# onofreiandrea/quantum_simulations

Measured on AMD Instinct MI355X. Metric: gate-applications/sec (random 1q+CX circuit, complex128 statevector), higher is better.
Workload: dtype f64

## Files before the change

### include/qsim_hip.h

```cpp
#ifndef QSIM_HIP_H
#define QSIM_HIP_H

#include <stdint.h>

#ifdef __cplusplus
extern "C" {
#endif

#define QSIM_OK            0
#define QSIM_ERR_INVALID  (-1)
#define QSIM_ERR_NONLOCAL (-2)
#define QSIM_ERR_HIP      (-3)
#define QSIM_ERR_NOMEM    (-4)

typedef struct qsim_chunk qsim_chunk;

const char* qsim_last_error(void);
int qsim_version(void);
int qsim_device_count(int* count);

int qsim_create(int device, int n_local_qubits, qsim_chunk** out);
int qsim_create_view(qsim_chunk* parent, uint64_t offset_amps, int n_local_qubits,
                     qsim_chunk** out);
int qsim_wrap(int device, void* device_ptr, int n_local_qubits, void* stream,
              qsim_chunk** out);
int qsim_destroy(qsim_chunk* c);
int qsim_n_local_qubits(const qsim_chunk* c);
void* qsim_device_ptr(const qsim_chunk* c);

int qsim_init_zero(qsim_chunk* c, int set_amp0);
int qsim_init_random(qsim_chunk* c, uint64_t seed);
int qsim_upload(qsim_chunk* c, const double* re_im, uint64_t offset_amps, uint64_t count);
int qsim_download(qsim_chunk* c, double* re_im, uint64_t offset_amps, uint64_t count);
int qsim_download_c64(qsim_chunk* c, float* re_im, uint64_t offset_amps, uint64_t count);
int qsim_upload_c64(qsim_chunk* c, const float* re_im, uint64_t offset_amps, uint64_t count);
int qsim_copy(qsim_chunk* dst, const qsim_chunk* src);
int qsim_copy_variant(qsim_chunk* dst, const qsim_chunk* src, int variant);

int qsim_apply_1q(qsim_chunk* c, int qubit, const double U[8]);
int qsim_apply_2q(qsim_chunk* c, int qa, int qb, const double U[32]);
int qsim_apply_fused_k(qsim_chunk* c, int k, const int32_t* qubits, const double* M);
int qsim_apply_ops(qsim_chunk* c, int n_ops, const int32_t* nq, const int32_t* qubits,
                   const double* mats);
int qsim_apply_ops_unfused(qsim_chunk* c, int n_ops, const int32_t* nq, const int32_t* qubits,
                           const double* mats);
int qsim_last_pass_count(const qsim_chunk* c);
int qsim_plan_cache_clear(void);
int qsim_apply_ops_tiled(qsim_chunk* c, int n_ops, const int32_t* nq, const int32_t* qubits, const double* mats,
                         int n_tiles, const uint64_t* tile_masks);

typedef struct {
  uint32_t struct_size;
  const qsim_chunk* src; int32_t src_m; int32_t src_bits[3];
  qsim_chunk* dst; int32_t dst_m; int32_t dst_bits[3];
  qsim_chunk* dst_own; int32_t own_pattern;
  int32_t dst_parts;
  int32_t src_parts;
  int32_t n_tiles;
  const uint64_t* tile_masks;
} qsim_ops_io;
int qsim_apply_ops_io(qsim_chunk* c, int n_ops, const int32_t* nq, const int32_t* qubits,
                      const double* mats, const qsim_ops_io* io, int* n_passes);
int qsim_apply_ops_io_own_slab(const qsim_chunk* c, int32_t* in_chunk);
int qsim_apply_ops_io_load(qsim_chunk* c, int part);
int qsim_apply_ops_io_source_parts(const qsim_chunk* c, int32_t* n_parts, uint64_t* piece_amps, int32_t* n_launches);
int qsim_apply_ops_io_parts(const qsim_chunk* c, int32_t* n_parts, uint64_t* piece_amps, int32_t* n_launches);
int qsim_apply_ops_io_part(qsim_chunk* c, int part);
int qsim_split_piece_count(int n_local_qubits, int m, int dst_parts);
int qsim_tiles_per_workgroup(int n_local_qubits, int tile_bits, int n_fixed_bits);
#define QSIM_PASS_IMAGE_BYTES 4096
int qsim_plan_ops(int n_local_qubits, int n_ops, const int32_t* nq, const int32_t* qubits, const double* mats,
                  void* out, uint64_t out_capacity_bytes, int32_t* n_passes);
int qsim_plan_ops_tiled(int n_local_qubits, int n_ops, const int32_t* nq, const int32_t* qubits, const double* mats,
                        int n_tiles, const uint64_t* tile_masks, void* out, uint64_t out_capacity_bytes, int32_t* n_passes);

int qsim_plan_peek_pass(int n_local_qubits, int n_total_qubits, int n_ops, const int32_t* nq, const int32_t* qubits,
                        const double* mats, const uint8_t* done, uint64_t avoid_mask, uint64_t hint_mask, uint64_t* tile_mask,
                        uint64_t* need_mask, int32_t* n_members, int32_t* members);

int qsim_plan_search(int n_local_qubits, int n_ops, const int32_t* nq, const int32_t* qubits, const double* mats, int beam,
                     uint64_t* out_masks, int out_capacity, int32_t* n_passes);

int qsim_rewrite_ops(int n_qubits, int n_ops, const int32_t* nq, const int32_t* qubits, const double* mats, int32_t* out_nq,
                     int32_t* out_qubits, double* out_mats, int out_capacity, int32_t* n_out, int32_t* need_tile);

int qsim_plan_count_layouts(int n_local_qubits, int n_ops, const int32_t* nq, const int32_t* qubits, const double* mats,
                            int n_layouts, const int32_t* layouts, int32_t* n_passes, int n_threads);

int qsim_choose_layout(int n_local_qubits, int n_tiles, const uint64_t* tile_masks, int top_bit, const double* bit_cost,
                       const double* pair_cost, const double* triple_cost , uint64_t seed,
                       int sweeps, int32_t* out_l2p, double* cost_identity, double* cost_chosen);

int qsim_apply_1q_pair(qsim_chunk* c0, qsim_chunk* c1, const double U[8]);
int qsim_apply_2q_pair_qa_local(qsim_chunk* c0, qsim_chunk* c1, int qa, const double U[32]);
int qsim_apply_2q_pair_qb_local(qsim_chunk* c0, qsim_chunk* c1, int qb, const double U[32]);
int qsim_apply_2q_quad(qsim_chunk* c00, qsim_chunk* c01, qsim_chunk* c10, qsim_chunk* c11,
                       const double U[32]);

int qsim_pack_half(const qsim_chunk* src, int bit, int value, qsim_chunk* buf);
int qsim_unpack_half(qsim_chunk* dst, int bit, int value, const qsim_chunk* buf);
int qsim_pack_bits(const qsim_chunk* src, int m, const int32_t* bits, int pattern,
                   qsim_chunk* buf, uint64_t buf_offset_amps);
int qsim_unpack_bits(qsim_chunk* dst, int m, const int32_t* bits, int pattern,
                     const qsim_chunk* buf, uint64_t buf_offset_amps);
int qsim_pack_all(const qsim_chunk* src, int m, const int32_t* bits, qsim_chunk* buf, int skip_pattern,
                  int piece, int n_pieces);
int qsim_unpack_all(qsim_chunk* dst, int m, const int32_t* bits, const qsim_chunk* buf, int skip_pattern,
                    int piece, int n_pieces);

int qsim_swap_global_local(qsim_chunk* const* chunks, int n_chunks, const int32_t* global_bits,
                           const int32_t* local_bits, int m);

#define QSIM_COMM_ID_BYTES 128
typedef struct qsim_comm qsim_comm;
int qsim_comm_get_unique_id(uint8_t id[QSIM_COMM_ID_BYTES]);
int qsim_comm_init(int device, int rank, int world, const uint8_t id[QSIM_COMM_ID_BYTES], qsim_comm** out);
int qsim_comm_destroy(qsim_comm* comm);
int qsim_comm_rank(const qsim_comm* comm);
int qsim_comm_world(const qsim_comm* comm);
int qsim_comm_exchange(qsim_comm* comm, int n_peers, const int32_t* peers, const qsim_chunk* send,
                       const uint64_t* send_off, qsim_chunk* recv, const uint64_t* recv_off, uint64_t count_amps);
int qsim_comm_exchange_bg(qsim_comm* comm, int n_peers, const int32_t* peers, const qsim_chunk* send,
                          const uint64_t* send_off, qsim_chunk* recv, const uint64_t* recv_off, uint64_t count_amps,
                          uint32_t* ticket);
int qsim_comm_join(qsim_comm* comm, qsim_chunk* c);
int qsim_comm_wait(qsim_comm* comm, qsim_chunk* c, uint32_t ticket);
int qsim_comm_relayout(qsim_comm* comm, qsim_chunk* state, qsim_chunk* buf0, qsim_chunk* buf1, int m,
                       const int32_t* local_bits, const int32_t* global_bits, int n_pieces);
int qsim_comm_relayout_plan(int rank, int world, int n_local_qubits, int m, const int32_t* local_bits,
                            const int32_t* global_bits, int n_pieces, int32_t* out_n_pieces, int32_t* out_n_peers,
                            int32_t* out_own_pattern, int32_t* out_peers, uint64_t* out_slab_offsets,
                            uint64_t* out_piece_amps);
int qsim_comm_relayout_loopback(qsim_comm* comm, qsim_chunk* state, qsim_chunk* buf0, qsim_chunk* buf1, int m,
                                const int32_t* local_bits, const int32_t* global_bits, int n_pieces, int as_rank,
                                int as_world);
int qsim_apply_1q_pair_remote(qsim_comm* comm, qsim_chunk* shard, qsim_chunk* buf, int partner_rank, int my_side,
                              const double U[8]);
int qsim_apply_2q_pair_qa_local_remote(qsim_comm* comm, qsim_chunk* shard, qsim_chunk* buf, int partner_rank,
                                       int my_side, int qa, const double U[32]);
int qsim_apply_2q_pair_qb_local_remote(qsim_comm* comm, qsim_chunk* shard, qsim_chunk* buf, int partner_rank,
                                       int my_side, int qb, const double U[32]);

int qsim_apply_2q_quad_remote(qsim_comm* comm, qsim_chunk* shard, qsim_chunk* buf, const int32_t ranks[4], int my_index,
                              const double U[32]);
typedef struct { int32_t n_ops; const int32_t* nq; const int32_t* qubits; const double* mats; } qsim_op_list;
int qsim_comm_relayout_fused(qsim_comm* comm, qsim_chunk* shard, qsim_chunk* send, qsim_chunk* recv,
                             const qsim_op_list* before, const qsim_op_list* after, int m, const int32_t* local_bits,
                             const int32_t* global_bits, int n_pieces, int as_rank, int as_world, int* n_passes);

int qsim_count_nonzero(qsim_chunk* c, double eps, uint64_t* count);
int qsim_export_nonzero(qsim_chunk* c, double eps, uint64_t capacity, uint64_t* out_idx, double* out_re_im,
                        uint64_t* n_rows);
int qsim_sync(qsim_chunk* c);
int qsim_norm2(qsim_chunk* c, double* out);
int qsim_probabilities(qsim_chunk* c, int r, const int32_t* qubits, double* out);
int qsim_reduced_density_matrix(qsim_chunk* c, int r, const int32_t* qubits, double* out);
int qsim_expectation_pauli(qsim_chunk* c, int n_terms, const uint64_t* x_masks, const uint64_t* z_masks, double* out,
                           int* n_passes);
int qsim_plan_expectation(int n_local_qubits, int n_terms, const uint64_t* x_masks, int32_t* pass_of_term,
                          uint64_t* tile_masks, int* n_passes);
int qsim_sample(qsim_chunk* c, uint64_t n_shots, const double* randnums, uint64_t* out_indices, double* total, int* n_passes);
int qsim_sample_locate(uint64_t n_blocks, const double* block_cdf, uint64_t n_shots, const double* randnums,
                       uint64_t* out_block, double* out_local);
int qsim_sample_block_bits(void);
int qsim_max_abs_err_closed_form(qsim_chunk* c, int kind, int n_total_qubits,
                                 uint64_t base_index, double* out);
int qsim_max_abs_err_closed_form_perm(qsim_chunk* c, int kind, int n_total_qubits,
                                      uint64_t base_index, const int32_t* log_to_phys,
                                      double* out);
int qsim_fingerprint(qsim_chunk* c, int n_total_qubits, uint64_t base_index, const int32_t* log_to_phys, uint64_t seed,
                     uint64_t sel_mask, uint64_t sel_value, double out[2]);
int qsim_time_begin(qsim_chunk* c);
int qsim_time_end(qsim_chunk* c, float* elapsed_ms);


typedef struct {
  char kernel[48];
  uint64_t launches;
  double total_ms;
  double algorithmic_bytes;
  double hbm_bytes;
  uint64_t streaming_launches;
} qsim_profile_entry;
int qsim_profile_begin(qsim_chunk* c);
int qsim_profile_end(qsim_chunk* c, int max_entries, int* n_entries, qsim_profile_entry* out);

#ifdef __cplusplus
}
#endif
#endif
```

### quantum_simulations_amd/_lib.py

```python
from __future__ import annotations

import ctypes as C
import os
from pathlib import Path

LIB_NAME = "libqsim_hip.so"
LIB_PATH = Path(os.environ.get("QSIM_LIBRARY") or (Path(__file__).resolve().parent / LIB_NAME))

QSIM_OK = 0
QSIM_ERR_INVALID = -1
QSIM_ERR_NONLOCAL = -2
QSIM_ERR_HIP = -3
QSIM_ERR_NOMEM = -4


class QsimLibraryMissing(RuntimeError):
    pass


class QsimHipError(RuntimeError):
    pass


_P = C.c_void_p
_D = C.POINTER(C.c_double)
_I32 = C.POINTER(C.c_int32)

SIGNATURES = {
    "qsim_last_error": (C.c_char_p, []),
    "qsim_version": (C.c_int, []),
    "qsim_device_count": (C.c_int, [C.POINTER(C.c_int)]),
    "qsim_create": (C.c_int, [C.c_int, C.c_int, C.POINTER(_P)]),
    "qsim_create_view": (C.c_int, [_P, C.c_uint64, C.c_int, C.POINTER(_P)]),
    "qsim_wrap": (C.c_int, [C.c_int, _P, C.c_int, _P, C.POINTER(_P)]),
    "qsim_destroy": (C.c_int, [_P]),
    "qsim_n_local_qubits": (C.c_int, [_P]),
    "qsim_device_ptr": (_P, [_P]),
    "qsim_init_zero": (C.c_int, [_P, C.c_int]),
    "qsim_init_random": (C.c_int, [_P, C.c_uint64]),
    "qsim_upload": (C.c_int, [_P, _P, C.c_uint64, C.c_uint64]),
    "qsim_download": (C.c_int, [_P, _P, C.c_uint64, C.c_uint64]),
    "qsim_download_c64": (C.c_int, [_P, _P, C.c_uint64, C.c_uint64]),
    "qsim_upload_c64": (C.c_int, [_P, _P, C.c_uint64, C.c_uint64]),
    "qsim_copy": (C.c_int, [_P, _P]),
    "qsim_copy_variant": (C.c_int, [_P, _P, C.c_int]),
    "qsim_apply_1q": (C.c_int, [_P, C.c_int, _P]),
    "qsim_apply_2q": (C.c_int, [_P, C.c_int, C.c_int, _P]),
    "qsim_apply_fused_k": (C.c_int, [_P, C.c_int, _P, _P]),
    "qsim_apply_ops": (C.c_int, [_P, C.c_int, _P, _P, _P]),
    "qsim_apply_ops_unfused": (C.c_int, [_P, C.c_int, _P, _P, _P]),
    "qsim_plan_ops": (C.c_int, [C.c_int, C.c_int, _P, _P, _P, _P, C.c_uint64, _P]),
    "qsim_plan_ops_tiled": (C.c_int, [C.c_int, C.c_int, _P, _P, _P, C.c_int, _P, _P, C.c_uint64, _P]),
    "qsim_plan_search": (C.c_int, [C.c_int, C.c_int, _P, _P, _P, C.c_int, _P, C.c_int, _P]),
    "qsim_rewrite_ops": (C.c_int, [C.c_int, C.c_int, _P, _P, _P, _P, _P, _P, C.c_int, _P, _P]),
    "qsim_apply_ops_tiled": (C.c_int, [_P, C.c_int, _P, _P, _P, C.c_int, _P]),
    "qsim_choose_layout": (C.c_int, [C.c_int, C.c_int, _P, C.c_int, _P, _P, _P, C.c_uint64, C.c_int, _P, C.POINTER(C.c_double), C.POINTER(C.c_double)]),
    "qsim_plan_count_layouts": (C.c_int, [C.c_int, C.c_int, _P, _P, _P, C.c_int, _P, _P, C.c_int]),
    "qsim_plan_peek_pass": (C.c_int, [C.c_int, C.c_int, C.c_int, _P, _P, _P, _P, C.c_uint64, C.c_uint64, C.POINTER(C.c_uint64),
                                      C.POINTER(C.c_uint64), C.POINTER(C.c_int32), _P]),
    "qsim_last_pass_count": (C.c_int, [_P]),
    "qsim_plan_cache_clear": (C.c_int, []),
    "qsim_apply_ops_io": (C.c_int, [_P, C.c_int, _P, _P, _P, _P, C.POINTER(C.c_int)]),
    "qsim_apply_ops_io_part": (C.c_int, [_P, C.c_int]),
    "qsim_apply_ops_io_load": (C.c_int, [_P, C.c_int]),
    "qsim_apply_ops_io_source_parts": (C.c_int, [_P, _P, _P, _P]),
    "qsim_apply_ops_io_parts": (C.c_int, [_P, _P, _P, _P]),
    "qsim_apply_ops_io_own_slab": (C.c_int, [_P, _P]),
    "qsim_split_piece_count": (C.c_int, [C.c_int, C.c_int, C.c_int]),
    "qsim_tiles_per_workgroup": (C.c_int, [C.c_int, C.c_int, C.c_int]),
    "qsim_apply_1q_pair": (C.c_int, [_P, _P, _P]),
    "qsim_apply_2q_pair_qa_local": (C.c_int, [_P, _P, C.c_int, _P]),
    "qsim_apply_2q_pair_qb_local": (C.c_int, [_P, _P, C.c_int, _P]),
    "qsim_apply_2q_quad": (C.c_int, [_P, _P, _P, _P, _P]),
    "qsim_pack_half": (C.c_int, [_P, C.c_int, C.c_int, _P]),
    "qsim_unpack_half": (C.c_int, [_P, C.c_int, C.c_int, _P]),
    "qsim_pack_bits": (C.c_int, [_P, C.c_int, _P, C.c_int, _P, C.c_uint64]),
    "qsim_unpack_bits": (C.c_int, [_P, C.c_int, _P, C.c_int, _P, C.c_uint64]),
    "qsim_pack_all": (C.c_int, [_P, C.c_int, _P, _P, C.c_int, C.c_int, C.c_int]),
    "qsim_unpack_all": (C.c_int, [_P, C.c_int, _P, _P, C.c_int, C.c_int, C.c_int]),
    "qsim_swap_global_local": (C.c_int, [_P, C.c_int, _P, _P, C.c_int]),
    "qsim_comm_get_unique_id": (C.c_int, [_P]),
    "qsim_comm_init": (C.c_int, [C.c_int, C.c_int, C.c_int, _P, C.POINTER(_P)]),
    "qsim_comm_destroy": (C.c_int, [_P]),
    "qsim_comm_rank": (C.c_int, [_P]),
    "qsim_comm_world": (C.c_int, [_P]),
    "qsim_comm_exchange": (C.c_int, [_P, C.c_int, _P, _P, _P, _P, _P, C.c_uint64]),
    "qsim_comm_exchange_bg": (C.c_int, [_P, C.c_int, _P, _P, _P, _P, _P, C.c_uint64, C.POINTER(C.c_uint32)]),
    "qsim_comm_wait": (C.c_int, [_P, _P, C.c_uint32]),
    "qsim_comm_join": (C.c_int, [_P, _P]),
    "qsim_comm_relayout": (C.c_int, [_P, _P, _P, _P, C.c_int, _P, _P, C.c_int]),
    "qsim_comm_relayout_plan": (C.c_int, [C.c_int, C.c_int, C.c_int, C.c_int, _P, _P, C.c_int, _P, _P, _P, _P, _P, _P]),
    "qsim_comm_relayout_loopback": (C.c_int, [_P, _P, _P, _P, C.c_int, _P, _P, C.c_int, C.c_int, C.c_int]),
    "qsim_apply_1q_pair_remote": (C.c_int, [_P, _P, _P, C.c_int, C.c_int, _P]),
    "qsim_apply_2q_pair_qa_local_remote": (C.c_int, [_P, _P, _P, C.c_int, C.c_int, C.c_int, _P]),
    "qsim_apply_2q_pair_qb_local_remote": (C.c_int, [_P, _P, _P, C.c_int, C.c_int, C.c_int, _P]),
    "qsim_apply_2q_quad_remote": (C.c_int, [_P, _P, _P, _P, C.c_int, _P]),
    "qsim_comm_relayout_fused": (C.c_int, [_P, _P, _P, _P, _P, _P, C.c_int, _P, _P, C.c_int, C.c_int, C.c_int, C.POINTER(C.c_int)]),
    "qsim_count_nonzero": (C.c_int, [_P, C.c_double, C.POINTER(C.c_uint64)]),
    "qsim_export_nonzero": (C.c_int, [_P, C.c_double, C.c_uint64, _P, _P, C.POINTER(C.c_uint64)]),
    "qsim_sync": (C.c_int, [_P]),
    "qsim_norm2": (C.c_int, [_P, C.POINTER(C.c_double)]),
    "qsim_probabilities": (C.c_int, [_P, C.c_int, _P, _P]),
    "qsim_reduced_density_matrix": (C.c_int, [_P, C.c_int, _P, _P]),
    "qsim_expectation_pauli": (C.c_int, [_P, C.c_int, _P, _P, _P, C.POINTER(C.c_int)]),
    "qsim_plan_expectation": (C.c_int, [C.c_int, C.c_int, _P, _P, _P, C.POINTER(C.c_int)]),
    "qsim_sample": (C.c_int, [_P, C.c_uint64, _P, _P, C.POINTER(C.c_double), C.POINTER(C.c_int)]),
    "qsim_sample_locate": (C.c_int, [C.c_uint64, _P, C.c_uint64, _P, _P, _P]),
    "qsim_sample_block_bits": (C.c_int, []),
    "qsim_max_abs_err_closed_form": (C.c_int, [_P, C.c_int, C.c_int, C.c_uint64,
                                               C.POINTER(C.c_double)]),
    "qsim_max_abs_err_closed_form_perm": (C.c_int, [_P, C.c_int, C.c_int, C.c_uint64, _P,
                                                    C.POINTER(C.c_double)]),
    "qsim_fingerprint": (C.c_int, [_P, C.c_int, C.c_uint64, _P, C.c_uint64, C.c_uint64, C.c_uint64, _P]),
    "qsim_time_begin": (C.c_int, [_P]),
    "qsim_time_end": (C.c_int, [_P, C.POINTER(C.c_float)]),
    "qsim_profile_begin": (C.c_int, [_P]),
    "qsim_profile_end": (C.c_int, [_P, C.c_int, C.POINTER(C.c_int), _P]),
}


class OpsIo(C.Structure):
    _fields_ = [("struct_size", C.c_uint32),
                ("src", C.c_void_p), ("src_m", C.c_int32), ("src_bits", C.c_int32 * 3),
                ("dst", C.c_void_p), ("dst_m", C.c_int32), ("dst_bits", C.c_int32 * 3),
                ("dst_own", C.c_void_p), ("own_pattern", C.c_int32), ("dst_parts", C.c_int32), ("src_parts", C.c_int32),
                ("n_tiles", C.c_int32), ("tile_masks", C.c_void_p)]

    def __init__(self, *args, **kw):
        super().__init__(*args, **kw)
        self.struct_size = C.sizeof(OpsIo)


class OpList(C.Structure):
    _fields_ = [("n_ops", C.c_int32), ("nq", C.c_void_p), ("qubits", C.c_void_p), ("mats", C.c_void_p)]


class ProfileEntry(C.Structure):
    _fields_ = [("kernel", C.c_char * 48), ("launches", C.c_uint64),
                ("total_ms", C.c_double), ("algorithmic_bytes", C.c_double),
                ("hbm_bytes", C.c_double), ("streaming_launches", C.c_uint64)]

_lib = None


def source_hash() -> str:
    import hashlib
    h = hashlib.sha256()
    csrc = Path(__file__).resolve().parent / "csrc"
    for path in sorted(list(csrc.glob("*.h")) + list(csrc.glob("*.hip")) + list(csrc.glob("*.py")) + [csrc / "Makefile"]):
        h.update(path.name.encode())
        h.update(path.read_bytes())
    return h.hexdigest()[:16]


def load() -> C.CDLL:
    global _lib
    if _lib is not None:
        return _lib
    if not LIB_PATH.exists():
        raise QsimLibraryMissing(
            f"{LIB_PATH} not found: the HIP extension is not built. Run "
            "`python -c 'import __graft_entry__ as g; g.build()'` (needs hipcc). "
            "This engine has no CPU fallback.")
    lib = C.CDLL(str(LIB_PATH))
    for name, (restype, argtypes) in SIGNATURES.items():
        fn = getattr(lib, name)
        fn.restype = restype
        fn.argtypes = argtypes
    _lib = lib
    return lib


def ptr(a):
    return None if a is None else a.ctypes.data_as(C.c_void_p)


def check(rc: int) -> None:
    if rc == QSIM_OK:
        return
    msg = (load().qsim_last_error() or b"").decode("utf-8", "replace")
    if rc == QSIM_ERR_NONLOCAL:
        raise NotImplementedError(msg)
    if rc == QSIM_ERR_INVALID:
        raise ValueError(msg)
    if rc == QSIM_ERR_NOMEM:
        raise MemoryError(msg)
    raise QsimHipError(msg)
```

### quantum_simulations_amd/csrc/abi_plan.h

```cpp
extern "C" {
int qsim_plan_cache_clear(void) {
  std::lock_guard<std::mutex> lock(g_plan_cache_mu);
  g_plan_cache.clear();
  return QSIM_OK;
}

static_assert(sizeof(TileArgs) == QSIM_PASS_IMAGE_BYTES, "pass image = the kernel-argument block of k_tile");

int qsim_plan_ops(int n_local_qubits, int n_ops, const int32_t* nq, const int32_t* qubits, const double* mats,
                  void* out, uint64_t out_capacity_bytes, int32_t* n_passes) {
  return qsim_plan_ops_tiled(n_local_qubits, n_ops, nq, qubits, mats, 0, nullptr, out, out_capacity_bytes, n_passes);
}

int qsim_plan_ops_tiled(int n_local_qubits, int n_ops, const int32_t* nq, const int32_t* qubits, const double* mats,
                        int n_tiles, const uint64_t* tile_masks, void* out, uint64_t out_capacity_bytes, int32_t* n_passes) {
  if (n_tiles < 0 || (n_tiles && !tile_masks)) return fail(QSIM_ERR_INVALID, "qsim_plan_ops_tiled: bad tile list");
  if (!n_passes) return fail(QSIM_ERR_INVALID, "qsim_plan_ops: n_passes is null");
  if (n_local_qubits < kTileMinChunk || n_local_qubits > kTileMaxQubits)
    return fail(QSIM_ERR_INVALID, "qsim_plan_ops: fused passes need %d..%d local qubits", kTileMinChunk, kTileMaxQubits);
  int rc = check_op_list(n_ops, nq, qubits, mats, n_local_qubits, kQubitOfPlan);
  if (rc) return rc;
  std::vector<FusedOp> ops;
  classify_ops(n_ops, nq, qubits, mats, &ops);
  int passes = 0;
  char* dst = (char*)out;
  uint64_t used = 0;
  const TileHint hint = {tile_masks, n_tiles};
  rc = plan_fused(n_local_qubits, ops, &passes, [&](TileArgs& a, int T, double, bool, bool) {
    if (dst) {
      if (used + sizeof(TileArgs) > out_capacity_bytes) return fail(QSIM_ERR_INVALID, "qsim_plan_ops: output buffer too small");
      std::memcpy(dst + used, &a, sizeof a);
    }
    used += sizeof(TileArgs);
    return (int)QSIM_OK;
  }, n_tiles ? &hint : nullptr);
  *n_passes = passes;
  return rc;
}

int qsim_plan_search(int n_local_qubits, int n_ops, const int32_t* nq, const int32_t* qubits, const double* mats, int beam,
                     uint64_t* out_masks, int out_capacity, int32_t* n_passes) {
  if (!n_passes || out_capacity < 0) return fail(QSIM_ERR_INVALID, "qsim_plan_search: bad arguments");
  if (n_local_qubits < kTileMinChunk || n_local_qubits > kTileMaxQubits)
    return fail(QSIM_ERR_INVALID, "qsim_plan_search: fused passes need %d..%d local qubits", kTileMinChunk, kTileMaxQubits);
  int rc = check_op_list(n_ops, nq, qubits, mats, n_local_qubits, kQubitOfPlan);
  if (rc) return rc;
  std::vector<FusedOp> ops;
  classify_ops(n_ops, nq, qubits, mats, &ops);
#ifdef QSIM_PROBES
  if (beam <= 0) if (const char* e = getenv("QSIM_PLAN_BEAM")) beam = atoi(e);
#endif
  std::vector<u64> masks;
  int passes = 0;
  rc = plan_search(n_local_qubits, ops, beam, &masks, &passes);
  if (rc) return rc;
  *n_passes = passes;
  if (out_masks) {
    if ((int)masks.size() > out_capacity) return fail(QSIM_ERR_INVALID, "qsim_plan_search: output buffer too small");
    for (size_t p = 0; p < masks.size(); ++p) out_masks[p] = masks[p];
  }
  return QSIM_OK;
}

int qsim_rewrite_ops(int n_qubits, int n_ops, const int32_t* nq, const int32_t* qubits, const double* mats, int32_t* out_nq,
                     int32_t* out_qubits, double* out_mats, int out_capacity, int32_t* n_out, int32_t* need_tile) {
  if (!n_out || out_capacity < 0 || (out_capacity && (!out_nq || !out_qubits || !out_mats)))
    return fail(QSIM_ERR_INVALID, "qsim_rewrite_ops: bad arguments");
  if (n_qubits < 1 || n_qubits > 63) return fail(QSIM_ERR_INVALID, "qsim_rewrite_ops: bad qubit count %d", n_qubits);
  int rc = check_op_list(n_ops, nq, qubits, mats, n_qubits, kQubitOfState);
  if (rc) return rc;
  std::vector<RwOp> ops;
  int need_in = 0, need_out = 0;
  rewrite_op_list(n_qubits, n_ops, nq, qubits, mats, &ops, &need_in);
  *n_out = (int32_t)ops.size();
  if (ops.size() > (size_t)out_capacity) return fail(QSIM_ERR_INVALID, "qsim_rewrite_ops: output buffer too small (%d ops)", (int)ops.size());
  for (size_t i = 0; i < ops.size(); ++i) {
    out_nq[i] = ops[i].nq;
    out_qubits[2 * i] = ops[i].q[0];
    out_qubits[2 * i + 1] = ops[i].nq == 2 ? ops[i].q[1] : 0;
    std::memcpy(out_mats + 32 * i, ops[i].U, sizeof ops[i].U);
    need_out += rw_needs_tile(ops[i]);
  }
  if (need_tile) { need_tile[0] = need_in; need_tile[1] = need_out; }
  return QSIM_OK;
}

int qsim_plan_peek_pass(int n_local_qubits, int n_total_qubits, int n_ops, const int32_t* nq, const int32_t* qubits,
                        const double* mats, const uint8_t* done, uint64_t avoid_mask, uint64_t hint_mask, uint64_t* tile_mask,
                        uint64_t* need_mask, int32_t* n_members, int32_t* members) {
  if (!done || !tile_mask || !n_members || !members) return fail(QSIM_ERR_INVALID, "qsim_plan_peek_pass: null argument");
  if (n_local_qubits < kTileMinChunk || n_local_qubits > kTileMaxQubits)
    return fail(QSIM_ERR_INVALID, "qsim_plan_peek_pass: fused passes need %d..%d local qubits", kTileMinChunk, kTileMaxQubits);
  if (n_total_qubits < n_local_qubits || n_total_qubits > 63) return fail(QSIM_ERR_INVALID, "qsim_plan_peek_pass: bad total qubit count %d", n_total_qubits);
  int rc = check_op_list(n_ops, nq, qubits, mats, n_total_qubits, kQubitOfState);
  if (rc) return rc;
  std::vector<FusedOp> ops;
  std::vector<int32_t> origin;
  classify_ops(n_ops, nq, qubits, mats, &ops, &origin);
  std::vector<uint8_t> done_ops;
  for (int32_t i : origin) done_ops.push_back(done[i]);
  std::vector<size_t> held;
  PeekPlan peek;
  peek.n_total = n_total_qubits;
  peek.done = done_ops.data();
  peek.avoid = avoid_mask;
  peek.tile_mask = peek.need_mask = 0;
  peek.members = &held;
  int passes = 0;
  const TileHint hint = {&hint_mask, 1};
  rc = plan_fused(n_local_qubits, ops, &passes, [](TileArgs&, int, double, bool, bool) { return (int)QSIM_OK; },
                  hint_mask ? &hint : nullptr, &peek);
  if (rc) return rc;
  *tile_mask = peek.tile_mask;
  if (need_mask) *need_mask = peek.need_mask;
  *n_members = (int32_t)held.size();
  for (size_t j = 0; j < held.size(); ++j) members[j] = origin[held[j]];
  return QSIM_OK;
}

int qsim_plan_count_layouts(int n_local_qubits, int n_ops, const int32_t* nq, const int32_t* qubits, const double* mats,
                            int n_layouts, const int32_t* layouts, int32_t* n_passes, int n_threads) {
  if (!n_passes || n_layouts < 0 || (n_layouts && !layouts)) return fail(QSIM_ERR_INVALID, "qsim_plan_count_layouts: bad arguments");
  if (n_local_qubits < kTileMinChunk || n_local_qubits > kTileMaxQubits)
    return fail(QSIM_ERR_INVALID, "qsim_plan_count_layouts: fused passes need %d..%d local qubits", kTileMinChunk, kTileMaxQubits);
  const int bad_ops = check_op_list(n_ops, nq, qubits, mats, n_local_qubits, kQubitOfPlan);
  if (bad_ops) return bad_ops;
  for (int l = 0; l < n_layouts; ++l) {
    u64 seen = 0;
    for (int q = 0; q < n_local_qubits; ++q) {
      const int b = layouts[(size_t)l * n_local_qubits + q];
      if (b < 0 || b >= n_local_qubits || ((seen >> b) & 1)) return fail(QSIM_ERR_INVALID, "qsim_plan_count_layouts: layout %d is not a permutation", l);
      seen |= 1ull << b;
    }
  }
  (void)tuning();
  std::atomic<int> next{0}, bad{0};
  auto work = [&]() {
    std::vector<FusedOp> ops;
    for (;;) {
      const int l = next.fetch_add(1);
      if (l >= n_layouts) return;
      const int32_t* lay = layouts + (size_t)l * n_local_qubits;
      ops.clear();
      for (int i = 0; i < n_ops; ++i) {
        const int32_t q[2] = {lay[qubits[2 * i]], nq[i] == 2 ? lay[qubits[2 * i + 1]] : -1};
        FusedOp o;
        if (classify_op(nq[i], q, mats + 32 * (size_t)i, &o)) ops.push_back(o);
      }
      int passes = 0;
      const int rc = plan_fused(n_local_qubits, ops, &passes, [](TileArgs&, int, double, bool, bool) { return (int)QSIM_OK; });
      if (rc) bad.store(1);
      n_passes[l] = rc ? -1 : passes;
    }
  };
  const int nt = std::max(1, std::min(n_threads > 0 ? n_threads : 1, std::min(n_layouts, 64)));
  std::vector<std::thread> pool;
  for (int t = 1; t < nt; ++t) pool.emplace_back(work);
  work();
  for (std::thread& t : pool) t.join();
  if (bad.load()) return fail(QSIM_ERR_INVALID, "qsim_plan_count_layouts: a layout could not be planned");
  return QSIM_OK;
}

int qsim_choose_layout(int n_local_qubits, int n_tiles, const uint64_t* tile_masks, int top_bit, const double* bit_cost,
                       const double* pair_cost, const double* triple_cost, uint64_t seed, int sweeps, int32_t* out_l2p,
                       double* cost_identity, double* cost_chosen) {
  const int n = n_local_qubits, low = kTileLow;
  if (n < low + 2 || n > 62 || n_tiles < 0 || (n_tiles && !tile_masks) || !bit_cost || !pair_cost || !out_l2p || top_bit < low || top_bit > 62 || sweeps < 1)
    return fail(QSIM_ERR_INVALID, "qsim_choose_layout: bad arguments");
  const int nb = top_bit - low + 1;
  std::vector<std::vector<int>> tiles((size_t)n_tiles);
  std::vector<std::vector<int>> member((size_t)n);
  for (int t = 0; t < n_tiles; ++t)
    for (int q = low; q < n; ++q)
      if ((tile_masks[t] >> q) & 1) { tiles[(size_t)t].push_back(q); member[(size_t)q].push_back(t); }
  std::vector<double> sym((size_t)nb * nb, 0.0);
  for (int a = 0; a < nb; ++a)
    for (int b = a + 1; b < nb; ++b) sym[(size_t)a * nb + b] = sym[(size_t)b * nb + a] = pair_cost[(size_t)a * nb + b];
  std::vector<int> l2p((size_t)n);
  for (int q = 0; q < n; ++q) l2p[(size_t)q] = q;
  auto cost_of = [&](int t) {
    int idx[64], m = 0;
    for (int q : tiles[(size_t)t]) idx[m++] = std::min(l2p[(size_t)q], top_bit) - low;
    double c = 0;
    for (int i = 0; i < m; ++i) {
      c += bit_cost[idx[i]];
      for (int j = i + 1; j < m; ++j) c += sym[(size_t)idx[i] * nb + idx[j]];
    }
    if (triple_cost) {
      std::sort(idx, idx + m);
      for (int i = 0; i < m; ++i)
        for (int j = i + 1; j < m; ++j) {
          if (idx[j] == idx[i]) continue;
          const double* row = triple_cost + ((size_t)idx[i] * nb + idx[j]) * nb;
          for (int l = j + 1; l < m; ++l) if (idx[l] != idx[j]) c += row[idx[l]];
        }
    }
    return c;
  };
  std::vector<double> costs((size_t)n_tiles);
  double cur = 0;
  for (int t = 0; t < n_tiles; ++t) cur += (costs[(size_t)t] = cost_of(t));
  const double identity = cur;
  double best = cur;
  std::vector<int> best_l2p = l2p;
  u64 rs = seed * 0x9E3779B97F4A7C15ull + 0x2545F4914F6CDD1Dull;
  auto rnd = [&]() { rs ^= rs << 13; rs ^= rs >> 7; rs ^= rs << 17; return rs; };
  const int np_ = n - low;
  const long steps = (long)sweeps * np_ * np_ / 2;
  const double T0 = std::max(1e-3, 0.03 * identity / std::max(1, n_tiles));
  std::vector<int> touched;
  std::vector<double> fresh;
  for (long it = 0; it < steps && n_tiles > 0; ++it) {
    const int a = low + (int)(rnd() % (u64)np_);
    int b = low + (int)(rnd() % (u64)(np_ - 1));
    if (b >= a) ++b;
    touched.clear();
    for (int t : member[(size_t)a]) touched.push_back(t);
    for (int t : member[(size_t)b]) if (std::find(touched.begin(), touched.end(), t) == touched.end()) touched.push_back(t);
    if (touched.empty()) continue;
    std::swap(l2p[(size_t)a], l2p[(size_t)b]);
    fresh.clear();
    double delta = 0;
    for (int t : touched) { fresh.push_back(cost_of(t)); delta += fresh.back() - costs[(size_t)t]; }
    const double T = T0 * (1.0 - (double)it / (double)steps) + 1e-4;
    const double u = (double)(rnd() >> 11) * 0x1p-53;
    if (delta < 0 || u < std::exp(-delta / T)) {
      for (size_t i = 0; i < touched.size(); ++i) costs[(size_t)touched[i]] = fresh[i];
      cur += delta;
      if (cur < best - 1e-12) { best = cur; best_l2p = l2p; }
    } else {
      std::swap(l2p[(size_t)a], l2p[(size_t)b]);
    }
  }
  for (int q = 0; q < n; ++q) out_l2p[q] = best_l2p[(size_t)q];
  if (cost_identity) *cost_identity = identity;
  if (cost_chosen) *cost_chosen = best;
  return QSIM_OK;
}

int qsim_split_piece_count(int n_local_qubits, int m, int dst_parts) {
  if (m < 1 || m > 3 || m > n_local_qubits || dst_parts == 0) return 1;
  return 1 << piece_bits_for(n_local_qubits, m, dst_parts < 0 ? -dst_parts : dst_parts, dst_parts < 0 ? kTileLow : 20);
}

int qsim_tiles_per_workgroup(int n_local_qubits, int tile_bits, int n_fixed_bits) {
  return tiles_per_workgroup(n_local_qubits, tile_bits, n_fixed_bits);
}
}
```

### quantum_simulations_amd/csrc/abi_relayout.h

```cpp

static int check_swapped_bits(int k, int g_bits, int m, const int32_t* local_bits, const int32_t* global_bits, const char* what,
                              const char* shards, const char* index_bit) {
  for (int i = 0; i < m; ++i) {
    if (local_bits[i] < 0 || local_bits[i] >= k) return fail(QSIM_ERR_NONLOCAL, "%s: local bit %d is non-local for 2^%d %s", what, local_bits[i], k, shards);
    if (global_bits[i] < 0 || global_bits[i] >= g_bits) return fail(QSIM_ERR_INVALID, "%s: %s %d out of range", what, index_bit, global_bits[i]);
    for (int j = 0; j < i; ++j)
      if (local_bits[j] == local_bits[i] || global_bits[j] == global_bits[i]) return fail(QSIM_ERR_INVALID, "%s: repeated bit", what);
  }
  return QSIM_OK;
}
static int peer_of(int rank, int m, const int32_t* global_bits, int d) {
  for (int i = 0; i < m; ++i) rank = (rank & ~(1 << global_bits[i])) | (((d >> i) & 1) << global_bits[i]);
  return rank;
}

static int partial_launch_args(const TileArgs& planned, int T, int k, const int* piece_bits, int n_free, int g, TileArgs* out) {
  *out = planned;
  out->nfix = (uint8_t)n_free;
  out->fix_or = 0;
  for (int i = 0; i < n_free; ++i) {
    const int bit = piece_bits[i];
    int below = 0;
    for (int j = 0; j < T - kTileLow; ++j) below += out->h[j] < bit;
    out->fix_pos[i] = (uint8_t)(bit - below);
    if ((g >> i) & 1) out->fix_or |= 1ull << bit;
    if (bit >= k || bit < kTileLow) return fail(QSIM_ERR_INVALID, "internal: piece bit %d", bit);
  }
  return QSIM_OK;
}

extern "C" {
static int half_slab(qsim_chunk* state, int bit, int value, qsim_chunk* buf, bool pack, const char* what) {
  int rc = check_chunk(state, what);
  if (rc || (rc = check_chunk(buf, what))) return rc;
  if (bit < 0 || bit >= state->k || buf->k != state->k - 1 || (value != 0 && value != 1))
    return fail(QSIM_ERR_INVALID, "%s: bit %d / buffer size mismatch", what, bit);
  HIP_TRY(hipSetDevice(state->device));
  const u64 n_half = amps(buf), off = value ? (1ull << bit) : 0ull;
  if (pack) hipLaunchKernelGGL(k_pack_half, dim3(stream_grid(n_half)), dim3(kBlock), 0, state->stream, buf->amp, (const double2*)state->amp, n_half, bit, off);
  else hipLaunchKernelGGL(k_unpack_half, dim3(stream_grid(n_half)), dim3(kBlock), 0, state->stream, state->amp, (const double2*)buf->amp, n_half, bit, off);
  HIP_TRY(hipGetLastError());
  return QSIM_OK;
}
int qsim_pack_half(const qsim_chunk* src, int bit, int value, qsim_chunk* buf) {
  return half_slab(const_cast<qsim_chunk*>(src), bit, value, buf, true, "qsim_pack_half");
}
int qsim_unpack_half(qsim_chunk* dst, int bit, int value, const qsim_chunk* buf) {
  return half_slab(dst, bit, value, const_cast<qsim_chunk*>(buf), false, "qsim_unpack_half");
}

static int slab_args(const qsim_chunk* c, int m, const int32_t* bits, int pattern, const qsim_chunk* buf,
                     uint64_t buf_offset, int pos[3], u64* value_off, u64* n_slab) {
  if (m < 1 || m > 3 || !bits) return fail(QSIM_ERR_INVALID, "slab: 1..3 bits expected, got %d", m);
  if (m > c->k) return fail(QSIM_ERR_INVALID, "slab: more bits than the chunk has");
  if (pattern < 0 || pattern >= (1 << m)) return fail(QSIM_ERR_INVALID, "slab: pattern out of range");
  int sorted[3] = {0, 0, 0};
  *value_off = 0;
  for (int i = 0; i < m; ++i) {
    if (bits[i] < 0 || bits[i] >= c->k) return fail(QSIM_ERR_INVALID, "slab: bit %d out of range", bits[i]);
    for (int j = 0; j < i; ++j)
      if (bits[j] == bits[i]) return fail(QSIM_ERR_INVALID, "slab: repeated bit %d", bits[i]);
    sorted[i] = bits[i];
    if ((pattern >> i) & 1) *value_off |= 1ull << bits[i];
  }
  std::sort(sorted, sorted + m);
  for (int i = 0; i < 3; ++i) pos[i] = sorted[i];
  *n_slab = 1ull << (c->k - m);
  if (buf_offset > amps(buf) || *n_slab > amps(buf) - buf_offset)
    return fail(QSIM_ERR_INVALID, "slab: buffer range outside the buffer chunk");
  return QSIM_OK;
}

static int one_slab(qsim_chunk* state, int m, const int32_t* bits, int pattern, qsim_chunk* buf, uint64_t buf_offset_amps,
                    bool pack, const char* what) {
  int rc = check_chunk(state, what);
  if (rc || (rc = check_chunk(buf, what))) return rc;
  int pos[3];
  u64 voff, n_slab;
  if ((rc = slab_args(state, m, bits, pattern, buf, buf_offset_amps, pos, &voff, &n_slab))) return rc;
  HIP_TRY(hipSetDevice(state->device));
  if (pack) hipLaunchKernelGGL(k_pack_bits, dim3(stream_grid(n_slab)), dim3(kBlock), 0, state->stream,
                               buf->amp + buf_offset_amps, (const double2*)state->amp, n_slab, m, pos[0], pos[1], pos[2], voff);
  else hipLaunchKernelGGL(k_unpack_bits, dim3(stream_grid(n_slab)), dim3(kBlock), 0, state->stream,
                          state->amp, (const double2*)buf->amp + buf_offset_amps, n_slab, m, pos[0], pos[1], pos[2], voff);
  HIP_TRY(hipGetLastError());
  return QSIM_OK;
}
int qsim_pack_bits(const qsim_chunk* src, int m, const int32_t* bits, int pattern, qsim_chunk* buf, uint64_t buf_offset_amps) {
  return one_slab(const_cast<qsim_chunk*>(src), m, bits, pattern, buf, buf_offset_amps, true, "qsim_pack_bits");
}
int qsim_unpack_bits(qsim_chunk* dst, int m, const int32_t* bits, int pattern, const qsim_chunk* buf, uint64_t buf_offset_amps) {
  return one_slab(dst, m, bits, pattern, const_cast<qsim_chunk*>(buf), buf_offset_amps, false, "qsim_unpack_bits");
}

static int slabs_all(qsim_chunk* state, int m, const int32_t* bits, qsim_chunk* buf, int skip_pattern, int piece,
                     int n_pieces, bool pack, const char* what) {
  int rc = check_chunk(state, what);
  if (rc || (rc = check_chunk(buf, what))) return rc;
  int pos[3];
  u64 voff, n_slab;
  if ((rc = slab_args(state, m, bits, 0, buf, 0, pos, &voff, &n_slab))) return rc;
  if (amps(buf) < amps(state)) return fail(QSIM_ERR_INVALID, "%s: the buffer must hold all 2^%d slabs", what, m);
  if (skip_pattern < -1 || skip_pattern >= (1 << m)) return fail(QSIM_ERR_INVALID, "%s: skip pattern out of range", what);
  int piece_bits = 0;
  while ((1 << piece_bits) < n_pieces) ++piece_bits;
  if (n_pieces < 1 || (1 << piece_bits) != n_pieces || piece_bits > 3 || piece_bits > state->k - m)
    return fail(QSIM_ERR_INVALID, "%s: n_pieces must be 1, 2, 4 or 8 and at most the slab length", what);
  if (piece < 0 || piece >= n_pieces) return fail(QSIM_ERR_INVALID, "%s: piece %d out of range", what, piece);
  int pb[3] = {0, 0, 0};
  top_free_bits(state->k, m, bits, piece_bits, pb);
  HIP_TRY(hipSetDevice(state->device));
  const int b0 = bits[0], b1 = m > 1 ? bits[1] : 0, b2 = m > 2 ? bits[2] : 0;
  const int s_lo = pos[0], s_mid = m > 1 ? pos[1] : 0, s_hi = m > 2 ? pos[2] : 0;
  const u64 n = amps(state) >> piece_bits;
  if (pack)
    hipLaunchKernelGGL((k_slabs_all<true>), dim3(stream_grid(n)), dim3(kBlock), 0, state->stream, state->amp, buf->amp,
                       n, m, b0, b1, b2, s_hi, s_mid, s_lo, state->k - m, skip_pattern, piece_bits, pb[0], pb[1], pb[2], piece);
  else
    hipLaunchKernelGGL((k_slabs_all<false>), dim3(stream_grid(n)), dim3(kBlock), 0, state->stream, state->amp, buf->amp,
                       n, m, b0, b1, b2, s_hi, s_mid, s_lo, state->k - m, skip_pattern, piece_bits, pb[0], pb[1], pb[2], piece);
  HIP_TRY(hipGetLastError());
  return QSIM_OK;
}

int qsim_pack_all(const qsim_chunk* src, int m, const int32_t* bits, qsim_chunk* buf, int skip_pattern, int piece, int n_pieces) {
  return slabs_all(const_cast<qsim_chunk*>(src), m, bits, buf, skip_pattern, piece, n_pieces, true, "qsim_pack_all");
}
int qsim_unpack_all(qsim_chunk* dst, int m, const int32_t* bits, const qsim_chunk* buf, int skip_pattern, int piece, int n_pieces) {
  return slabs_all(dst, m, bits, const_cast<qsim_chunk*>(buf), skip_pattern, piece, n_pieces, false, "qsim_unpack_all");
}

int qsim_swap_global_local(qsim_chunk* const* chunks, int n_chunks, const int32_t* global_bits, const int32_t* local_bits, int m) {
  if (!chunks || !global_bits || !local_bits) return fail(QSIM_ERR_INVALID, "qsim_swap_global_local: null argument");
  if (m < 1 || m > 3) return fail(QSIM_ERR_INVALID, "qsim_swap_global_local: 1..3 qubit pairs expected, got %d", m);
  if (n_chunks < 2 || (n_chunks & (n_chunks - 1)) || n_chunks > 4096)
    return fail(QSIM_ERR_INVALID, "qsim_swap_global_local: chunk count must be a power of two >= 2");
  int rc = QSIM_OK;
  for (int i = 0; i < n_chunks; ++i) {
    if ((rc = check_chunk(chunks[i], "qsim_swap_global_local"))) return rc;
    if (chunks[i]->k != chunks[0]->k || chunks[i]->device != chunks[0]->device)
      return fail(QSIM_ERR_INVALID, "qsim_swap_global_local: chunks differ in size or device");
  }
  const int k = chunks[0]->k;
  int g_bits = 0;
  while ((1 << g_bits) < n_chunks) ++g_bits;
  if ((rc = check_swapped_bits(k, g_bits, m, local_bits, global_bits, "qsim_swap_global_local", "chunks", "chunk-index bit"))) return rc;
  int sorted[3] = {0, 0, 0};
  std::copy(local_bits, local_bits + m, sorted);
  std::sort(sorted, sorted + m);
  HIP_TRY(hipSetDevice(chunks[0]->device));
  const u64 n_slab = 1ull << (k - m);
  auto local_offset = [&](int pattern) {
    u64 off = 0;
    for (int i = 0; i < m; ++i) if ((pattern >> i) & 1) off |= 1ull << local_bits[i];
    return off;
  };
  for (int c = 0; c < n_chunks; ++c) {
    int mine = 0;
    for (int i = 0; i < m; ++i) mine |= ((c >> global_bits[i]) & 1) << i;
    for (int d = 0; d < (1 << m); ++d) {
      if (d == mine) continue;
      const int peer = peer_of(c, m, global_bits, d);
      if (peer < c) continue;
      hipLaunchKernelGGL(k_swap_slabs, dim3(stream_grid(n_slab)), dim3(kBlock), 0, chunks[0]->stream,
                         chunks[c]->amp, chunks[peer]->amp, n_slab, m, sorted[0], sorted[1], sorted[2],
                         local_offset(d), local_offset(mine));
      HIP_TRY(hipGetLastError());
    }
  }
  return QSIM_OK;
}

static int finish_out_side(qsim_chunk* c, const qsim_ops_io* io, FusedIo& fio) {
  int rc = QSIM_OK;
  if (io->dst && io->dst_parts != 0) {
    PendingLast* p = c->pending ? c->pending : (c->pending = new PendingLast());
    const bool stashed = p->mode == PendingLast::kStashed;
    p->mode = stashed ? PendingLast::kTile : (fio.fused_out ? PendingLast::kDone : PendingLast::kPack);
    p->m = io->dst_m;
    for (int i = 0; i < io->dst_m; ++i) p->bits[i] = io->dst_bits[i];
    p->dst = io->dst; p->dst_own = io->dst_own; p->own_pattern = io->own_pattern;
    const int min_piece_bits = io->dst_parts < 0 ? kTileLow : 20;
    const int want = io->dst_parts < 0 ? -io->dst_parts : io->dst_parts;
    plan_parts(p, c->k, want, p->mode == PendingLast::kTile ? p->a.h : nullptr, p->mode == PendingLast::kTile ? p->T - kTileLow : 0, min_piece_bits);
  } else if (io->dst && !fio.fused_out) {
    if ((rc = slabs_all(c, io->dst_m, io->dst_bits, io->dst, io->own_pattern, 0, 1, true, "qsim_apply_ops_io"))) return rc;
    if (io->own_pattern >= 0) {
      const uint64_t slab = 1ull << (c->k - io->dst_m);
      if ((rc = qsim_pack_bits(c, io->dst_m, io->dst_bits, io->own_pattern, io->dst_own, (uint64_t)io->own_pattern * slab))) return rc;
    }
  }
  return QSIM_OK;
}

static int apply_ops_io_deferred(qsim_chunk* c, int n_ops, const int32_t* nq, const int32_t* qubits, const double* mats,
                                 const qsim_ops_io* io, const FusedIo& fio_in, const std::vector<FusedOp>& ops, bool tiles, int* n_passes) {
  DeferredIo* d = c->deferred ? c->deferred : (c->deferred = new DeferredIo());
  *d = DeferredIo();
  d->tiles = tiles;
  d->n_ops = n_ops;
  d->io = *io;
  d->fio = fio_in;
  const int want = io->src_parts < 0 ? -io->src_parts : io->src_parts;
  d->nb = piece_bits_for(c->k, io->src_m, want, io->src_parts < 0 ? kTileLow : 20);
  top_free_bits(c->k, io->src_m, io->src_bits, d->nb, d->piece_bit);
  int passes = 0, rc = QSIM_OK;
  if (io->src && !d->fio.src) ++passes;
  if (tiles) {
    int p = 0;
    const TileHint hint = {io->tile_masks, io->n_tiles};
    if ((rc = run_fused(c, ops, &p, &d->fio, n_ops, nq, qubits, mats, &d->passes, io->n_tiles ? &hint : nullptr))) return rc;
    d->io.tile_masks = nullptr;
    d->io.n_tiles = 0;
    passes += p;
    c->own_in_chunk = d->fio.own_in_chunk;
    if (d->fio.src && !d->fio.fused_in) return fail(QSIM_ERR_INVALID, "internal: the first pass did not take the source buffer");
    const bool first_stores = d->passes.size() == 1 && io->dst != nullptr;
    if (d->fio.src && !first_stores && !d->passes.empty() && d->passes[0].T == kTileBitsMax) {
      auto is_tile = [&](int b) { for (int j = 0; j < kTileBitsMax - kTileLow; ++j) if (d->passes[0].a.h[j] == b) return true; return false; };
      while (d->nb_free < d->nb && !is_tile(d->piece_bit[d->nb - 1 - d->nb_free])) ++d->nb_free;
    }
  } else {
    d->nq.assign(nq, nq + n_ops);
    d->qubits.assign(qubits, qubits + 2 * (size_t)n_ops);
    d->mats.assign(mats, mats + 32 * (size_t)n_ops);
    passes += n_ops;
  }
  if (io->dst && !d->fio.fused_out) ++passes;
  d->active = true;
  c->last_passes = passes;
  if (n_passes) *n_passes = passes;
  return QSIM_OK;
}

int qsim_apply_ops_io(qsim_chunk* c, int n_ops, const int32_t* nq, const int32_t* qubits, const double* mats, const qsim_ops_io* io, int* n_passes) {
  int rc = validate_ops(c, n_ops, nq, qubits, mats);
  if (rc) return rc;
  if (!io) return fail(QSIM_ERR_INVALID, "qsim_apply_ops_io: io is null");
  if (io->struct_size != sizeof(qsim_ops_io))
    return fail(QSIM_ERR_INVALID, "qsim_apply_ops_io: io->struct_size is %u, this library's qsim_ops_io has %zu bytes (zero the struct, "
                "set struct_size = sizeof(qsim_ops_io) and rebuild against this library's include/qsim_hip.h)", io->struct_size, sizeof(qsim_ops_io));
  if (io->n_tiles < 0 || (io->n_tiles && !io->tile_masks)) return fail(QSIM_ERR_INVALID, "qsim_apply_ops_io: bad tile list");
  auto check_side = [&](const qsim_chunk* b, int m, const int32_t* bits, const char* side) -> int {
    int r = check_chunk(b, "qsim_apply_ops_io");
    if (r) return r;
    if (b->k != c->k || b->device != c->device || b->amp == c->amp)
      return fail(QSIM_ERR_INVALID, "qsim_apply_ops_io: the %s buffer must be a distinct chunk of the state's size and device", side);
    if (m < 1 || m > 3 || m > c->k) return fail(QSIM_ERR_INVALID, "qsim_apply_ops_io: %s: 1..3 slab bits expected, got %d", side, m);
    for (int i = 0; i < m; ++i) {
      if (bits[i] < 0 || bits[i] >= c->k) return fail(QSIM_ERR_NONLOCAL, "qsim_apply_ops_io: %s slab bit %d is non-local for 2^%d amplitudes", side, bits[i], c->k);
      for (int j = 0; j < i; ++j) if (bits[j] == bits[i]) return fail(QSIM_ERR_INVALID, "qsim_apply_ops_io: %s: repeated slab bit %d", side, bits[i]);
    }
    return QSIM_OK;
  };
  if (io->src && (rc = check_side(io->src, io->src_m, io->src_bits, "source"))) return rc;
  if (io->dst) {
    if ((rc = check_side(io->dst, io->dst_m, io->dst_bits, "destination"))) return rc;
    if (io->own_pattern < -1 || io->own_pattern >= (1 << io->dst_m)) return fail(QSIM_ERR_INVALID, "qsim_apply_ops_io: own_pattern out of range");
    if (io->own_pattern >= 0 && (rc = check_side(io->dst_own, io->dst_m, io->dst_bits, "own-slab"))) return rc;
    if (io->own_pattern >= 0 && io->dst_own->amp == io->dst->amp) return fail(QSIM_ERR_INVALID, "qsim_apply_ops_io: the own-slab buffer must differ from the destination");
    if (io->src && io->src->amp == io->dst->amp)
      return fail(QSIM_ERR_INVALID, "qsim_apply_ops_io: the source buffer must differ from the destination buffer (one pass may read and write them at once)");
  }
  HIP_TRY(hipSetDevice(c->device));
  std::vector<FusedOp> ops;
  classify_ops(n_ops, nq, qubits, mats, &ops);
  const bool tiles = c->k >= kTileMinChunk && c->k <= kTileMaxQubits && !ops.empty();
  auto whole_lines = [](int m, const int32_t* bits) { for (int i = 0; i < m; ++i) if (bits[i] < kTileLow) return false; return true; };
  FusedIo fio;
  if (io->src && tiles && whole_lines(io->src_m, io->src_bits)) {
    fio.src = io->src;
    fio.in.m = io->src_m;
    for (int i = 0; i < io->src_m; ++i) fio.in.bits[i] = io->src_bits[i];
  }
  if (io->dst && tiles && whole_lines(io->dst_m, io->dst_bits)) {
    fio.dst = io->dst;
    fio.dst_own = io->dst_own;
    fio.own_pattern = io->own_pattern;
    fio.out.m = io->dst_m;
    for (int i = 0; i < io->dst_m; ++i) fio.out.bits[i] = io->dst_bits[i];
  }
  const bool parts = io->dst && io->dst_parts != 0;
  c->own_in_chunk = false;
  if (parts_pending(c))
    return fail(QSIM_ERR_INVALID, "qsim_apply_ops_io: pieces of an earlier split call are pending on this chunk (qsim_apply_ops_io_part / _load)");
  fio.parts = parts;
  if (io->src && io->src_parts != 0) return apply_ops_io_deferred(c, n_ops, nq, qubits, mats, io, fio, ops, tiles, n_passes);
  int passes = 0;
  if (io->src && !fio.src) {
    if ((rc = slabs_all(c, io->src_m, io->src_bits, const_cast<qsim_chunk*>(io->src), -1, 0, 1, false, "qsim_apply_ops_io"))) return rc;
    ++passes;
  }
  if (tiles) {
    int p = 0;
    const TileHint hint = {io->tile_masks, io->n_tiles};
    if ((rc = run_fused(c, ops, &p, &fio, n_ops, nq, qubits, mats, nullptr, io->n_tiles ? &hint : nullptr))) return rc;
    passes += p;
    c->own_in_chunk = fio.own_in_chunk;
    if (fio.src && !fio.fused_in) return fail(QSIM_ERR_INVALID, "internal: the first pass did not take the source buffer");
  } else {
    if ((rc = qsim_apply_ops_unfused(c, n_ops, nq, qubits, mats))) return rc;
    passes += n_ops;
  }
  if (io->dst && !fio.fused_out) ++passes;
  if ((rc = finish_out_side(c, io, fio))) return rc;
  c->last_passes = passes;
  if (n_passes) *n_passes = passes;
  return QSIM_OK;
}

int qsim_apply_ops_io_part(qsim_chunk* c, int part) {
  int rc = check_chunk(c, "qsim_apply_ops_io_part");
  if (rc) return rc;
  PendingLast* p = c->pending;
  if (!p || p->mode == PendingLast::kNone) return fail(QSIM_ERR_INVALID, "qsim_apply_ops_io_part: no split op list is pending on this chunk");
  const int n_parts = 1 << p->nb;
  if (part < 0 || part >= n_parts) return fail(QSIM_ERR_INVALID, "qsim_apply_ops_io_part: piece %d out of range", part);
  if ((p->stored >> part) & 1) return fail(QSIM_ERR_INVALID, "qsim_apply_ops_io_part: piece %d has been stored already", part);
  HIP_TRY(hipSetDevice(c->device));
  if (p->mode == PendingLast::kTile) {
    const int g = part >> (p->nb - p->nb_free);
    if (!((p->launched >> g) & 1)) {
      TileArgs a;
      if ((rc = partial_launch_args(p->a, p->T, c->k, p->piece_bit + (p->nb - p->nb_free), p->nb_free, g, &a))) return rc;
      if ((rc = launch_tile_any(a, p->T, c, c->stream, p->alg_bytes / (double)(1 << p->nb_free)))) return rc;
      p->launched |= 1u << g;
    }
  } else if (p->mode == PendingLast::kPack) {
    if ((rc = slabs_all(c, p->m, p->bits, p->dst, p->own_pattern, part, n_parts, true, "qsim_apply_ops_io_part"))) return rc;
    if (p->own_pattern >= 0 && p->stored == 0) {
      const uint64_t slab = 1ull << (c->k - p->m);
      if ((rc = qsim_pack_bits(c, p->m, p->bits, p->own_pattern, p->dst_own, (uint64_t)p->own_pattern * slab))) return rc;
    }
  }
  p->stored |= 1u << part;
  if (p->stored == (1u << n_parts) - 1u) p->mode = PendingLast::kNone;
  return QSIM_OK;
}

int qsim_apply_ops_io_load(qsim_chunk* c, int part) {
  int rc = check_chunk(c, "qsim_apply_ops_io_load");
  if (rc) return rc;
  DeferredIo* d = c->deferred;
  if (!d || !d->active) return fail(QSIM_ERR_INVALID, "qsim_apply_ops_io_load: no op list with a split source is pending on this chunk");
  const int n_parts = 1 << d->nb;
  if (part < 0 || part >= n_parts) return fail(QSIM_ERR_INVALID, "qsim_apply_ops_io_load: piece %d out of range", part);
  if ((d->announced >> part) & 1) return fail(QSIM_ERR_INVALID, "qsim_apply_ops_io_load: piece %d has been announced already", part);
  HIP_TRY(hipSetDevice(c->device));
  PendingGuard guard{c, true};
  d->announced |= 1u << part;
  const qsim_ops_io* io = &d->io;
  if (!d->fio.src) {
    if ((rc = slabs_all(c, io->src_m, io->src_bits, const_cast<qsim_chunk*>(io->src), -1, part, n_parts, false, "qsim_apply_ops_io_load"))) return rc;
  } else if (d->nb_free > 0) {
    const int shift = d->nb - d->nb_free;
    const int g = part >> shift;
    const unsigned group = ((1u << (1 << shift)) - 1u) << (g << shift);
    if ((d->announced & group) == group && !((d->launched >> g) & 1)) {
      CachedPass& p0 = d->passes[0];
      TileArgs a;
      if ((rc = partial_launch_args(p0.a, p0.T, c->k, d->piece_bit + shift, d->nb_free, g, &a))) return rc;
      if ((rc = launch_tile_any(a, p0.T, c, c->stream, p0.alg_bytes / (double)(1 << d->nb_free)))) return rc;
      d->launched |= 1u << g;
    }
  }
  if (d->announced != (n_parts >= 32 ? ~0u : (1u << n_parts) - 1u)) { guard.armed = false; return QSIM_OK; }
  d->active = false;
  if (d->tiles) {
    for (size_t i = 0; i < d->passes.size(); ++i) {
      if (i == 0 && d->nb_free > 0) continue;
      CachedPass& p = d->passes[i];
      if ((rc = dispatch_planned(c, p.a, p.T, p.alg_bytes, i + 1 == d->passes.size(), &d->fio))) return rc;
    }
  } else {
    if ((rc = qsim_apply_ops_unfused(c, d->n_ops, d->nq.data(), d->qubits.data(), d->mats.data()))) return rc;
  }
  if ((rc = finish_out_side(c, io, d->fio))) return rc;
  guard.armed = false;
  return QSIM_OK;
}

int qsim_apply_ops_io_own_slab(const qsim_chunk* c, int32_t* in_chunk) {
  if (!c || !in_chunk) return fail(QSIM_ERR_INVALID, "qsim_apply_ops_io_own_slab: null argument");
  *in_chunk = c->own_in_chunk ? 1 : 0;
  return QSIM_OK;
}

int qsim_apply_ops_io_source_parts(const qsim_chunk* c, int32_t* n_parts, uint64_t* piece_amps, int32_t* n_launches) {
  if (!c || !c->deferred || !c->deferred->active) return fail(QSIM_ERR_INVALID, "qsim_apply_ops_io_source_parts: nothing pending on this chunk");
  const DeferredIo* d = c->deferred;
  if (n_parts) *n_parts = 1 << d->nb;
  if (piece_amps) *piece_amps = (1ull << (c->k - d->io.src_m)) >> d->nb;
  if (n_launches) *n_launches = d->nb_free > 0 ? (1 << d->nb_free) : 0;
  return QSIM_OK;
}

int qsim_apply_ops_io_parts(const qsim_chunk* c, int32_t* n_parts, uint64_t* piece_amps, int32_t* n_launches) {
  if (!c || !c->pending || c->pending->mode == PendingLast::kNone) return fail(QSIM_ERR_INVALID, "qsim_apply_ops_io_parts: no split op list is pending on this chunk");
  const PendingLast* p = c->pending;
  if (n_parts) *n_parts = 1 << p->nb;
  if (piece_amps) *piece_amps = (1ull << (c->k - p->m)) >> p->nb;
  if (n_launches) *n_launches = p->mode == PendingLast::kTile ? (1 << p->nb_free) : (p->mode == PendingLast::kPack ? (1 << p->nb) : 0);
  return QSIM_OK;
}
}
```

### quantum_simulations_amd/csrc/tile_groups.h

```cpp

template <class Fn>
static void for_each_triple(unsigned mask, Fn&& fn) {
  for (unsigned a = mask; a; a &= a - 1)
    for (unsigned b = a & (a - 1); b; b &= b - 1)
      for (unsigned c = b & (b - 1); c; c &= c - 1) fn((a & -a) | (b & -b) | (c & -c));
}

struct PhaseRuns {
  struct Acc { uint16_t blk; u64 outer; double2 phi[3]; unsigned touched; };
  std::vector<Acc> open;

  static int run_bytes(unsigned touched) { const int n = __builtin_popcount(touched); return desc_bytes(n == 1 ? 2 : (n == 2 ? 6 : 14)); }
  int reserve() const {
    int bytes = 0;
    for (const Acc& acc : open) bytes += run_bytes(acc.touched);
    return bytes;
  }
  void add(uint16_t blk, u64 outer, int r, double2 phase) {
    size_t i = 0;
    while (i < open.size() && !(open[i].blk == blk && open[i].outer == outer)) ++i;
    if (i == open.size()) {
      Acc acc;
      acc.blk = blk; acc.outer = outer; acc.touched = 0;
      for (int e = 0; e < 3; ++e) acc.phi[e] = make_double2(1.0, 0.0);
      open.push_back(acc);
    }
    Acc& acc = open[i];
    acc.phi[r] = cmul(acc.phi[r], phase);
    acc.touched |= 1u << r;
  }
  static TileDesc single(const TileDesc& pred, int r, double2 v) {
    TileDesc s1 = pred;
    const int fam = phase_family(v);
    s1.opcode = (uint8_t)(fam + (1u << r));
    if (fam == OPC_PHASE) { s1.m[0] = v.x; s1.m[1] = v.y; s1.nd = 2; }
    return s1;
  }
  static int cost1(double2 v) {
    if (!tuning().tile_special) return 16;
    return (v.x == -1 && v.y == 0) ? 8 : ((v.x == 0 && (v.y == 1 || v.y == -1)) ? 12 : 16);
  }
  int flush(size_t i, std::vector<TileDesc>* gates) {
    const Acc acc = open[i];
    open.erase(open.begin() + (long)i);
    const size_t from = gates->size();
    TileDesc d;
    std::memset(&d, 0, sizeof d);
    d.blk_mask = acc.blk;
    d.outer_mask = acc.outer;
    double2 m[3];
    int nm = 0, regs[3];
    for (int r = 0; r < 3; ++r) if (acc.touched & (1u << r)) { regs[nm] = r; m[nm++] = acc.phi[r]; }
    auto put = [&](int at, double2 v) { d.m[2 * at] = v.x; d.m[2 * at + 1] = v.y; };
    int separate = 0;
    for (int e = 0; e < nm; ++e) separate += cost1(m[e]);
    if (nm == 1 || separate < (nm == 2 ? 24 : 28)) {
      for (int e = 0; e < nm; ++e) gates->push_back(single(d, regs[e], m[e]));
    } else if (nm == 2) {
      d.opcode = (uint8_t)(OPC_DIAGR + (acc.touched == 3 ? 0 : acc.touched == 5 ? 1 : 2));
      put(0, m[0]); put(1, m[1]); put(2, cmul(m[0], m[1])); d.nd = 6;
      gates->push_back(d);
    } else {
      d.opcode = (uint8_t)(OPC_DIAGR + 3);
      const double2 ab = cmul(m[0], m[1]);
      put(0, m[0]); put(1, m[1]); put(2, m[2]);
      put(3, ab); put(4, cmul(m[0], m[2])); put(5, cmul(m[1], m[2])); put(6, cmul(ab, m[2]));
      d.nd = 14;
      gates->push_back(d);
    }
    int bytes = 0;
    for (size_t g = from; g < gates->size(); ++g) bytes += desc_bytes((*gates)[g]);
    return bytes;
  }
};

struct GroupEmitter {
  static constexpr int kDirectWorth = 2;

  const std::vector<FusedOp>& ops;
  const std::vector<size_t>& members;
  const std::vector<int>& high;
  const int T, low = kTileLow;
  std::vector<TileGroup>* out;
  std::vector<char>* emitted;
  const unsigned line_bits = (1u << kTileLow) - 1;
  const bool merge_on = tuning().tile_merge_diag != 0;
  const bool direct_ends;
  double pass_scale = 1.0;
  std::vector<char> done;
  size_t left;
  int used = 0;
  int regs[kGroupBits] = {0, 0, 0};
  std::vector<char> reserved;
  unsigned last_own = 0;
  int reserve_bytes = 0;
  size_t n_reserved = 0;

  struct Item { FusedOp op; size_t mi; int with_next; };
  struct Half { FusedOp op; size_t stands_for; };

  GroupEmitter(const std::vector<FusedOp>& ops_, const std::vector<size_t>& members_, const std::vector<int>& high_, int T_,
               std::vector<TileGroup>* out_, std::vector<char>* emitted_)
      : ops(ops_), members(members_), high(high_), T(T_), out(out_), emitted(emitted_),
        direct_ends(tuning().tile_direct && T_ == kTileBitsMax), done(members_.size(), 0), left(members_.size()),
        reserved(members_.size(), 0) {}

  static void emit(const std::vector<FusedOp>& ops, const std::vector<size_t>& members, const std::vector<int>& high, int T,
                   std::vector<TileGroup>* out, std::vector<char>* emitted, bool last_search = false) {
    GroupEmitter e(ops, members, high, T, out, emitted);
    out->clear();
    if (e.direct_ends && last_search && members.size() > 1) e.reserve_last();
    while (e.left > e.n_reserved) {
      std::vector<size_t> grp;
      unsigned claimed = 0;
      e.next_group(&grp, &claimed);
      if (grp.empty()) break;
      if (e.write_group(grp, claimed)) break;
    }
    if (e.n_reserved) e.write_reserved();
    e.move_last_forward();
    e.apply_scale();
  }

  int tile_pos(int b) const {
    if (b < low) return b;
    for (size_t j = 0; j < high.size(); ++j) if (high[j] == b) return low + (int)j;
    return -1;
  }
  int reg_pos(int tile_bit) const {
    for (int j = 0; j < kGroupBits; ++j) if (regs[j] == tile_bit) return j;
    return -1;
  }
  struct Pending { size_t mi; u64 qm; unsigned need; int bytes; };
  Pending pending(size_t mi, int phase_bytes) const {
    const FusedOp& o = ops[members[mi]];
    const OpShape shape = op_shape(o);
    unsigned need = 0;
    for (int t = 0; t < o.ntargets; ++t) need |= 1u << tile_pos(o.target[t]);
    return Pending{mi, op_qmask(o), need, phase_bytes ? phase_bytes : desc_bytes(shape.nd)};
  }

  int terminal(const std::vector<Pending>& tail, unsigned own, std::vector<char>* mark) {
    u64 blocked = 0;
    int count = 0, bytes = kGroupRecordBytes;
    for (size_t mi = members.size(); mi-- > 0;) {
      const Pending& t = tail[mi];
      if ((blocked & t.qm) || (t.need & ~own) || bytes + t.bytes > kTileRecordBudget / 2) { blocked |= t.qm; continue; }
      bytes += t.bytes;
      ++count;
      if (mark) (*mark)[mi] = 1;
    }
    if (mark) reserve_bytes = bytes;
    return count;
  }
  void reserve_last() {
    std::vector<Pending> tail;
    unsigned cand = 0;
    for (size_t mi = 0; mi < members.size(); ++mi) {
      tail.push_back(pending(mi, ops[members[mi]].kind == TG_PHASE ? 48 : 0));
      cand |= tail[mi].need & ~line_bits;
    }
    int best = 0;
    while (__builtin_popcount(cand) < kGroupBits)
      for (int b = T - 1; b >= low; --b) if (!(cand & (1u << b))) { cand |= 1u << b; break; }
    for_each_triple(cand, [&](unsigned own) {
      const int count = terminal(tail, own, nullptr);
      if (count > best) { best = count; last_own = own; }
    });
    if (best > 0 && (size_t)best < members.size()) {
      n_reserved = (size_t)terminal(tail, last_own, &reserved);
      used = reserve_bytes;
    } else {
      last_own = 0;
    }
  }
  void write_reserved() {
    used -= reserve_bytes;
    std::vector<size_t> grp;
    u64 blocked = 0;
    for (size_t mi = 0; mi < members.size(); ++mi) {
      if (done[mi]) continue;
      const u64 qm = op_qmask(ops[members[mi]]);
      if (!reserved[mi] || (blocked & qm)) { blocked |= qm; continue; }
      grp.push_back(mi);
    }
    if (!grp.empty()) write_group(grp, last_own);
  }

  int select(const std::vector<Pending>& pend, unsigned own, std::vector<size_t>* grp_out, unsigned* claimed_out) const {
    const bool first_come = own == 0;
    u64 blocked = 0;
    int est = used + kGroupRecordBytes, count = 0;
    unsigned claimed = own;
    for (const Pending& pd : pend) {
      bool ok = !(blocked & pd.qm);
      if (ok && first_come && __builtin_popcount(claimed | pd.need) > kGroupBits) ok = false;
      if (ok && !first_come && (pd.need & ~own)) ok = false;
      if (ok && est + pd.bytes > kTileRecordBudget) ok = false;
      if (!ok) { blocked |= pd.qm; continue; }
      claimed |= pd.need;
      est += pd.bytes;
      ++count;
      if (grp_out) grp_out->push_back(pd.mi);
    }
    if (claimed_out) *claimed_out = first_come ? claimed : own;
    return count;
  }
  int score(int count, unsigned own_bits) const {
    const bool want_direct = out->empty() && direct_ends;
    return count * 2 + ((want_direct && !(own_bits & line_bits)) ? 2 * kDirectWorth - 1 : 0);
  }
  void next_group(std::vector<size_t>* grp, unsigned* claimed) const {
    std::vector<Pending> pend;
    pend.reserve(left);
    unsigned cand_mask = 0;
    for (size_t mi = 0; mi < members.size(); ++mi) {
      if (done[mi] || reserved[mi]) continue;
      pend.push_back(pending(mi, (merge_on && op_shape(ops[members[mi]]).family == OPC_PHASE) ? 16 : 0));
      cand_mask |= pend.back().need;
    }
    unsigned best_own = 0;
    unsigned fc_claimed = 0;
    const int fc_count = select(pend, 0, nullptr, &fc_claimed);
    int best_score = score(fc_count, fc_claimed);
    if (tuning().tile_group_search && __builtin_popcount(cand_mask) > kGroupBits)
      for_each_triple(cand_mask, [&](unsigned own) {
        const int count = select(pend, own, nullptr, nullptr);
        if (count > 0 && score(count, own) > best_score) { best_score = score(count, own); best_own = own; }
      });
    select(pend, best_own, grp, claimed);
  }

  std::vector<Item> mux_pairs(const std::vector<size_t>& grp) const {
    const size_t ng = grp.size();
    std::vector<Item> seq;
    seq.reserve(ng + 4);
    std::vector<char> gone(ng, 0), paired(ng, 0);
    std::vector<Half> first_half(ng);
    auto op_at = [&](size_t g) -> const FusedOp& { return ops[members[grp[g]]]; };
    auto is_plain_1q = [](const FusedOp& u) { return (u.kind == TG_DENSE1 || u.kind == TG_ANTI1) && u.control < 0; };
    for (size_t p = 0; p < (tuning().tile_mux ? ng : 0); ++p) {
      const FusedOp& cv = op_at(p);
      if (gone[p] || paired[p] || cv.control < 0 || tile_pos(cv.control) >= 0) continue;
      if (cv.kind != TG_SWAP1 && cv.kind != TG_ANTI1 && cv.kind != TG_DENSE1) continue;
      const u64 tbit = 1ull << cv.target[0];
      long partner = -1;
      bool u_first = false;
      for (size_t q = p + 1; q < ng; ++q) {
        if (gone[q] || !(op_qmask(op_at(q)) & tbit)) continue;
        if (is_plain_1q(op_at(q)) && !paired[q]) partner = (long)q;
        break;
      }
      if (partner < 0) {
        bool touched_later = false;
        for (size_t q = p + 1; q < ng && !touched_later; ++q) touched_later = !gone[q] && (op_qmask(op_at(q)) & tbit);
        if (cv.kind == TG_SWAP1 && tuning().tile_sink_swaps && !touched_later) continue;
        for (size_t q = p; q-- > 0;) {
          if (gone[q] || !(op_qmask(op_at(q)) & tbit)) continue;
          if (is_plain_1q(op_at(q)) && !paired[q]) { partner = (long)q; u_first = true; }
          break;
        }
      }
      if (partner < 0) continue;
      const FusedOp& u = op_at((size_t)partner);
      Half& half = first_half[(size_t)partner];
      half.op = cv;
      if (u_first) mul2x2(cv.m, u.m, half.op.m); else mul2x2(u.m, cv.m, half.op.m);
      set_1q_kind(&half.op);
      half.stands_for = p;
      paired[(size_t)partner] = 1;
      gone[p] = 1;
    }
    for (size_t q = 0; q < ng; ++q) {
      if (gone[q]) continue;
      const FusedOp& u = op_at(q);
      if (!paired[q]) { seq.push_back(Item{u, grp[q], 0}); continue; }
      const FusedOp& a = first_half[q].op;
      FusedOp b = u;
      b.control = a.control;
      b.control_zero = true;
      b.nq = 2;
      b.qubits[1] = a.control;
      seq.push_back(Item{a, grp[first_half[q].stands_for], desc_bytes(op_shape(b).nd)});
      seq.push_back(Item{b, grp[q], 0});
    }
    return seq;
  }

  TileDesc describe(const FusedOp& o, const OpShape& shape, u64 touched_later, unsigned* reg_mask) {
    TileDesc d;
    std::memset(&d, 0, sizeof d);
    int ctrl_reg = -1;
    *reg_mask = 0;
    auto require_one = [&](int qubit) {
      const int p = tile_pos(qubit);
      if (p < 0) { d.outer_mask |= 1ull << qubit; return; }
      const int r = reg_pos(p);
      if (r >= 0) { *reg_mask |= 1u << r; ctrl_reg = r; }
      else d.blk_mask |= (uint16_t)(1u << p);
    };
    auto put = [&](int at, double2 v) { d.m[2 * at] = v.x; d.m[2 * at + 1] = v.y; };
    if (o.kind == TG_PHASE) {
      for (int t = 0; t < o.nbits; ++t) require_one(o.bits[t]);
      d.opcode = (uint8_t)(shape.family + *reg_mask);
      if (shape.nd) { put(0, o.m[0]); d.nd = 2; }
    } else if (o.kind == TG_DENSE2) {
      d.opcode = (uint8_t)(OPC_DENSE2 + 3 * reg_pos(tile_pos(o.target[0])) + reg_pos(tile_pos(o.target[1])));
      for (int e = 0; e < 16; ++e) put(e, o.m[e]);
      d.nd = 32;
    } else {
      const int J = reg_pos(tile_pos(o.target[0]));
      if (o.control >= 0 && o.control_zero) { d.outer_mask |= 1ull << o.control; d.outer_zero = true; }
      else if (o.control >= 0) require_one(o.control);
      d.opcode = (uint8_t)(shape.family + opc_1q_variant(J, ctrl_reg));
      if (shape.family == OPC_SWAP1 && tuning().tile_sink_swaps &&
          !(touched_later & (1ull << o.target[0])) && !(ctrl_reg >= 0 && (touched_later & (1ull << o.control))))
        d.opcode = (uint8_t)(OPC_ASWAP1 + opc_1q_variant(J, ctrl_reg));
      if (shape.family == OPC_HAD1) {
        pass_scale *= o.m[0].x;
      } else if (shape.family == OPC_REAL1) {
        d.m[0] = o.m[0].x; d.m[1] = o.m[1].x; d.m[2] = o.m[2].x; d.m[3] = o.m[3].x; d.nd = 4;
      } else if (shape.family == OPC_ANTI1) {
        put(0, o.m[1]); put(1, o.m[2]); d.nd = 4;
      } else if (shape.family == OPC_DENSE1) {
        for (int e = 0; e < 4; ++e) put(e, o.m[e]);
        d.nd = 8;
      }
    }
    return d;
  }

  bool write_group(const std::vector<size_t>& grp, unsigned claimed) {
    std::vector<int> S;
    for (unsigned m = claimed; m; m &= m - 1) S.push_back(__builtin_ctz(m));
    for (int b = T - 1; (int)S.size() < kGroupBits && b >= 0; --b)
      if (std::find(S.begin(), S.end(), b) == S.end()) S.push_back(b);
    std::sort(S.begin(), S.end());
    TileGroup tg;
    for (int j = 0; j < 3; ++j) tg.s[j] = regs[j] = S[j];
    tg.qmask = 0;
    used += kGroupRecordBytes;
    PhaseRuns runs;
    const std::vector<Item> seq = mux_pairs(grp);
    std::vector<u64> later(seq.size() + 1, 0);
    for (size_t i = seq.size(); i-- > 0;) later[i] = later[i + 1] | op_qmask(seq[i].op);
    bool cut = false;
    size_t gi = 0;
    for (const Item& item : seq) {
      const u64 touched_later = later[++gi];
      const FusedOp& o = item.op;
      const OpShape shape = op_shape(o);
      {
        const bool mergeable = merge_on && o.kind == TG_PHASE;
        if (used + runs.reserve() + (mergeable ? desc_bytes(14) : desc_bytes(shape.nd)) + item.with_next > kTileRecordBudget) { cut = true; break; }
      }
      done[item.mi] = 1;
      (*emitted)[item.mi] = 1;
      --left;
      tg.qmask |= op_qmask(o);
      unsigned reg_mask = 0;
      const TileDesc d = describe(o, shape, touched_later, &reg_mask);
      if (o.kind == TG_PHASE && merge_on && __builtin_popcount(reg_mask) == 1) {
        runs.add(d.blk_mask, d.outer_mask, __builtin_ctz(reg_mask), o.m[0]);
        continue;
      }
      if (o.kind != TG_PHASE) {
        unsigned tmask = 0;
        for (int t = 0; t < o.ntargets; ++t) tmask |= 1u << reg_pos(tile_pos(o.target[t]));
        for (size_t i = runs.open.size(); i-- > 0;) if (runs.open[i].touched & tmask) used += runs.flush(i, &tg.gates);
      }
      used += desc_bytes(d);
      tg.gates.push_back(d);
    }
    while (!runs.open.empty()) used += runs.flush(0, &tg.gates);
    if (!tg.gates.empty()) out->push_back(tg);
    else used -= kGroupRecordBytes;
    return cut;
  }

  void move_last_forward() {
    if (!(tuning().tile_direct && T == kTileBitsMax && out->size() > 1 && out->back().s[0] < low)) return;
    size_t at = out->size() - 1;
    while (at > 0 && !((*out)[at].qmask & (*out)[at - 1].qmask)) { std::swap((*out)[at], (*out)[at - 1]); --at; }
    if (out->back().s[0] < low)
      while (at + 1 < out->size()) { std::swap((*out)[at], (*out)[at + 1]); ++at; }
  }
  void apply_scale() {
    if (!(pass_scale != 1.0 && !out->empty())) return;
    TileDesc* host = nullptr;
    for (TileGroup& g : *out)
      for (TileDesc& d : g.gates) {
        const bool fam = (d.opcode >= OPC_REAL1 && d.opcode < OPC_REAL1 + 3) || (d.opcode >= OPC_DENSE1 && d.opcode < OPC_DENSE1 + 3) ||
                         (d.opcode >= OPC_ANTI1 && d.opcode < OPC_ANTI1 + 3);
        if (fam && !d.blk_mask && !d.outer_mask && !host) host = &d;
      }
    if (host) {
      for (int e = 0; e < host->nd; ++e) host->m[e] *= pass_scale;
    } else {
      TileDesc d;
      std::memset(&d, 0, sizeof d);
      d.opcode = OPC_SCALE;
      d.m[0] = pass_scale;
      d.nd = 1;
      out->back().gates.push_back(d);
    }
  }
};
```

### quantum_simulations_amd/csrc/tile_kernel.h

```cpp
#include "tile_engine_gen.h"

#ifndef QSIM_TILE_LOW
#define QSIM_TILE_LOW 3
#endif
constexpr int kTileLow = QSIM_TILE_LOW;
#ifndef QSIM_TILE_BITS_MAX
#define QSIM_TILE_BITS_MAX 11
#endif
constexpr int kTileBitsMax = QSIM_TILE_BITS_MAX;
constexpr int kGroupBits = 3;
#ifndef QSIM_TILE_THREAD_BITS
#define QSIM_TILE_THREAD_BITS 8
#endif
constexpr int kTileThreadBits = QSIM_TILE_THREAD_BITS;
constexpr int kTileThreads = 1 << kTileThreadBits;
constexpr int kTileMaxQubits = 35;

enum : uint8_t {
  OPC_NOP = QS_ENT_NOP,
  OPC_DENSE1 = QS_ENT_DENSE1,
  OPC_SWAP1 = QS_ENT_SWAP1,
  OPC_ANTI1 = QS_ENT_ANTI1,
  OPC_PHASE = QS_ENT_PHASE,
  OPC_DENSE2 = QS_ENT_DENSE2,
  OPC_REAL1 = QS_ENT_REAL1,
  OPC_YLIKE1 = QS_ENT_YLIKE1,
  OPC_PHASE_NEG = QS_ENT_PHASE_NEG,
  OPC_PHASE_I = QS_ENT_PHASE_I,
  OPC_PHASE_NI = QS_ENT_PHASE_NI,
  OPC_DIAGR = QS_ENT_DIAGR,
  OPC_PRED_OUTER = QS_ENT_PRED_OUTER,
  OPC_PRED_LANE = QS_ENT_PRED_LANE,
  OPC_GROUP = QS_ENT_GROUP,
  OPC_GROUP_FIRST = QS_ENT_GROUP_FIRST,
  OPC_END = QS_ENT_END,
  OPC_HAD1 = QS_ENT_HAD1,
  OPC_SCALE = QS_ENT_SCALE,
  OPC_ASWAP1 = QS_ENT_ASWAP1,
  OPC_GROUP_DIRECT = QS_ENT_GROUP_DIRECT,
  OPC_END_DIRECT = QS_ENT_END_DIRECT,
  OPC_PRED_OUTER_ZERO = QS_ENT_PRED_OUTER_ZERO
};
static inline int opc_1q_variant(int J, int C) {
  return C < 0 ? J : 3 + 2 * J + ((C > J ? C - 1 : C) == 0 ? 0 : 1);
}

constexpr int kTileArgBytes = 4096;
constexpr int kTileStreamOff = 192;
constexpr int kTileStreamBytes = kTileArgBytes - kTileStreamOff;
constexpr int kTileStreamSlack = 48;

struct TileSlab {
  u64 field[4];
  uint8_t bit[3];
  uint8_t top;
  uint8_t pad[4];
};
struct TileArgs {
  double2* amp;
  int nrec;
  int T;
  uint8_t h[11];
  uint8_t order;
  uint32_t ntiles;
  uint8_t lay_in[12];
  uint8_t lay_out[12];
  double2* amp_out;
  double2* amp_out_own;
  u64 own_mask, own_value;
  TileSlab slab_in, slab_out;
  uint8_t nbits;
  uint8_t perm;
  uint8_t nfix;
  uint8_t fix_pos[3];
  uint8_t reserved0[2];
  u64 fix_or;
  uint8_t reserved[8];
  uint32_t stream[kTileStreamBytes / 4];
};
constexpr uint8_t kTilePermIn = 1, kTilePermOut = 2, kTileOwnOut = 4;
constexpr uint8_t kTileDirectIn = 0x10, kTileDirectOut = 0x20, kTileOrderMask = 0x03;
static_assert(sizeof(TileArgs) == kTileArgBytes, "kernel arguments are one 4 KiB block");
static_assert(offsetof(TileArgs, nbits) % 8 == 0 && offsetof(TileArgs, nfix) == offsetof(TileArgs, nbits) + 2 &&
              offsetof(TileArgs, fix_pos) == offsetof(TileArgs, nbits) + 3 && offsetof(TileArgs, fix_or) == offsetof(TileArgs, nbits) + 8,
              "k_tile<PART> reads {nbits .. fix_pos} and fix_or as two aligned 8-byte words");
static_assert(offsetof(TileArgs, stream) == kTileStreamOff, "record offsets are relative to the argument block");

__host__ __device__ __forceinline__ unsigned lds_slot(unsigned t) { return t ^ ((t >> 4) & 15u); }

constexpr int tile_waves(int T, int tiles_per_wg = 1) {
  const int granules = ((1 << T) * 16 + 1279) / 1280;
  const int per_simd = (128 / granules) * (kTileThreads / 256);
  return per_simd > 5 ? 5 : (per_simd < 1 ? 1 : per_simd);
}

template <int T, bool NT, bool WIDE, int TPW, bool PART = false>
__global__ __launch_bounds__(kTileThreads, tile_waves(T, TPW)) void k_tile(const TileArgs a) {
  constexpr int N = 1 << T;
  constexpr int LOW = kTileLow;
  constexpr int NH = T - LOW;
  constexpr int BLOCK = kTileThreads;
  constexpr int TB = kTileThreadBits;
  constexpr int PER = N / BLOCK;
  constexpr int NBLK = N >> kGroupBits;
  static_assert(N >= BLOCK && NBLK <= BLOCK, "one register block per thread, at least one element per thread");
#ifndef QSIM_LDS_PAD_ELEMS
#define QSIM_LDS_PAD_ELEMS 0
#endif
  __shared__ double2 lds[N + QSIM_LDS_PAD_ELEMS];
#ifdef QSIM_PROBES
  unsigned long long* const stamps = *reinterpret_cast<unsigned long long* const*>(&a.stream[(kTileArgBytes - 8 - kTileStreamOff) / 4]);
  const unsigned long long t_entry = __builtin_readcyclecounter();
  unsigned long long t_loaded = 0, t_engine = 0;
#endif
  const int tid = threadIdx.x;
  int hs[NH];
#pragma unroll
  for (int j = 0; j < NH; ++j) hs[j] = __builtin_amdgcn_readfirstlane((int)a.h[j]);
  using off_t = typename std::conditional<WIDE, u64, unsigned>::type;
  constexpr int NTB = (TB - LOW) < NH ? (TB - LOW) : NH;
  const bool din = (a.order & kTileDirectIn) != 0, dout = (a.order & kTileDirectOut) != 0;
  auto thread_off = [&](const uint8_t* lay) -> off_t {
    off_t o = tid & ((1 << LOW) - 1);
#pragma unroll
    for (int i = 0; i < NTB; ++i) o |= (off_t)((tid >> (LOW + i)) & 1) << __builtin_amdgcn_readfirstlane((int)lay[i]);
    return o;
  };
  const off_t tin = thread_off(a.lay_in), tout = thread_off(a.lay_out);
  int rin[NH - NTB + 1], rout[NH - NTB + 1];
#pragma unroll
  for (int i = NTB; i < NH; ++i) {
    rin[i - NTB] = __builtin_amdgcn_readfirstlane((int)a.lay_in[i]);
    rout[i - NTB] = __builtin_amdgcn_readfirstlane((int)a.lay_out[i]);
  }
  const unsigned nfix = PART ? __builtin_amdgcn_readfirstlane((unsigned)a.nfix) : 0u;
  auto tile_base = [&](unsigned i) -> u64 {
    unsigned tile = blockIdx.x * TPW + i;
#ifdef QSIM_PROBES
    if ((a.order & kTileOrderMask) == 1) tile = (tile * 0x9E3779B1u) & (a.ntiles - 1);
    if ((a.order & kTileOrderMask) == 2) tile = a.ntiles > 1 ? __brev(tile) >> (__clz(a.ntiles) + 1) : 0;
#endif
    u64 base = (u64)tile << LOW;
    u64 fix_or = 0;
    if (PART && nfix) {
      typedef __attribute__((address_space(4))) const u64 cu64_t;
      cu64_t* fp = (cu64_t*)((__attribute__((address_space(4))) const char*)__builtin_amdgcn_kernarg_segment_ptr() + offsetof(TileArgs, nbits));
      asm volatile("" : "+s"(fp));
      const u64 w0 = fp[0];
      fix_or = fp[1];
      for (unsigned j = 0; j < nfix; ++j) {
        const int p = (int)((w0 >> (8 * (3 + j))) & 0xffu);
        base = ((base >> p) << (p + 1)) | (base & ((1ull << p) - 1));
      }
    }
#pragma unroll
    for (int j = 0; j < NH; ++j) {
      const int p = hs[j];
      base = ((base >> p) << (p + 1)) | (base & ((1ull << p) - 1));
    }
    return base | fix_or;
  };
  const unsigned perm = __builtin_amdgcn_readfirstlane((unsigned)a.perm);
  typedef __attribute__((address_space(4))) const TileSlab cslab_t;
  auto slab_base = [&](u64 lbase, unsigned off) -> u64 {
    cslab_t* sp = (cslab_t*)((__attribute__((address_space(4))) const char*)__builtin_amdgcn_kernarg_segment_ptr() + off);
    asm volatile("" : "+s"(sp));
    u64 o = (lbase & sp->field[0]) | ((lbase & sp->field[1]) >> 1) | ((lbase & sp->field[2]) >> 2) | ((lbase & sp->field[3]) >> 3);
#pragma unroll
    for (int j = 0; j < 3; ++j) o |= ((lbase >> sp->bit[j]) & 1ull) << (sp->top + j);
    return o;
  };
  auto base_in = [&](u64 lbase) -> u64 { return (perm & kTilePermIn) ? slab_base(lbase, (unsigned)offsetof(TileArgs, slab_in)) : lbase; };
  auto base_out = [&](u64 lbase) -> u64 { return (perm & kTilePermOut) ? slab_base(lbase, (unsigned)offsetof(TileArgs, slab_out)) : lbase; };
  typedef double amp_t __attribute__((ext_vector_type(2)));
  typedef __attribute__((address_space(1))) amp_t gamp_t;
  auto element = [&](u64 base, int j, off_t toff, const int* rbits, double2* amp) -> gamp_t* {
    u64 oj = 0;
#pragma unroll
    for (int i = 0; i < NH - NTB; ++i) oj |= (u64)((j >> i) & 1) << rbits[i];
    if constexpr (WIDE) {
      return (gamp_t*)(u64)(amp + base + toff + oj);
    } else {
      const u64 r = reinterpret_cast<u64>(amp + base + oj);
      const u64 row = ((u64)__builtin_amdgcn_readfirstlane((unsigned)(r >> 32)) << 32) |
                      (unsigned)__builtin_amdgcn_readfirstlane((unsigned)r);
      unsigned tb = toff << 4;
      asm volatile("" : "+v"(tb));
      return (gamp_t*)((__attribute__((address_space(1))) char*)row + tb);
    }
  };
#ifndef QSIM_TILE_LOAD_NT
#define QSIM_TILE_LOAD_NT 1
#endif
#ifndef QSIM_TILE_STORE_NT
#define QSIM_TILE_STORE_NT 1
#endif
  auto load = [&](gamp_t* p) -> amp_t { return (NT && QSIM_TILE_LOAD_NT) ? __builtin_nontemporal_load(p) : *p; };
  auto store = [&](gamp_t* p, amp_t v) { if (NT && QSIM_TILE_STORE_NT) __builtin_nontemporal_store(v, p); else *p = v; };
  auto store_to = [&](u64 lbase) -> double2* {
    return ((perm & kTileOwnOut) && (lbase & a.own_mask) == a.own_value) ? a.amp_out_own : a.amp_out;
  };
  const unsigned slot0 = lds_slot(tid);
  static_assert(BLOCK >= 256, "lds_slot(tid + BLOCK * j) = lds_slot(tid) + BLOCK * j needs BLOCK to be a multiple of 256");
  amp_t* const tile = reinterpret_cast<amp_t*>(lds);
  u64 base = tile_base(0);
  amp_t v[PER];
  {
    const u64 pb = base_in(base);
#pragma unroll
    for (int j = 0; j < PER; ++j) v[j] = load(element(pb, j, tin, rin, a.amp));
  }
#pragma unroll 1
  for (int it = 0; it < TPW; ++it) {
    amp_t x[8];
#pragma unroll
    for (int j = 0; j < 8; ++j) x[j] = j < PER ? v[j < PER ? j : 0] : amp_t{0.0, 0.0};
    if (!din) {
#pragma unroll
      for (int j = 0; j < PER; ++j) tile[slot0 + BLOCK * j] = v[j];
      __syncthreads();
    }
    const u64 cur = base;
    if (it + 1 < TPW) {
      base = tile_base(it + 1);
      const u64 pb = base_in(base);
#pragma unroll
      for (int j = 0; j < PER; ++j) v[j] = load(element(pb, j, tin, rin, a.amp));
    }
#ifdef QSIM_PROBES
    if (it == 0) t_loaded = __builtin_readcyclecounter();
#endif
    {
      const auto karg = __builtin_amdgcn_kernarg_segment_ptr();
      const unsigned baseh = __builtin_amdgcn_readfirstlane((unsigned)(cur >> LOW));
      if constexpr (NBLK == BLOCK) {
        asm volatile(QS_ENGINE_ASM_FULL
                     : "+{v[4:7]}"(x[0]), "+{v[8:11]}"(x[1]), "+{v[12:15]}"(x[2]), "+{v[16:19]}"(x[3]),
                       "+{v[20:23]}"(x[4]), "+{v[24:27]}"(x[5]), "+{v[28:31]}"(x[6]), "+{v[32:35]}"(x[7])
                     : [tid] "v"(tid), [karg] "s"(karg), [baseh] "s"(baseh), [first] "i"(kTileStreamOff)
                     : QS_ENGINE_CLOBBERS);
      } else {
        asm volatile(QS_ENGINE_ASM_PARTIAL
                     : "+{v[4:7]}"(x[0]), "+{v[8:11]}"(x[1]), "+{v[12:15]}"(x[2]), "+{v[16:19]}"(x[3]),
                       "+{v[20:23]}"(x[4]), "+{v[24:27]}"(x[5]), "+{v[28:31]}"(x[6]), "+{v[32:35]}"(x[7])
                     : [tid] "v"(tid), [karg] "s"(karg), [baseh] "s"(baseh), [first] "i"(kTileStreamOff), [nblk] "s"(NBLK)
                     : QS_ENGINE_CLOBBERS);
      }
    }
#ifdef QSIM_PROBES
    if (it == 0) t_engine = __builtin_readcyclecounter();
#endif
    double2* const dst = store_to(cur);
    const u64 pcur = base_out(cur);
    if (dout) {
#pragma unroll
      for (int j = 0; j < PER; ++j) store(element(pcur, j, tout, rout, dst), x[j < 8 ? j : 0]);
    } else {
      amp_t w[PER];
#pragma unroll
      for (int j = 0; j < PER; ++j) w[j] = tile[slot0 + BLOCK * j];
#pragma unroll
      for (int j = 0; j < PER; ++j) store(element(pcur, j, tout, rout, dst), w[j]);
    }
    if (it + 1 < TPW) __syncthreads();
  }
#ifdef QSIM_PROBES
  if (stamps && tid == 0 && (blockIdx.x & 63) == 0) {
    unsigned long long* o = stamps + 4 * (blockIdx.x >> 6);
    o[0] = t_entry; o[1] = t_loaded; o[2] = t_engine; o[3] = __builtin_readcyclecounter();
  }
#endif
}

struct TileDesc {
  uint8_t opcode;
  uint16_t blk_mask;
  u64 outer_mask;
  bool outer_zero;
  int nd;
  double m[32];
};
struct TileGroup {
  int s[3];
  u64 qmask = 0;
  std::vector<TileDesc> gates;
};

static inline int desc_bytes(int nd) { return 16 + ((8 * nd + 15) & ~15); }
static inline int desc_bytes(const TileDesc& d) { return desc_bytes(d.nd); }
constexpr int kGroupRecordBytes = 48;
constexpr int kEndRecordBytes = 16;
constexpr int kScaleRecordBytes = 32;
constexpr int kTileRecordBudget = kTileStreamBytes - kEndRecordBytes - kTileStreamSlack - kScaleRecordBytes;

static int serialize_pass(const std::vector<TileGroup>& groups, TileArgs* a) {
  unsigned char* const base = reinterpret_cast<unsigned char*>(a);
  int off = kTileStreamOff;
  int nrec = 0;
  auto put32 = [&](int at, uint32_t v) { std::memcpy(base + at, &v, 4); };
  auto room = [&](int bytes) { return off + bytes + kEndRecordBytes + kTileStreamSlack <= kTileArgBytes; };
  bool first = true;
  if (groups.empty()) return fail(QSIM_ERR_INVALID, "internal: a pass needs at least one register group");
  const int nh = a->T - kTileLow;
  const bool full = a->T == kTileBitsMax && kTileBitsMax - kTileLow == kTileThreadBits;
  auto layout = [&](const TileGroup& g, uint8_t* lay) -> bool {
    const bool direct = full && tuning().tile_direct && g.s[0] >= kTileLow;
    if (!direct) {
      for (int i = 0; i < nh; ++i) lay[i] = a->h[i];
      return false;
    }
    int nt = 0;
    for (int b = kTileLow; b < a->T; ++b)
      if (b != g.s[0] && b != g.s[1] && b != g.s[2]) lay[nt++] = a->h[b - kTileLow];
    for (int i = 0; i < 3; ++i) lay[nt + i] = a->h[g.s[i] - kTileLow];
    return true;
  };
  const bool din = layout(groups.front(), a->lay_in), dout = layout(groups.back(), a->lay_out);
  a->order = (uint8_t)((a->order & kTileOrderMask) | (din ? kTileDirectIn : 0) | (dout ? kTileDirectOut : 0));
  for (const TileGroup& g : groups) {
    if (!room(kGroupRecordBytes)) return fail(QSIM_ERR_INVALID, "internal: pass record stream overflow");
    put32(off + 0, 4u * (first ? (din ? OPC_GROUP_DIRECT : OPC_GROUP_FIRST) : OPC_GROUP));
    put32(off + 4, (uint32_t)(off + kGroupRecordBytes));
    for (int i = 0; i < 3; ++i) put32(off + 8 + 4 * i, ~0u << g.s[i]);
    for (int r = 1; r < 8; ++r) {
      unsigned t = 0;
      for (int i = 0; i < 3; ++i) if ((r >> i) & 1) t |= 1u << g.s[i];
      put32(off + 16 + 4 * r, lds_slot(t) << 4);
    }
    off += kGroupRecordBytes;
    ++nrec;
    first = false;
    for (TileDesc d : g.gates) {
      if (dout && &g == &groups.back() && d.opcode >= OPC_ASWAP1 && d.opcode < OPC_ASWAP1 + 9)
        d.opcode = (uint8_t)(OPC_SWAP1 + (d.opcode - OPC_ASWAP1));
      const int bytes = desc_bytes(d);
      if (!room(bytes)) return fail(QSIM_ERR_INVALID, "internal: pass record stream overflow");
      if ((d.outer_mask & ((1ull << kTileLow) - 1)) || (d.outer_mask >> kTileLow) > 0xFFFFFFFFull)
        return fail(QSIM_ERR_INVALID, "internal: outer predicate outside index bits %d..%d", kTileLow, kTileMaxQubits - 1);
      if (d.outer_zero && (d.blk_mask || !d.outer_mask))
        return fail(QSIM_ERR_INVALID, "internal: a zero-predicate needs outer bits and no lane bits");
      const uint32_t entry = d.blk_mask ? OPC_PRED_LANE : (d.outer_mask ? (d.outer_zero ? OPC_PRED_OUTER_ZERO : OPC_PRED_OUTER) : d.opcode);
      put32(off + 0, 4u * entry);
      put32(off + 4, (uint32_t)(off + bytes));
      put32(off + 8, (uint32_t)(d.outer_mask >> kTileLow));
      put32(off + 12, (uint32_t)d.blk_mask | (4u * d.opcode) << 16);
      if (d.opcode >= OPC_DENSE2 && d.opcode < OPC_DENSE2 + 9) {
        std::memcpy(base + off + bytes - 256, d.m, 256);
      } else {
        const int head = d.nd < 6 ? d.nd : 6;
        std::memcpy(base + off + 16, d.m, 8 * (size_t)head);
        if (d.nd > 6) std::memcpy(base + off + bytes - 8 * (d.nd - 6), d.m + 6, 8 * (size_t)(d.nd - 6));
      }
      off += bytes;
      ++nrec;
    }
  }
  put32(off + 0, 4u * (dout ? OPC_END_DIRECT : OPC_END));
  put32(off + 4, (uint32_t)off);
  ++nrec;
  a->nrec = nrec;
  return QSIM_OK;
}
```

### quantum_simulations_amd/csrc/tile_launch.h

```cpp
static int tile_order_for(const TileArgs&, int) {
#ifdef QSIM_PROBES
  if (tuning().tile_order >= 0) return tuning().tile_order;
#endif
  return 0;
}

static uint8_t slab_position(const TileSlab& t, int b) {
  for (int j = 0; j < 3; ++j) if (t.bit[j] == b) return (uint8_t)(t.top + j);
  for (int i = 0; i < 4; ++i) if ((t.field[i] >> b) & 1) return (uint8_t)(b - i);
  return (uint8_t)b;
}

static void probe_out_of_place(TileArgs* args, const qsim_chunk* c) {
#ifdef QSIM_PROBES
  if (getenv("QSIM_DEBUG_OUT_OF_PLACE")) {
    static double2* other = nullptr;
    static size_t other_bytes = 0;
    const size_t need = sizeof(double2) << c->k;
    if (other_bytes < need) { if (other) (void)hipFree(other); (void)hipMalloc((void**)&other, need); other_bytes = need; }
    args->amp_out = other;
  }
#endif
}
static void probe_stamps_arm(TileArgs* args, u64 ntiles, hipStream_t stream) {
#ifdef QSIM_PROBES
  static unsigned long long* dbuf = nullptr;
  static const char* path = getenv("QSIM_DEBUG_STAMPS");
  if (path && !dbuf) (void)hipMalloc((void**)&dbuf, sizeof(unsigned long long) * 4 * ((1u << 22)));
  unsigned long long* p = path ? dbuf : nullptr;
  std::memcpy(reinterpret_cast<unsigned char*>(args) + kTileArgBytes - 8, &p, 8);
  if (p) (void)hipMemsetAsync(p, 0, sizeof(unsigned long long) * 4 * (ntiles / 64 + 1), stream);
#endif
}
static void probe_stamps_dump(const TileArgs& args, int nrec, u64 ntiles, hipStream_t stream) {
#ifdef QSIM_PROBES
  if (const char* path = getenv("QSIM_DEBUG_STAMPS")) {
    unsigned long long* p = nullptr;
    std::memcpy(&p, reinterpret_cast<const unsigned char*>(&args) + kTileArgBytes - 8, 8);
    std::vector<unsigned long long> host(4 * (ntiles / 64 + 1));
    (void)hipStreamSynchronize(stream);
    (void)hipMemcpy(host.data(), p, host.size() * 8, hipMemcpyDeviceToHost);
    if (FILE* f = std::fopen(path, "a")) {
      std::fprintf(f, "# pass nrec %d ntiles %llu\n", nrec, (u64)ntiles);
      for (size_t i = 0; i + 3 < host.size(); i += 4)
        if (host[i]) std::fprintf(f, "%llu %llu %llu %llu\n", host[i], host[i + 1], host[i + 2], host[i + 3]);
      std::fclose(f);
    }
  }
#endif
}

#ifndef QSIM_TILES_PER_WG
#define QSIM_TILES_PER_WG 2
#endif
template <int T, int TPW, bool PART>
static void launch_k_tile(bool nt, bool wide, unsigned grid, hipStream_t stream, const TileArgs& args) {
  if (nt && wide) hipLaunchKernelGGL((k_tile<T, true, true, TPW, PART>), dim3(grid), dim3(kTileThreads), 0, stream, args);
  else if (nt) hipLaunchKernelGGL((k_tile<T, true, false, TPW, PART>), dim3(grid), dim3(kTileThreads), 0, stream, args);
  else if (wide) hipLaunchKernelGGL((k_tile<T, false, true, TPW, PART>), dim3(grid), dim3(kTileThreads), 0, stream, args);
  else hipLaunchKernelGGL((k_tile<T, false, false, TPW, PART>), dim3(grid), dim3(kTileThreads), 0, stream, args);
}

static int tiles_per_workgroup(int k, int T, int nfix) {
  if (T > kTileBitsMax || T < kTileThreadBits) return fail(QSIM_ERR_INVALID, "internal: tile size %d not built", T);
  if (k < T) return fail(QSIM_ERR_INVALID, "internal: a %d-bit tile on a chunk of %d qubits", T, k);
  if (nfix < 0 || (nfix && (T != kTileBitsMax || nfix > 3 || k - T < nfix)))
    return fail(QSIM_ERR_INVALID, "internal: partial launch of a %d-bit tile", T);
  if (k - T - nfix >= 32) return fail(QSIM_ERR_INVALID, "internal: too many tiles");
  const u64 ntiles = 1ull << (k - T - nfix);
  constexpr int TPW = QSIM_TILES_PER_WG;
  return TPW > 1 && ntiles >= (u64)TPW * 4096 ? TPW : 1;
}

template <int T>
static int launch_tile(const TileArgs& a, const qsim_chunk* c, hipStream_t stream, double alg_bytes) {
  if constexpr (T > kTileBitsMax || T < kTileThreadBits) {
    return fail(QSIM_ERR_INVALID, "internal: tile size %d not built", T);
  } else {
  const int per_wg = tiles_per_workgroup(c->k, T, a.nfix);
  if (per_wg < 0) return per_wg;
  const u64 ntiles = 1ull << (c->k - T - a.nfix);
  TileArgs args = a;
  args.ntiles = (uint32_t)ntiles;
  args.order = (uint8_t)((a.order & ~kTileOrderMask) | (tile_order_for(a, T) & kTileOrderMask));
  args.nbits = (uint8_t)c->k;
  if (!args.amp_out) args.amp_out = args.amp;
  for (int i = 0; i < T - kTileLow; ++i) {
    if (args.perm & kTilePermIn) args.lay_in[i] = slab_position(args.slab_in, args.lay_in[i]);
    if (args.perm & kTilePermOut) args.lay_out[i] = slab_position(args.slab_out, args.lay_out[i]);
  }
  probe_out_of_place(&args, c);
  probe_stamps_arm(&args, ntiles, stream);
  bool wide = false;
  for (int i = 0; i < kTileThreadBits - kTileLow && i < T - kTileLow; ++i) wide = wide || args.lay_in[i] >= 28 || args.lay_out[i] >= 28;
  bool nt = c->span_bytes > tuning().mall_bytes;
  if (tuning().force_nt >= 0) nt = tuning().force_nt != 0;
  ProfileScope prof(6, alg_bytes, stream, nt, 32.0 * (double)(ntiles << T));
  constexpr int TPW = QSIM_TILES_PER_WG;
  const bool two = per_wg > 1;
  const unsigned grid = (unsigned)(two ? ntiles / TPW : ntiles);
  bool part = false;
  if constexpr (T == kTileBitsMax) {
    part = args.nfix != 0;
    if (part && two) launch_k_tile<T, TPW, true>(nt, wide, grid, stream, args);
    else if (part) launch_k_tile<T, 1, true>(nt, wide, grid, stream, args);
  }
  if (!part && two) launch_k_tile<T, TPW, false>(nt, wide, grid, stream, args);
  else if (!part) launch_k_tile<T, 1, false>(nt, wide, grid, stream, args);
  prof.done(stream);
  HIP_TRY(hipGetLastError());
  if (!part) probe_stamps_dump(args, a.nrec, ntiles, stream);
  return QSIM_OK;
  }
}

static int launch_tile_any(const TileArgs& a, int T, const qsim_chunk* c, hipStream_t stream, double alg_bytes) {
  switch (T) {
    case 8: return launch_tile<8>(a, c, stream, alg_bytes);
    case 9: return launch_tile<9>(a, c, stream, alg_bytes);
    case 10: return launch_tile<10>(a, c, stream, alg_bytes);
    case 11: return launch_tile<11>(a, c, stream, alg_bytes);
    case 12: return launch_tile<12>(a, c, stream, alg_bytes);
  }
  return fail(QSIM_ERR_INVALID, "internal: tile size %d", T);
}

struct SlabLayout {
  int m = 0;
  int bits[3] = {0, 0, 0};
};
static void slab_descriptor(int k, const SlabLayout& L, TileSlab* t) {
  int sorted[3] = {64, 64, 64};
  for (int j = 0; j < L.m; ++j) sorted[j] = L.bits[j];
  std::sort(sorted, sorted + L.m);
  auto below = [](int b) -> u64 { return b >= 64 ? ~0ull : ((1ull << b) - 1); };
  t->field[0] = below(sorted[0]);
  for (int i = 1; i < 4; ++i) {
    const int lo = sorted[i - 1], hi = i < 3 ? sorted[i] : 64;
    t->field[i] = lo >= 64 ? 0 : (below(hi) & ~below(lo + 1));
  }
  for (int j = 0; j < 3; ++j) t->bit[j] = (uint8_t)(j < L.m ? L.bits[j] : 63);
  t->top = (uint8_t)(k - L.m);
  std::memset(t->pad, 0, sizeof t->pad);
}
struct FusedIo {
  const qsim_chunk* src = nullptr;
  SlabLayout in;
  qsim_chunk* dst = nullptr;
  SlabLayout out;
  qsim_chunk* dst_own = nullptr;
  int own_pattern = -1;
  bool parts = false;
  bool fused_in = false, fused_out = false;
  bool own_in_chunk = false;
};

struct PendingLast {
  enum Mode { kNone = 0, kStashed, kTile, kPack, kDone };
  int mode = kNone;
  TileArgs a;
  int T = 0;
  double alg_bytes = 0;
  int m = 0;
  int32_t bits[3] = {0, 0, 0};
  qsim_chunk* dst = nullptr;
  qsim_chunk* dst_own = nullptr;
  int own_pattern = -1;
  int nb = 0;
  int piece_bit[3] = {0, 0, 0};
  int nb_free = 0;
  unsigned stored = 0;
  unsigned launched = 0;
};

static int piece_bits_for(int k, int m, int want, int min_piece_bits) {
  int nb = 0;
  while (nb < 3 && (2 << nb) <= want && (k - m) - (nb + 1) >= min_piece_bits && (k - m) - (nb + 1) >= kTileLow) ++nb;
  return nb;
}

static void top_free_bits(int k, int m, const int32_t* slab_bits, int nb, int* out) {
  for (int b = k - 1, found = 0; b >= 0 && found < nb; --b) {
    bool slab = false;
    for (int i = 0; i < m; ++i) slab = slab || slab_bits[i] == b;
    if (!slab) out[nb - 1 - found++] = b;
  }
}

static void plan_parts(PendingLast* p, int k, int want, const uint8_t* tile_high, int n_tile_high, int min_piece_bits) {
  auto is_tile = [&](int b) { for (int j = 0; j < n_tile_high; ++j) if (tile_high[j] == b) return true; return false; };
  p->nb = piece_bits_for(k, p->m, want, min_piece_bits);
  top_free_bits(k, p->m, p->bits, p->nb, p->piece_bit);
  p->nb_free = 0;
  while (p->nb_free < p->nb && !is_tile(p->piece_bit[p->nb - 1 - p->nb_free])) ++p->nb_free;
  p->stored = p->launched = 0;
}

static void prepare_planned(qsim_chunk* c, TileArgs& a, int T, bool first, bool last, FusedIo* io) {
  a.amp = c->amp;
  a.amp_out = c->amp;
  a.amp_out_own = nullptr;
  a.perm = 0;
  if (io && first && io->src) {
    a.amp = io->src->amp;
    a.perm |= kTilePermIn;
    slab_descriptor(c->k, io->in, &a.slab_in);
    io->fused_in = true;
  }
  if (io && last && io->dst) {
    bool clash = false;
    for (int j = 0; j < T - kTileLow; ++j)
      for (int i = 0; i < io->out.m; ++i) clash = clash || a.h[j] == io->out.bits[i];
    if (!clash || io->own_pattern < 0) {
      a.amp_out = io->dst->amp;
      a.perm |= kTilePermOut;
      slab_descriptor(c->k, io->out, &a.slab_out);
      if (io->own_pattern >= 0) {
        a.perm |= kTileOwnOut;
        a.amp_out_own = io->dst_own->amp;
        if (first && io->src && io->dst_own->amp == io->src->amp) {
          a.amp_out_own = c->amp;
          io->own_in_chunk = true;
        }
        a.own_mask = a.own_value = 0;
        for (int i = 0; i < io->out.m; ++i) {
          a.own_mask |= 1ull << io->out.bits[i];
          if ((io->own_pattern >> i) & 1) a.own_value |= 1ull << io->out.bits[i];
        }
      }
      io->fused_out = true;
    }
  }
}

static int dispatch_planned(qsim_chunk* c, TileArgs& a, int T, double alg_bytes, bool last, FusedIo* io) {
  if (io && last && io->dst && io->parts && io->fused_out && T == kTileBitsMax) {
    PendingLast* p = c->pending ? c->pending : (c->pending = new PendingLast());
    p->mode = PendingLast::kStashed; p->a = a; p->T = T; p->alg_bytes = alg_bytes; p->launched = 0;
    return QSIM_OK;
  }
  if (tuning().debug_stats < 2) return launch_tile_any(a, T, c, c->stream, alg_bytes);
  hipEvent_t e0, e1;
  (void)hipEventCreate(&e0); (void)hipEventCreate(&e1);
  (void)hipEventRecord(e0, c->stream);
  const int rc = launch_tile_any(a, T, c, c->stream, alg_bytes);
  (void)hipEventRecord(e1, c->stream);
  (void)hipEventSynchronize(e1);
  float ms = 0;
  (void)hipEventElapsedTime(&ms, e0, e1);
  std::fprintf(stderr, "[qsim] timed pass: %.3f ms, %d records, high bits", ms, a.nrec);
  for (int j = 0; j < T - kTileLow; ++j) std::fprintf(stderr, " %d", a.h[j]);
  std::fprintf(stderr, "\n");
  (void)hipEventDestroy(e0); (void)hipEventDestroy(e1);
  return rc;
}

static int launch_planned(qsim_chunk* c, TileArgs& a, int T, double alg_bytes, bool first, bool last, FusedIo* io) {
  prepare_planned(c, a, T, first, last, io);
  return dispatch_planned(c, a, T, alg_bytes, last, io);
}

struct CachedPass { TileArgs a; int T; double alg_bytes; };
struct CachedPlan {
  int k = 0;
  u64 hash = 0;
  std::vector<unsigned char> key;
  std::vector<CachedPass> passes;
};
constexpr size_t kPlanCacheEntries = 8;
constexpr size_t kPlanCacheMaxKeyBytes = 4u << 20;
static std::list<CachedPlan> g_plan_cache;
static std::mutex g_plan_cache_mu;

static int run_fused(qsim_chunk* c, const std::vector<FusedOp>& ops, int* n_passes, FusedIo* io = nullptr,
                     int n_ops = 0, const int32_t* nq = nullptr, const int32_t* qubits = nullptr, const double* mats = nullptr,
                     std::vector<CachedPass>* defer = nullptr, const TileHint* hint = nullptr) {
  std::vector<unsigned char> key;
  u64 hash = 0;
  const size_t hint_bytes = hint ? sizeof(uint64_t) * (size_t)hint->n : 0;
  const size_t key_bytes = (size_t)n_ops * (sizeof(int32_t) * 3 + sizeof(double) * 32) + hint_bytes;
  const bool cacheable = nq && qubits && mats && n_ops > 0 && key_bytes <= kPlanCacheMaxKeyBytes && tuning().debug_stats == 0 &&
                         tuning().debug_skip_gates == 0;
  if (cacheable) {
    key.resize(key_bytes);
    unsigned char* w = key.data();
    std::memcpy(w, nq, sizeof(int32_t) * (size_t)n_ops); w += sizeof(int32_t) * (size_t)n_ops;
    std::memcpy(w, qubits, sizeof(int32_t) * 2 * (size_t)n_ops); w += sizeof(int32_t) * 2 * (size_t)n_ops;
    std::memcpy(w, mats, sizeof(double) * 32 * (size_t)n_ops); w += sizeof(double) * 32 * (size_t)n_ops;
    if (hint_bytes) std::memcpy(w, hint->masks, hint_bytes);
    hash = fnv1a(key.data(), key.size(), 1469598103934665603ull ^ (u64)c->k);
    std::vector<CachedPass> hit;
    {
      std::lock_guard<std::mutex> lock(g_plan_cache_mu);
      for (auto it = g_plan_cache.begin(); it != g_plan_cache.end(); ++it)
        if (it->hash == hash && it->k == c->k && it->key == key) {
          g_plan_cache.splice(g_plan_cache.begin(), g_plan_cache, it);
          hit = g_plan_cache.front().passes;
          break;
        }
    }
    if (!hit.empty()) {
      for (size_t p = 0; p < hit.size(); ++p) {
        if (defer) {
          prepare_planned(c, hit[p].a, hit[p].T, p == 0, p + 1 == hit.size(), io);
          defer->push_back(hit[p]);
          continue;
        }
        const int rc = launch_planned(c, hit[p].a, hit[p].T, hit[p].alg_bytes, p == 0, p + 1 == hit.size(), io);
        if (rc) return rc;
      }
      *n_passes = (int)hit.size();
      return QSIM_OK;
    }
  }
  std::vector<CachedPass> made;
  const int rc = plan_fused(c->k, ops, n_passes, [&](TileArgs& a, int T, double alg_bytes, bool first, bool last) {
    if (cacheable) made.push_back(CachedPass{a, T, alg_bytes});
    if (defer) {
      prepare_planned(c, a, T, first, last, io);
      defer->push_back(CachedPass{a, T, alg_bytes});
      return (int)QSIM_OK;
    }
    return launch_planned(c, a, T, alg_bytes, first, last, io);
  }, hint);
  if (rc == QSIM_OK && cacheable && !made.empty()) {
    std::lock_guard<std::mutex> lock(g_plan_cache_mu);
    g_plan_cache.emplace_front();
    CachedPlan& e = g_plan_cache.front();
    e.k = c->k; e.hash = hash; e.key.swap(key); e.passes.swap(made);
    while (g_plan_cache.size() > kPlanCacheEntries) g_plan_cache.pop_back();
  }
  return rc;
}
```

### quantum_simulations_amd/csrc/tile_planner.h

```cpp
constexpr int kTileMinChunk = kTileThreadBits > 8 ? kTileThreadBits : 8;

struct TileHint { const uint64_t* masks; int n; };
struct PeekPlan {
  int n_total;
  const uint8_t* done;
  uint64_t avoid;
  uint64_t tile_mask;
  uint64_t need_mask;
  std::vector<size_t>* members;
};

struct PassBuilder {
  const Tuning& tune;
  const std::vector<FusedOp>& ops;
  const int k, T, low, cap;
  const size_t n_ops;
  std::vector<char> done;
  std::vector<u64> qm, need;
  std::vector<u64> tm;
  std::vector<u64> xm;
  u64 all_qubits, rank_bits;
  bool lookahead;
  size_t remaining, first = 0;
  int scan_window;
  static constexpr int kSaturated = 64;
  bool tie_break;
  u64 jit_state;
  u64 forced_static = 0;
  int anchor;
  std::vector<u64> cands, cands2;
  std::vector<size_t> trial;

  PassBuilder(int k_, const std::vector<FusedOp>& ops_, int n_bits)
      : tune(tuning()), ops(ops_), k(k_), T(k_ < kTileBitsMax ? k_ : kTileBitsMax), low(kTileLow), cap(T - kTileLow),
        n_ops(ops_.size()), done(ops_.size(), 0), qm(ops_.size()), need(ops_.size()), tm(ops_.size()), xm(ops_.size()) {
    for (size_t i = 0; i < n_ops; ++i) {
      qm[i] = op_qmask(ops[i]);
      need[i] = 0;
      tm[i] = xm[i] = 0;
      for (int t = 0; t < ops[i].ntargets; ++t) {
        tm[i] |= 1ull << ops[i].target[t];
        if (ops[i].target[t] >= low) need[i] |= 1ull << ops[i].target[t];
      }
      if (ops[i].kind == TG_SWAP1 && tune.plan_commute >= 2) xm[i] = tm[i];
      if (!tune.plan_commute) tm[i] = qm[i];
    }
    all_qubits = n_bits >= 64 ? ~0ull : ((1ull << n_bits) - 1);
    rank_bits = all_qubits & ~(k >= 64 ? ~0ull : ((1ull << k) - 1));
    lookahead = tune.plan_lookahead >= 0 ? tune.plan_lookahead != 0 : k >= 24;
    remaining = n_ops;
    scan_window = tune.plan_scan_window;
    tie_break = tune.plan_conflict_cost < 0;
    jit_state = 0x9E3779B97F4A7C15ull * (u64)(tune.plan_jitter + 1);
    for (int b = low; b < low + tune.plan_force_low && b < k && __builtin_popcountll(forced_static) < cap; ++b) forced_static |= 1ull << b;
    anchor = tune.plan_anchor;
  }

  struct Blocked {
    const PassBuilder& pb;
    u64 bt = 0, bd = 0, bx = 0;
    bool admits(size_t i) const { return !(pb.qm[i] & bt) && !(pb.tm[i] & bd) && !((pb.qm[i] & ~pb.xm[i]) & bx); }
    bool add(size_t i) {
      bt |= pb.tm[i] & ~pb.xm[i];
      bx |= pb.xm[i];
      bd |= pb.qm[i] & ~pb.tm[i];
      return bt == pb.all_qubits;
    }
  };

  void begin_pass() {
    while (first < n_ops && done[first]) ++first;
    scan_window = remaining > 4 * (size_t)tune.plan_scan_window ? std::max(1, tune.plan_scan_window * 2 / 3) : tune.plan_scan_window;
  }

  int holds(u64 tile_mask, std::vector<size_t>* out) const {
    Blocked blocked{*this};
    int count = 0, seen = 0;
    for (size_t i = first; i < n_ops && count < tune.max_gates_per_pass; ++i) {
      if (done[i]) continue;
      if (++seen > scan_window) break;
      if (!blocked.admits(i) || (need[i] & ~tile_mask)) {
        if (blocked.add(i)) break;
        continue;
      }
      ++count;
      if (out) out->push_back(i);
    }
    return count;
  }
  static int conflicts(u64 mask) {
    int c = 0;
    for (int b = 13; b <= 16; ++b) c += 2 * (int)(((mask >> b) & (mask >> (b + 7)) & 1));
    for (int b = 18; b <= 19; ++b) c += (int)(((mask >> b) & (mask >> (b + 8)) & 1));
    return c;
  }
  int penalty(u64 mask) const { return tune.plan_conflict_cost > 0 ? tune.plan_conflict_cost * conflicts(mask) / 2 : 0; }
  unsigned jitter() { jit_state ^= jit_state << 13; jit_state ^= jit_state >> 7; jit_state ^= jit_state << 17; return (unsigned)(jit_state >> 33); }
  int keyed(int count, u64 mask) {
    if (tune.plan_jitter > 0) return (count - (int)(jitter() % 8 == 0) - (int)(jitter() % 16 == 0)) * 64 + (int)(jitter() % 64);
    return tie_break ? count * 64 - conflicts(mask) : count;
  }
  static u64 mask_of(const std::vector<int>& bits, size_t n) { u64 m = 0; for (size_t i = 0; i < n && i < bits.size(); ++i) m |= 1ull << bits[i]; return m; }

  u64 grow(u64 mask) {
    while (__builtin_popcountll(mask) < cap) {
      int pick = -1, pick_count = -(1 << 20);
      for (int b = low; b < k; ++b) {
        if ((mask >> b) & 1) continue;
        const int c = keyed(holds(mask | (1ull << b), nullptr) - penalty(mask | (1ull << b)), mask | (1ull << b));
        if (c > pick_count) { pick_count = c; pick = b; }
      }
      if (pick < 0) break;
      mask |= 1ull << pick;
    }
    return mask;
  }


  u64 first_come(u64 forced, std::vector<int>* claimed) const {
    const int n_forced = __builtin_popcountll(forced);
    Blocked blocked{*this};
    u64 mask = forced;
    int count = 0, seen = 0;
    for (size_t i = first; i < n_ops && count < tune.max_gates_per_pass; ++i) {
      if (done[i]) continue;
      if (++seen > scan_window) break;
      bool ok = blocked.admits(i);
      const u64 extra = need[i] & ~mask;
      if (ok && (n_forced + (int)claimed->size() + __builtin_popcountll(extra) > cap || (extra & rank_bits))) ok = false;
      if (!ok) { if (blocked.add(i)) break; continue; }
      for (u64 e = extra; e; e &= e - 1) claimed->push_back(__builtin_ctzll(e));
      mask |= extra;
      ++count;
    }
    return mask;
  }

  void candidates(std::vector<u64>* out, size_t max_seed, size_t seed_step, u64 prev, bool always = false) {
    u64 forced = forced_static;
    if (anchor > 0 && prev) {
      for (int picked = 0; picked < anchor && picked < cap; ++picked) {
        int pick = -1, pick_count = -(1 << 20);
        for (int b = low; b < k; ++b) {
          if (!((prev >> b) & 1) || ((forced >> b) & 1)) continue;
          const int c = holds(forced | (1ull << b), nullptr);
          if (c > pick_count) { pick_count = c; pick = b; }
        }
        if (pick < 0) break;
        forced |= 1ull << pick;
      }
    }
    std::vector<int> claimed;
    first_come(forced, &claimed);
    out->clear();
    out->push_back(forced | mask_of(claimed, claimed.size()));
    if (!((lookahead || always) && k - low > cap) || holds(out->front(), nullptr) >= kSaturated) return;
    for (size_t seed = 0; seed <= max_seed && seed <= claimed.size(); seed += seed_step)
      out->push_back(grow(forced | mask_of(claimed, seed)));
  }

  std::vector<int> filled(std::vector<int> high) const {
    for (int b = low; (int)high.size() < cap && b < k; ++b)
      if (std::find(high.begin(), high.end(), b) == high.end()) high.push_back(b);
    std::sort(high.begin(), high.end());
    return high;
  }
  std::vector<int> bits_of(u64 mask) const {
    std::vector<int> high;
    for (int b = low; b < k; ++b) if ((mask >> b) & 1) high.push_back(b);
    return high;
  }

  void emit(const std::vector<size_t>& members, const std::vector<int>& high, std::vector<TileGroup>* groups, std::vector<char>* emitted) const {
    emitted->assign(members.size(), 0);
    GroupEmitter::emit(ops, members, high, T, groups, emitted);
    if (lookahead && tune.tile_direct && tune.tile_last_search && T == kTileBitsMax) {
      auto trips = [&](const std::vector<TileGroup>& g) {
        return g.empty() ? 1 << 20 : (int)g.size() + (g.front().s[0] < kTileLow) + (g.back().s[0] < kTileLow);
      };
      auto count = [](const std::vector<char>& e) { size_t c = 0; for (char x : e) c += x != 0; return c; };
      std::vector<char> emitted2(members.size(), 0);
      std::vector<TileGroup> groups2;
      GroupEmitter::emit(ops, members, high, T, &groups2, &emitted2, true);
      if (count(emitted2) > count(*emitted) || (count(emitted2) == count(*emitted) && trips(groups2) < trips(*groups))) {
        groups->swap(groups2);
        emitted->swap(emitted2);
      }
    }
  }

  u64 choose_tile(const TileHint* hint, int pass, u64 prev_mask, bool depth2) {
    if (hint && pass < hint->n) {
      const u64 m = hint->masks[pass] & all_qubits & ~((1ull << low) - 1);
      if (m && __builtin_popcountll(m) <= cap && holds(m, nullptr) > 0) return m;
    }
    candidates(&cands, 6, 2, prev_mask);
    u64 best_mask = cands[0];
    int best_score = -(1 << 20);
    for (size_t ci = 0; ci < cands.size(); ++ci) {
      trial.clear();
      int score = std::min(holds(cands[ci], &trial), kSaturated) - penalty(cands[ci]);
      if (depth2 && cands.size() > 1 && trial.size() < remaining) {
        const size_t first_saved = first;
        for (size_t i : trial) done[i] = 1;
        while (first < n_ops && done[first]) ++first;
        candidates(&cands2, 4, 4, cands[ci]);
        int next_best = 0;
        for (u64 m2 : cands2) next_best = std::max(next_best, std::min(holds(m2, nullptr), kSaturated) - penalty(m2));
        for (size_t i : trial) done[i] = 0;
        first = first_saved;
        score += next_best;
      } else if (depth2 && trial.size() >= remaining) {
        score += 2 * kSaturated;
      }
      score = keyed(score, cands[ci]);
      if (score > best_score) { best_score = score; best_mask = cands[ci]; }
    }
    return best_mask;
  }

  u64 keep_needed(const std::vector<size_t>& members, u64 avoid, std::vector<int>* high) const {
    u64 needed = 0;
    for (size_t i : members) needed |= need[i];
    std::vector<int> kept;
    for (int b : *high) if ((needed >> b) & 1) kept.push_back(b);
    for (int b = low; (int)kept.size() < cap && b < k; ++b)
      if (!((avoid >> b) & 1) && std::find(kept.begin(), kept.end(), b) == kept.end()) kept.push_back(b);
    *high = kept;
    return needed;
  }
  double account(const std::vector<size_t>& members, const std::vector<char>& emitted, size_t* n_emitted) {
    double alg_bytes = 0;
    *n_emitted = 0;
    for (size_t mi = 0; mi < members.size(); ++mi)
      if (emitted[mi]) {
        const FusedOp& o = ops[members[mi]];
        const int halvings = o.kind == TG_PHASE ? o.nbits : (o.control >= 0 ? 1 : o.halvings);
        alg_bytes += 32.0 * (double)((1ull << k) >> halvings) + 32.0 * (double)(1ull << k) * o.absorbed;
        done[members[mi]] = 1; --remaining; ++*n_emitted;
      }
    return alg_bytes;
  }
};

#ifdef QSIM_PROBES
static std::vector<int> probe_int_list(const char* name) {
  std::vector<int> bits;
  if (const char* e = getenv(name))
    for (const char* p = e; *p;) { bits.push_back(atoi(p)); while (*p && *p != ',') ++p; if (*p) ++p; }
  return bits;
}
#endif
static void probe_tile_bits(int k, int low, int cap, std::vector<int>* high_io) {
#ifdef QSIM_PROBES
  std::vector<int>& high = *high_io;
  const int mode = tuning().debug_skip_gates;
  if (mode == 2) for (int j = 0; j < cap; ++j) high[j] = low + j;
  if (mode == 3) for (int j = 0; j < cap; ++j) high[j] = k - cap + j;
  if (mode == 4) {
    const std::vector<int> bits = probe_int_list("QSIM_DEBUG_TILE_BITS");
    if ((int)bits.size() == cap) { high = bits; std::sort(high.begin(), high.end()); }
  }
#endif
}
static void probe_strip_gates(std::vector<TileGroup>* groups) {
#ifdef QSIM_PROBES
  if (tuning().debug_skip_gates) {
    groups->resize(1);
    (*groups)[0].gates.clear();
  }
#endif
}
static void probe_remap_tile(int T, int cap, TileArgs* a) {
#ifdef QSIM_PROBES
  std::vector<int> bits = probe_int_list("QSIM_DEBUG_REMAP_TILE");
  if ((int)bits.size() == cap && T == kTileBitsMax) {
    std::sort(bits.begin(), bits.end());
    uint8_t map[64];
    for (int b = 0; b < 64; ++b) map[b] = (uint8_t)b;
    for (int j = 0; j < cap; ++j) map[a->h[j]] = (uint8_t)bits[(size_t)j];
    for (int j = 0; j < cap; ++j) { a->lay_in[j] = map[a->lay_in[j]]; a->lay_out[j] = map[a->lay_out[j]]; }
    for (int j = 0; j < cap; ++j) a->h[j] = (uint8_t)bits[(size_t)j];
  }
#endif
}

template <class Sink>
static int plan_fused(int k, const std::vector<FusedOp>& ops_in, int* n_passes, Sink&& sink, const TileHint* hint = nullptr,
                      PeekPlan* peek = nullptr) {
  const Tuning& tune = tuning();
  const std::vector<FusedOp> ops = planned_ops(ops_in);
  PassBuilder pb(k, ops, peek ? peek->n_total : k);
  const int T = pb.T;
  *n_passes = 0;
  if (peek) {
    pb.remaining = 0;
    for (size_t i = 0; i < pb.n_ops; ++i) { pb.done[i] = peek->done[i] != 0; pb.remaining += !pb.done[i]; }
    peek->tile_mask = peek->need_mask = 0;
    peek->members->clear();
  }
  const bool depth2 = tune.plan_lookahead >= 0 ? tune.plan_lookahead >= 2 : k >= 26;
  u64 prev_mask = 0;
  while (pb.remaining) {
    pb.begin_pass();
    const u64 best_mask = pb.choose_tile(hint, *n_passes, prev_mask, depth2);
    std::vector<int> high = pb.bits_of(best_mask);
    std::vector<size_t> members;
    pb.holds(best_mask, &members);
    if (peek) {
      if (members.empty()) { *n_passes = 0; return QSIM_OK; }
      peek->need_mask = pb.keep_needed(members, peek->avoid, &high);
    }
    if (members.empty()) return fail(QSIM_ERR_INVALID, "internal: fused planner made no progress");
    high = pb.filled(high);
    prev_mask = PassBuilder::mask_of(high, high.size());
    probe_tile_bits(k, pb.low, pb.cap, &high);
    TileArgs a;
    std::memset(&a, 0, sizeof a);
    a.T = T;
    for (size_t j = 0; j < high.size(); ++j) a.h[j] = (uint8_t)high[j];
    std::vector<char> emitted;
    std::vector<TileGroup> groups;
    pb.emit(members, high, &groups, &emitted);
    size_t n_emitted = 0;
    const double alg_bytes = pb.account(members, emitted, &n_emitted);
    if (!n_emitted) return fail(QSIM_ERR_INVALID, "internal: fused planner emitted nothing");
    if (peek) {
      for (int b : high) peek->tile_mask |= 1ull << b;
      for (size_t mi = 0; mi < members.size(); ++mi) if (emitted[mi]) peek->members->push_back(members[mi]);
      *n_passes = 1;
      return QSIM_OK;
    }
    probe_strip_gates(&groups);
    int rc = serialize_pass(groups, &a);
    if (rc) return rc;
    probe_remap_tile(T, pb.cap, &a);
    if (tune.debug_stats) {
      size_t descs = 0;
      for (const TileGroup& g : groups) descs += g.gates.size();
      std::fprintf(stderr, "[qsim] pass %d: %zu gates, %zu groups, %zu descriptors\n", *n_passes, n_emitted, groups.size(), descs);
    }
    rc = sink(a, T, alg_bytes, *n_passes == 0, pb.remaining == 0);
    if (rc) return rc;
    ++*n_passes;
  }
  return QSIM_OK;
}
```

### quantum_simulations_amd/csrc/tile_search.h

```cpp
struct SearchNode { int parent; u64 mask; };
struct SearchState {
  std::vector<char> done;
  size_t remaining;
  int parent;
  u64 mask;
  long rank;
  int conflicts;
  u64 hash;
};

constexpr int kSearchBeamDefault = 8;
constexpr size_t kSearchPairSeeds = 10;
constexpr int kSearchBeamMax = 4096;

static int planned_tiles(int k, const std::vector<FusedOp>& ops, const TileHint* hint, std::vector<u64>* masks, int* n_passes) {
  masks->clear();
  return plan_fused(k, ops, n_passes, [&](TileArgs& a, int T, double, bool, bool) {
    u64 m = 0;
    for (int j = 0; j < T - kTileLow; ++j) m |= 1ull << a.h[j];
    masks->push_back(m);
    return (int)QSIM_OK;
  }, hint);
}

static int plan_search(int k, const std::vector<FusedOp>& ops_in, int beam, std::vector<u64>* masks, int* n_passes) {
  beam = std::max(1, std::min(beam > 0 ? beam : kSearchBeamDefault, kSearchBeamMax));
  int rc = planned_tiles(k, ops_in, nullptr, masks, n_passes);
  if (rc) return rc;
  const int greedy_passes = *n_passes;
  const std::vector<FusedOp> ops = planned_ops(ops_in);
  PassBuilder pb(k, ops, k);
  if (greedy_passes <= 1 || k - pb.low <= pb.cap) return QSIM_OK;
  const size_t n_ops = pb.n_ops;

  std::vector<std::vector<SearchNode>> nodes;
  std::vector<SearchState> states(1), children;
  states[0].done.assign(n_ops, 0);
  states[0].remaining = n_ops;
  states[0].parent = -1;
  states[0].mask = 0;
  states[0].conflicts = 0;
  std::vector<u64> cands, tried, seeds;
  std::vector<size_t> members, order;
  std::vector<int> claimed;
  std::vector<char> emitted;
  std::vector<TileGroup> groups;
  int finished = -1;
  for (int depth = 0; depth + 1 < greedy_passes && finished < 0 && !states.empty(); ++depth) {
    children.clear();
    for (size_t si = 0; si < states.size(); ++si) {
      const SearchState& s = states[si];
      pb.done = s.done;
      pb.remaining = s.remaining;
      pb.first = 0;
      pb.begin_pass();
      pb.candidates(&cands, (size_t)pb.cap, 1, s.mask, true);
      {
        PassBuilder::Blocked blocked{pb};
        int seen = 0;
        seeds.clear();
        for (size_t i = pb.first; i < n_ops; ++i) {
          if (pb.done[i]) continue;
          if (++seen > pb.scan_window) break;
          if (blocked.admits(i) && pb.need[i] && __builtin_popcountll(pb.need[i]) <= pb.cap &&
              std::find(seeds.begin(), seeds.end(), pb.need[i]) == seeds.end())
            seeds.push_back(pb.need[i]);
          if (blocked.add(i)) break;
        }
        for (u64 seed : seeds) cands.push_back(pb.grow(seed));
        for (size_t a = 0; a < seeds.size() && a < kSearchPairSeeds; ++a)
          for (size_t b = a + 1; b < seeds.size() && b < kSearchPairSeeds; ++b)
            if (__builtin_popcountll(seeds[a] | seeds[b]) <= pb.cap) cands.push_back(pb.grow(seeds[a] | seeds[b]));
      }
      tried.clear();
      for (u64 cand : cands) {
        const std::vector<int> high = pb.filled(pb.bits_of(cand));
        u64 mask = 0;
        for (int b : high) mask |= 1ull << b;
        if (std::find(tried.begin(), tried.end(), mask) != tried.end()) continue;
        tried.push_back(mask);
        members.clear();
        if (pb.holds(mask, &members) == 0) continue;
        pb.emit(members, high, &groups, &emitted);
        SearchState c;
        c.done = s.done;
        c.remaining = s.remaining;
        for (size_t mi = 0; mi < members.size(); ++mi)
          if (emitted[mi]) { c.done[members[mi]] = 1; --c.remaining; }
        if (c.remaining == s.remaining) continue;
        c.parent = depth == 0 ? -1 : (int)si;
        c.mask = mask;
        c.conflicts = s.conflicts + PassBuilder::conflicts(mask);
        c.hash = fnv1a(reinterpret_cast<const unsigned char*>(c.done.data()), n_ops);
        children.push_back(std::move(c));
      }
    }
    for (SearchState& c : children) {
      pb.done = c.done;
      pb.remaining = c.remaining;
      pb.first = 0;
      pb.begin_pass();
      claimed.clear();
      const u64 next = pb.first_come(pb.forced_static, &claimed);
      c.rank = 2 * (long)c.remaining - std::min(pb.holds(next, nullptr), PassBuilder::kSaturated);
    }
    order.resize(children.size());
    for (size_t i = 0; i < order.size(); ++i) order[i] = i;
    std::stable_sort(order.begin(), order.end(), [&](size_t a, size_t b) {
      if (children[a].rank != children[b].rank) return children[a].rank < children[b].rank;
      return children[a].conflicts < children[b].conflicts;
    });
    std::vector<SearchState> kept;
    nodes.emplace_back();
    for (size_t i : order) {
      if ((int)kept.size() >= beam) break;
      bool dup = false;
      for (const SearchState& o : kept) if (o.hash == children[i].hash && o.done == children[i].done) { dup = true; break; }
      if (dup) continue;
      nodes.back().push_back(SearchNode{children[i].parent, children[i].mask});
      kept.push_back(std::move(children[i]));
    }
    for (size_t i = 0; i < kept.size() && finished < 0; ++i) if (kept[i].remaining == 0) finished = (int)i;
    states.swap(kept);
  }
  if (finished < 0) return QSIM_OK;
  std::vector<u64> found(nodes.size());
  for (int d = (int)nodes.size() - 1, at = finished; d >= 0; --d) {
    found[(size_t)d] = nodes[(size_t)d][(size_t)at].mask;
    at = nodes[(size_t)d][(size_t)at].parent;
  }
  std::vector<u64> replay;
  int replay_passes = 0;
  const std::vector<uint64_t> named(found.begin(), found.end());
  const TileHint hint = {named.data(), (int)named.size()};
  rc = planned_tiles(k, ops_in, &hint, &replay, &replay_passes);
  if (rc) return rc;
  if (replay_passes == (int)found.size() && replay == found) { *masks = found; *n_passes = replay_passes; }
  return QSIM_OK;
}
```

### quantum_simulations_amd/kernel/planner.py

```python
from __future__ import annotations

import ctypes as C

import numpy as np

from quantum_simulations_amd import _lib
from quantum_simulations_amd._lib import ptr
from quantum_simulations_amd.kernel.device import as_packed

IMAGE_BYTES = 4096
STREAM_OFF = 192
PASS_IMAGE = np.dtype([("amp", "<u8"), ("nrec", "<i4"), ("T", "<i4"), ("h", "u1", (11,)), ("order", "u1"), ("ntiles", "<u4"),
                       ("lay_in", "u1", (12,)), ("lay_out", "u1", (12,)), ("amp_out", "<u8"),
                       ("amp_out_own", "<u8"), ("own_mask", "<u8"), ("own_value", "<u8"),
                       ("slab_in", "u1", (40,)), ("slab_out", "u1", (40,)), ("nbits", "u1"), ("perm", "u1"), ("reserved", "u1", (22,)),
                       ("stream", "u1", (IMAGE_BYTES - STREAM_OFF,))])
assert PASS_IMAGE.itemsize == IMAGE_BYTES
_FIRST_BUFFER = 64


def tile_bits(image) -> list:
    return [int(b) for b in image["h"][:int(image["T"]) - 3]]


def tile_masks(images) -> np.ndarray:
    return np.array([sum(1 << b for b in tile_bits(img)) for img in images], dtype=np.uint64)


def _plan(n: int, ops, tiles, images) -> tuple:
    nq, qubits, mats = as_packed(ops)
    lib, count = _lib.load(), C.c_int32()
    head = (n, len(nq), ptr(nq), ptr(qubits), ptr(mats))
    tail = (ptr(images), 0 if images is None else images.nbytes, C.byref(count))
    tm = np.ascontiguousarray(tiles if tiles is not None else [], dtype=np.uint64)
    rc = lib.qsim_plan_ops_tiled(*head, len(tm), ptr(tm), *tail) if len(tm) else lib.qsim_plan_ops(*head, *tail)
    return rc, count.value


def plan_ops(n: int, ops, tiles=None) -> np.ndarray:
    room = _FIRST_BUFFER
    while True:
        images = np.zeros(room, dtype=PASS_IMAGE)
        rc, count = _plan(n, ops, tiles, images)
        if rc != _lib.QSIM_ERR_INVALID or count < room:
            _lib.check(rc)
            return images[:count]
        room *= 2


def pass_count(n: int, ops, tiles=None) -> int:
    rc, count = _plan(n, ops, tiles, None)
    _lib.check(rc)
    return count


def tiles_per_workgroup(n: int, tile_bits: int, fixed_bits: int = 0) -> int:
    rc = int(_lib.load().qsim_tiles_per_workgroup(int(n), int(tile_bits), int(fixed_bits)))
    if rc < 0:
        _lib.check(rc)
    return rc


def search_tiles(n: int, ops, beam: int = 0) -> np.ndarray:
    nq, qubits, mats = as_packed(ops)
    count = C.c_int32()
    out = np.zeros(len(nq), dtype=np.uint64)
    _lib.check(_lib.load().qsim_plan_search(n, len(nq), ptr(nq), ptr(qubits), ptr(mats), beam, ptr(out), len(out), C.byref(count)))
    return out[:count.value].copy()


def rewrite_ops(n: int, ops, stats: dict = None) -> list:
    nq, qubits, mats = as_packed(ops)
    room = 2 * len(nq) + n
    out_nq, out_q = np.zeros(room, dtype=np.int32), np.zeros(2 * room, dtype=np.int32)
    out_m = np.zeros((room, 16), dtype=np.complex128)
    count, need = C.c_int32(), np.zeros(2, dtype=np.int32)
    _lib.check(_lib.load().qsim_rewrite_ops(n, len(nq), ptr(nq), ptr(qubits), ptr(mats), ptr(out_nq), ptr(out_q), ptr(out_m),
                                            room, C.byref(count), ptr(need)))
    if stats is not None:
        stats.update(ops_in=len(nq), ops_out=int(count.value), need_tile_in=int(need[0]), need_tile_out=int(need[1]))
    return [([int(out_q[2 * i])], out_m[i, :4].reshape(2, 2).copy()) if out_nq[i] == 1 else
            ([int(out_q[2 * i]), int(out_q[2 * i + 1])], out_m[i].reshape(4, 4).copy()) for i in range(count.value)]


def count_layouts(n: int, ops, layouts, threads: int) -> np.ndarray:
    nq, qubits, mats = as_packed(ops)
    lay = np.ascontiguousarray(layouts, dtype=np.int32)
    out = np.zeros(len(lay), dtype=np.int32)
    _lib.check(_lib.load().qsim_plan_count_layouts(n, len(nq), ptr(nq), ptr(qubits), ptr(mats), len(lay), ptr(lay), ptr(out), threads))
    return out


def peek_pass(k: int, n: int, nq, qubits, mats, done, members, avoid: int = 0, hint: int = 0) -> tuple:
    mask, need, count = C.c_uint64(), C.c_uint64(), C.c_int32()
    _lib.check(_lib.load().qsim_plan_peek_pass(k, n, len(nq), ptr(nq), ptr(qubits), ptr(mats), ptr(done), avoid, hint,
                                               C.byref(mask), C.byref(need), C.byref(count), ptr(members)))
    return int(mask.value), int(need.value), [int(i) for i in members[:count.value]]
```

### quantum_simulations_amd/runner/engine.py

```python
from __future__ import annotations

import numpy as np

from quantum_simulations_amd.circuit.fusion import batch_levels
from quantum_simulations_amd.circuit.io import levelize, validate_circuit_dict
from quantum_simulations_amd.kernel import gates as gate_table, planner
from quantum_simulations_amd.kernel.device import DeviceChunk


def gate_ops(cd: dict) -> list:
    return [(g["qubits"], gate_table.gate_matrix(g["gate"], g["params"])) for g in cd["gates"]]


class GpuPlan(list):
    tiles: list
    l2p: list | None = None
    model_ms: tuple | None = None


class SingleGpuEngine:

    world = 1
    rank = 0
    LAYOUT_MIN_QUBITS = 26
    LAYOUT_MIN_REPEATS = 8
    LAYOUT_CANDIDATES = 31
    LAYOUT_BEAM = 0
    LAYOUT_FINALISTS = 8

    def __init__(self, n_qubits: int, device: int = 0, mode: str = "fused", layout: str = "auto", tune_on_device: bool = False):
        if layout not in ("auto", "search", "identity"):
            raise ValueError("layout must be 'auto', 'search' or 'identity'")
        self.n = n_qubits
        self.mode = mode
        self.layout_mode = layout
        self.tune_on_device = bool(tune_on_device)
        self.state = DeviceChunk.empty(n_qubits, device)
        self.l2p: list | None = None
        self._zero = False

    def init_zero_state(self) -> None:
        self.state.init_zero(True)
        self.l2p, self._zero = None, True

    def init_random_state(self, seed: int) -> None:
        self.state.init_random(seed)
        self.l2p, self._zero = None, False

    def norm2(self) -> float:
        return self.state.norm2()

    def state_vector(self) -> np.ndarray:
        psi = self.state.download()
        if self.l2p is None:
            return psi
        from quantum_simulations_amd.circuit.staging import permute_state
        return permute_state(psi, self.l2p)

    def expectation(self, obs) -> float:
        return self.state.expectation(obs, l2p=self.l2p if self.l2p is not None else list(range(self.n)))

    def reduced_density_matrix(self, qubits) -> np.ndarray:
        l2p = self.l2p if self.l2p is not None else list(range(self.n))
        return self.state.reduced_density_matrix([l2p[int(q)] for q in qubits])

    def sample(self, shots: int, seed: int = 0, qubits=None) -> np.ndarray:
        from quantum_simulations_amd import sampling
        values = sampling.to_logical(self.state.sample(sampling.draw(shots, seed)), self.l2p)
        return values if qubits is None else sampling.marginal(values, qubits)

    def logical_index(self, offset: int, count: int) -> np.ndarray:
        x = offset + np.arange(count, dtype=np.int64)
        if self.l2p is None:
            return x
        y = np.zeros_like(x)
        for q, p in enumerate(self.l2p):
            y |= ((x >> p) & 1) << q
        return y

    def plan(self, circuit_dict: dict, repeats: int = 1) -> GpuPlan:
        cd = validate_circuit_dict(circuit_dict)
        if cd["number_of_qubits"] != self.n:
            raise ValueError(f"circuit has {cd['number_of_qubits']} qubits, engine has {self.n}")
        from quantum_simulations_amd.kernel.device import pack_ops
        if self.mode == "per-gate":
            plan = GpuPlan([pack_ops(gate_ops(cd))])
            plan.tiles = [None]
            return plan
        return self.plan_batches([p["local_ops"] for p in batch_levels(levelize(cd), self.n)], repeats)

    def plan_batches(self, batches, repeats: int = 1) -> GpuPlan:
        from quantum_simulations_amd.kernel.device import pack_ops
        search = self.layout_mode == "search" or (self.layout_mode == "auto" and repeats >= self.LAYOUT_MIN_REPEATS)
        if not search or self.n < self.LAYOUT_MIN_QUBITS:
            plan = GpuPlan([pack_ops(ops) for ops in batches])
            plan.tiles = [None] * len(batches)
            return plan
        import time
        t0 = time.perf_counter()
        tune = self.tune_on_device and self._zero
        own_batches, rewrite = batches, {"ops_in": 0, "ops_out": 0, "need_tile_in": 0, "need_tile_out": 0}
        batches = []
        for ops in own_batches:
            stats = {}
            batches.append(planner.rewrite_ops(self.n, ops, stats))
            for key in rewrite:
                rewrite[key] += stats[key]
        own_identity = int(_count_passes(self.n, own_batches, np.arange(self.n, dtype=np.int32)[None, :], 1)[0])
        finalists = choose_plan_layout(self.n, batches, self.LAYOUT_CANDIDATES, n_finalists=self.LAYOUT_FINALISTS if tune else 4,
                                       all_finalists=True, beam=self.LAYOUT_BEAM)

        def build(l2p, masks, info):
            plan = GpuPlan([pack_ops([([l2p[q] for q in qs], U) for qs, U in ops]) for ops in batches])
            plan.tiles = masks
            plan.l2p = None if l2p == list(range(self.n)) else l2p
            plan.model_ms = info["model_ms"]
            plan.layout_info = dict(info, passes_identity=own_identity, rewrite=dict(rewrite))
            return plan
        plans = [build(*f) for f in finalists]
        chosen = plans[0]
        if tune and len(plans) > 1:
            timed = []
            for p in plans:
                self.init_zero_state()
                self.execute(p)
                ms = []
                for _ in range(2):
                    self.state.time_begin()
                    self.execute(p)
                    ms.append(self.state.time_end())
                timed.append(min(ms))
            chosen = plans[int(np.argmin(timed))]
            chosen.layout_info["tuned_on_device_ms"] = [round(t, 3) for t in timed]
            self.init_zero_state()
        chosen.layout_info["seconds"] = round(time.perf_counter() - t0, 3)
        return chosen

    def _adopt_layout(self, l2p) -> None:
        if l2p == self.l2p or (l2p is None and self.l2p == list(range(self.n))):
            return
        if self._zero:
            self.l2p = l2p
            return
        SW = gate_table.SWAP()
        swaps = [([a, b], SW) for a, b in layout_swaps(self.l2p, l2p, self.n)]
        if swaps:
            self.state.apply_ops(swaps)
        self.l2p = l2p

    def execute(self, plan) -> None:
        self._adopt_layout(getattr(plan, "l2p", None))
        self._zero = False
        self.last_passes = 0
        tiles = getattr(plan, "tiles", None) or [None] * len(plan)
        for ops, masks in zip(plan, tiles):
            if masks is not None and self.mode != "per-gate":
                self.last_passes += self.state.apply_ops_tiled(ops, masks)
            else:
                self.last_passes += self.state.apply_ops(ops, fused=self.mode != "per-gate")

    def passes_per_step(self, plan: list) -> int:
        return getattr(self, "last_passes", sum(len(ops[0]) for ops in plan))

    def barrier(self) -> None:
        self.state.sync()

    def max_over_ranks(self, value: float) -> float:
        return value

    def profile_begin(self) -> None:
        self.state.profile_begin()

    def profile_end(self) -> list[dict]:
        return self.state.profile_end()

    def sweep_gates(self, n: int, reps: int = 5) -> dict:
        dev = self.state if n == self.n else DeviceChunk.empty(n, self.state.device)
        dev.init_random(30)
        if dev is self.state:
            self.l2p, self._zero = None, False
        H, T, CX = gate_table.H(), gate_table.T(), gate_table.CNOT()
        N = 1 << n

        def timed(fn) -> float:
            fn()
            dev.sync()
            ts = []
            for _ in range(reps):
                dev.time_begin()
                fn()
                ts.append(dev.time_end())
            return float(np.median(ts))

        def moved_bytes(fn) -> float:
            dev.profile_begin()
            fn()
            return float(sum(e["hbm_bytes"] for e in dev.profile_end()))

        def row(label, targets, fn, nbytes, note=None) -> dict:
            ms = [timed(lambda q=q: fn(q)) for q in targets]
            fr = [nbytes / (t * 1e-3) / 8.0e12 for t in ms]
            moved = [moved_bytes(lambda q=q: fn(q)) for q in targets]
            mf = [b / (t * 1e-3) / 8.0e12 for b, t in zip(moved, ms)]
            out = {"targets": [int(q) for q in targets], "algorithmic_bytes_per_gate": nbytes,
                   "ms_per_target": [round(t, 4) for t in ms], "frac_of_8TBps": [round(f, 4) for f in fr],
                   "moved_bytes_per_target": [int(b) for b in moved], "moved_frac": [round(f, 4) for f in mf],
                   "min_frac": round(min(fr), 4), "median_frac": round(float(np.median(fr)), 4),
                   "max_frac": round(max(fr), 4), "min_moved_frac": round(min(mf), 4),
                   "gate_apps_per_s_median": round(1e3 / float(np.median(ms)), 1)}
            if note:
                out["note"] = note
            return out

        subline = ("a diagonal / control bit below index bit 3 shares every 128-B line with the untouched half: every "
                   "line must move, so the algorithmic fraction of those targets is capped near 0.37 by construction")
        rows = {"H(q)": row("H", range(n), lambda q: dev.apply_1q(q, H), 32 * N),
                "T(q)": row("T", range(n), lambda q: dev.apply_1q(q, T), 16 * N, subline),
                "CNOT(q,q+1)": row("CX", range(n - 1), lambda q: dev.apply_2q(q, q + 1, CX), 16 * N, subline),
                "CNOT(0,q)": row("CX0", range(1, n), lambda q: dev.apply_2q(0, q, CX), 16 * N, subline)}
        rng = np.random.default_rng(4)
        dense = {}
        MFMA_F64_PEAK_TFLOPS = 78.6
        for k in (3, 4, 5, 6):
            mixed = [5, 14, n - 2, n - 9, 8, 12][:k]
            sets = [list(range(3, 3 + k)), list(range(10, 10 + k)), list(range(n - k, n)), mixed, list(range(k))]
            sets = [qs for qs in sets if max(qs) < n and len(set(qs)) == k]
            M = np.linalg.qr(rng.standard_normal((1 << k, 1 << k)) + 1j * rng.standard_normal((1 << k, 1 << k)))[0]
            ms = [timed(lambda qs=qs: dev.apply_fused_k(qs, M)) for qs in sets]
            fr = [32 * N / (t * 1e-3) / 8.0e12 for t in ms]
            flop = 8.0 * (1 << k) * N
            tf = [flop / (t * 1e-3) / 1e12 for t in ms]
            bound = "mfma" if flop / (MFMA_F64_PEAK_TFLOPS * 1e12) > 32.0 * N / 8.0e12 else "hbm"
            dense[f"k={k}"] = {"qubit_sets": sets, "sets_are": ["low", "middle", "high", "mixed", "line bits 0.." + str(k - 1)][:len(sets)],
                               "ms": [round(t, 4) for t in ms], "frac_of_8TBps": [round(f, 4) for f in fr],
                               "flop_per_amplitude": 8 * (1 << k), "achieved_TFLOPs": [round(x, 2) for x in tf],
                               "frac_of_mfma_f64_peak": [round(x / MFMA_F64_PEAK_TFLOPS, 4) for x in tf], "bound": bound,
                               "kernel": f"k_dense_mfma2<{k}> (v_mfma_f64_16x16x4_f64, 16 blocks per wave and step, in place; "
                                         + ("matrix image in LDS" if k >= 5 else "matrix image in registers") + ")"}
        norm2 = dev.norm2()
        if dev is not self.state:
            dev.close()
        return {"n_qubits": n, "reps": reps, "rows": rows, "dense_blocks": dense, "norm2_after": norm2}

    def copy_ceiling(self, reps: int = 7) -> dict:
        other = DeviceChunk.empty(self.n, self.state.device)
        other.copy_from(self.state)
        other.sync()
        ts = []
        for _ in range(reps):
            other.time_begin()
            other.copy_from(self.state)
            ts.append(other.time_end())
        other.close()
        ms = float(np.median(ts))
        gbps = 32.0 * (1 << self.n) / (ms * 1e-3) / 1e9
        return {"GBps": round(gbps, 1), "frac_of_8TBps": round(gbps / 8000.0, 4), "ms": round(ms, 4),
                "bytes": 32 * (1 << self.n), "kernel": "k_copy (read + write, non-temporal above 256 MiB)"}

    def stream_ceiling(self, reps: int = 5) -> dict:
        other = DeviceChunk.empty(self.n, self.state.device)
        nbytes = 32.0 * (1 << self.n)
        H = gate_table.H()

        def timed(fn) -> float:
            fn()
            other.sync()
            ts = []
            for _ in range(reps):
                other.time_begin()
                fn()
                ts.append(other.time_end())
            return float(np.median(ts))
        other.copy_from(self.state)
        rows = {"copy_nontemporal": timed(lambda: other.copy_from(self.state, 1)),
                "copy_plain": timed(lambda: other.copy_from(self.state, 2)),
                "copy_hipMemcpyAsync": timed(lambda: other.copy_from(self.state, 3)),
                "inplace_rmw_H_bit12": timed(lambda: other.apply_1q(min(12, self.n - 1), H)),
                "inplace_rmw_H_bit5": timed(lambda: other.apply_1q(min(5, self.n - 1), H))}
        other.close()
        gbps = {name: round(nbytes / (ms * 1e-3) / 1e9, 1) for name, ms in rows.items()}
        best = max(gbps, key=gbps.get)
        return {"GBps": gbps[best], "best": best, "frac_of_8TBps": round(gbps[best] / 8000.0, 4), "candidates_GBps": gbps,
                "bytes": int(nbytes), "note": "each candidate moves 32 B per amplitude of a buffer of the state's size; median of %d" % reps}

    def prefix_parity(self, circuit_dict: dict, n_gates: int, expected: np.ndarray) -> float:
        cd = validate_circuit_dict(circuit_dict)
        prefix = {"number_of_qubits": self.n, "gates": cd["gates"][:n_gates]}
        self.init_zero_state()
        tune, self.tune_on_device = self.tune_on_device, False
        try:
            plan = self.plan(prefix, repeats=self.LAYOUT_MIN_REPEATS)
        finally:
            self.tune_on_device = tune
        self.execute(plan)
        worst = 0.0
        step = 1 << 24
        for off in range(0, 1 << self.n, step):
            cnt = min(step, (1 << self.n) - off)
            got = self.state.download(off, cnt)
            want = expected[off:off + cnt] if self.l2p is None else expected[self.logical_index(off, cnt)]
            worst = max(worst, float(np.max(np.abs(got - want))))
        self.last_parity_layout = None if self.l2p is None else list(self.l2p)
        return worst

    def close(self) -> None:
        self.state.close()


def layout_swaps(cur, want, n: int) -> list:
    cur = list(cur) if cur is not None else list(range(n))
    want = list(want) if want is not None else list(range(n))
    at = {p: q for q, p in enumerate(cur)}
    swaps = []
    for q in range(n):
        a, b = cur[q], want[q]
        if a != b:
            other = at[b]
            swaps.append((a, b))
            at[a], at[b] = other, q
            cur[other], cur[q] = a, b
    return swaps


def _count_passes(n: int, batches, layouts: np.ndarray, threads: int) -> np.ndarray:
    total = np.zeros(len(layouts), dtype=np.int64)
    for ops in batches:
        total += planner.count_layouts(n, ops, layouts, threads) if len(ops) >= 2 else len(ops)
    return total


def choose_plan_layout(n: int, batches, n_candidates: int = 31, seed: int = 20260504, n_finalists: int = 4,
                       all_finalists: bool = False, beam: int = 0):
    import os
    from concurrent.futures import ThreadPoolExecutor

    from quantum_simulations_amd import _lib
    from quantum_simulations_amd.runner import tile_layout
    rng = np.random.default_rng(seed)
    layouts = np.tile(np.arange(n, dtype=np.int32), (n_candidates + 1, 1))
    for row in layouts[1:]:
        for bit, q in enumerate(int(x) for x in rng.choice(n, size=3, replace=False)):
            j = int(np.flatnonzero(row == bit)[0])
            row[j], row[q] = row[q], bit
    try:
        threads = len(os.sched_getaffinity(0))
    except AttributeError:
        threads = os.cpu_count() or 1
    threads = max(1, min(16, threads))
    _lib.load()

    def relabelled(lay):
        return [[([int(lay[q]) for q in qs], U) for qs, U in ops] for ops in batches]

    def search(lay):
        none = np.zeros(0, dtype=np.uint64)
        return [planner.search_tiles(n, ops, beam) if len(ops) >= 2 else none for ops in relabelled(lay)]
    with ThreadPoolExecutor(threads) as pool:
        found = list(pool.map(search, layouts))
    short = sum(len(ops) for ops in batches if len(ops) < 2)
    counts = np.array([short + sum(len(ms) for ms in f) for f in found], dtype=np.int64)
    best = int(counts.min())
    finalists = [int(i) for i in np.flatnonzero(counts == best)][:max(1, n_finalists)]
    greedy_identity = int(_count_passes(n, batches, layouts[:1], 1)[0])
    out = []
    for f in finalists:
        first = [int(x) for x in layouts[f]]
        moved = relabelled(first)
        masks = found[f]
        tiles = [[b for b in range(tile_layout.LOW, n) if (int(m) >> b) & 1] for ms in masks for m in ms]
        second, cost0, cost1 = min((tile_layout.choose_layout(tiles, n, seed=s) for s in range(1, 9)), key=lambda r: r[2])
        final_masks = [np.array([sum(1 << second[b] for b in range(n) if (int(m) >> b) & 1) for m in ms], dtype=np.uint64) for ms in masks]
        replanned = sum(planner.pass_count(n, [([second[b] for b in qs], U) for qs, U in ops], ms) if len(ops) >= 2 else len(ops)
                        for ops, ms in zip(moved, final_masks))
        if replanned != best:
            second, final_masks, cost1 = list(range(n)), [np.array(ms, dtype=np.uint64) for ms in masks], cost0
        l2p = [second[first[q]] for q in range(n)]
        info = {"passes_identity": greedy_identity, "passes_chosen": best, "candidates": n_candidates + 1,
                "candidates_by_passes": {int(c): int((counts == c).sum()) for c in np.unique(counts)},
                "passes_identity_searched": int(counts[0]), "beam": int(beam) if beam > 0 else "default",
                "model_ms": (round(cost0, 3), round(cost1, 3))}
        out.append((l2p, final_masks, info))
    out.sort(key=lambda r: r[2]["model_ms"][1])
    return out if all_finalists else out[0]


def _planned_tile_masks(n: int, ops) -> np.ndarray:
    return planner.tile_masks(planner.plan_ops(n, ops)) if len(ops) >= 2 else np.zeros(0, dtype=np.uint64)


def make_engine(n_qubits: int, world: int = 1, rank: int = 0, local_rank: int = 0,
                mode: str = "fused", **kw):
    if world == 1:
        return SingleGpuEngine(n_qubits, device=local_rank, mode=mode, layout=kw.get("layout", "auto"),
                               tune_on_device=kw.get("tune_on_device", False))
    from quantum_simulations_amd.runner.distributed import DistributedEngine
    return DistributedEngine(n_qubits, world, rank, local_rank, mode=mode, **kw)
```

### quantum_simulations_amd/runner/tile_layout.py

```python
from __future__ import annotations

import json
from pathlib import Path

import numpy as np

LOW = 3
_MODEL_PATH = Path(__file__).resolve().parent / "tile_cost_model.json"
_models: dict | None = None


def _load_models() -> dict:
    global _models
    if _models is None:
        doc = json.loads(_MODEL_PATH.read_text())
        _models = {}
        for k, m in doc["models"].items():
            nb = int(m["top"]) - LOW + 1
            tri = None
            if m.get("tri"):
                tri = np.zeros((nb, nb, nb), dtype=np.float64)
                for a, b, c, w in m["tri"]:
                    tri[int(a), int(b), int(c)] = w
            _models[int(k)] = {"c0": m["c0"], "bit": np.asarray(m["bit"], dtype=np.float64),
                               "pair": np.asarray(m["pair"], dtype=np.float64), "tri": tri, "top": int(m["top"])}
    return _models


def model_for(n: int) -> dict:
    models = _load_models()
    key = min(models, key=lambda k: (abs(k - n), k))
    return models[key]


def tile_cost(model: dict, bits) -> float:
    idx = sorted(min(int(b), model["top"]) - LOW for b in bits)
    c = model["c0"] + float(model["bit"][idx].sum())
    pair, tri = model["pair"], model.get("tri")
    for i, a in enumerate(idx):
        for j in range(i + 1, len(idx)):
            b = idx[j]
            if a == b:
                continue
            c += float(pair[a, b])
            if tri is not None:
                for d in idx[j + 1:]:
                    if d != b:
                        c += float(tri[a, b, d])
    return c


def choose_layout(tiles: list, n: int, seed: int = 1, sweeps: int = 200) -> tuple:
    import ctypes as C

    from quantum_simulations_amd import _lib
    model = model_for(n)
    if n < LOW + 2 or not tiles:
        return list(range(n)), 0.0, 0.0
    masks = np.array([sum(1 << int(q) for q in t if q >= LOW) for t in tiles], dtype=np.uint64)
    bit = np.ascontiguousarray(model["bit"], dtype=np.float64)
    pair = np.ascontiguousarray(model["pair"], dtype=np.float64)
    tri = None if model.get("tri") is None else np.ascontiguousarray(model["tri"], dtype=np.float64)
    out = np.zeros(n, dtype=np.int32)
    c0, c1 = C.c_double(), C.c_double()
    _lib.check(_lib.load().qsim_choose_layout(n, len(masks), _lib.ptr(masks), model["top"], _lib.ptr(bit), _lib.ptr(pair), _lib.ptr(tri),
                                              seed, sweeps, _lib.ptr(out), C.byref(c0), C.byref(c1)))
    base = model["c0"] * len(tiles)
    return [int(x) for x in out], c0.value + base, c1.value + base
```

Baseline: 39090.

## Add pair-tile passes that process two tiles across one extra qubit per pass

Adds a k_tile_pair kernel in which each workgroup loads the tile for one extra high qubit p along with its partner tile, applies an optional opening and closing 1-qubit op across the pair, and runs the engine stream on both halves. The planner search gains a pair mode that encodes the pair bit in the high byte of each tile mask, and the layout chooser enables it by default. The intent is to absorb gates on a qubit outside the tile and so cut the number of full statevector passes. In exchange, the record budget of a pass shrinks to make room for the pair block, there is extra planner complexity, and a heuristic pair-pass cost penalty is applied when ranking layouts.

```diff
diff --git a/include/qsim_hip.h b/include/qsim_hip.h
--- a/include/qsim_hip.h
+++ b/include/qsim_hip.h
@@ -80,6 +80,8 @@
 
 int qsim_plan_search(int n_local_qubits, int n_ops, const int32_t* nq, const int32_t* qubits, const double* mats, int beam,
                      uint64_t* out_masks, int out_capacity, int32_t* n_passes);
+int qsim_plan_search_pair(int n_local_qubits, int n_ops, const int32_t* nq, const int32_t* qubits, const double* mats, int beam,
+                          uint64_t* out_masks, int out_capacity, int32_t* n_passes);
 
 int qsim_rewrite_ops(int n_qubits, int n_ops, const int32_t* nq, const int32_t* qubits, const double* mats, int32_t* out_nq,
                      int32_t* out_qubits, double* out_mats, int out_capacity, int32_t* n_out, int32_t* need_tile);
diff --git a/quantum_simulations_amd/_lib.py b/quantum_simulations_amd/_lib.py
--- a/quantum_simulations_amd/_lib.py
+++ b/quantum_simulations_amd/_lib.py
@@ -52,6 +52,7 @@
     "qsim_plan_ops": (C.c_int, [C.c_int, C.c_int, _P, _P, _P, _P, C.c_uint64, _P]),
     "qsim_plan_ops_tiled": (C.c_int, [C.c_int, C.c_int, _P, _P, _P, C.c_int, _P, _P, C.c_uint64, _P]),
     "qsim_plan_search": (C.c_int, [C.c_int, C.c_int, _P, _P, _P, C.c_int, _P, C.c_int, _P]),
+    "qsim_plan_search_pair": (C.c_int, [C.c_int, C.c_int, _P, _P, _P, C.c_int, _P, C.c_int, _P]),
     "qsim_rewrite_ops": (C.c_int, [C.c_int, C.c_int, _P, _P, _P, _P, _P, _P, C.c_int, _P, _P]),
     "qsim_apply_ops_tiled": (C.c_int, [_P, C.c_int, _P, _P, _P, C.c_int, _P]),
     "qsim_choose_layout": (C.c_int, [C.c_int, C.c_int, _P, C.c_int, _P, _P, _P, C.c_uint64, C.c_int, _P, C.POINTER(C.c_double), C.POINTER(C.c_double)]),
diff --git a/quantum_simulations_amd/csrc/abi_plan.h b/quantum_simulations_amd/csrc/abi_plan.h
--- a/quantum_simulations_amd/csrc/abi_plan.h
+++ b/quantum_simulations_amd/csrc/abi_plan.h
@@ -38,8 +38,8 @@
   return rc;
 }
 
-int qsim_plan_search(int n_local_qubits, int n_ops, const int32_t* nq, const int32_t* qubits, const double* mats, int beam,
-                     uint64_t* out_masks, int out_capacity, int32_t* n_passes) {
+static int plan_search_abi(int n_local_qubits, int n_ops, const int32_t* nq, const int32_t* qubits, const double* mats, int beam,
+                           uint64_t* out_masks, int out_capacity, int32_t* n_passes, bool pair) {
   if (!n_passes || out_capacity < 0) return fail(QSIM_ERR_INVALID, "qsim_plan_search: bad arguments");
   if (n_local_qubits < kTileMinChunk || n_local_qubits > kTileMaxQubits)
     return fail(QSIM_ERR_INVALID, "qsim_plan_search: fused passes need %d..%d local qubits", kTileMinChunk, kTileMaxQubits);
@@ -52,7 +52,7 @@
 #endif
   std::vector<u64> masks;
   int passes = 0;
-  rc = plan_search(n_local_qubits, ops, beam, &masks, &passes);
+  rc = plan_search(n_local_qubits, ops, beam, &masks, &passes, pair);
   if (rc) return rc;
   *n_passes = passes;
   if (out_masks) {
@@ -60,6 +60,15 @@
     for (size_t p = 0; p < masks.size(); ++p) out_masks[p] = masks[p];
   }
   return QSIM_OK;
+}
+
+int qsim_plan_search(int n_local_qubits, int n_ops, const int32_t* nq, const int32_t* qubits, const double* mats, int beam,
+                     uint64_t* out_masks, int out_capacity, int32_t* n_passes) {
+  return plan_search_abi(n_local_qubits, n_ops, nq, qubits, mats, beam, out_masks, out_capacity, n_passes, false);
+}
+int qsim_plan_search_pair(int n_local_qubits, int n_ops, const int32_t* nq, const int32_t* qubits, const double* mats, int beam,
+                          uint64_t* out_masks, int out_capacity, int32_t* n_passes) {
+  return plan_search_abi(n_local_qubits, n_ops, nq, qubits, mats, beam, out_masks, out_capacity, n_passes, true);
 }
 
 int qsim_rewrite_ops(int n_qubits, int n_ops, const int32_t* nq, const int32_t* qubits, const double* mats, int32_t* out_nq,
diff --git a/quantum_simulations_amd/csrc/abi_relayout.h b/quantum_simulations_amd/csrc/abi_relayout.h
--- a/quantum_simulations_amd/csrc/abi_relayout.h
+++ b/quantum_simulations_amd/csrc/abi_relayout.h
@@ -193,6 +193,13 @@
   return QSIM_OK;
 }
 
+static std::vector<uint64_t> io_tile_masks(const qsim_ops_io* io, const FusedIo& fio) {
+  std::vector<uint64_t> masks(io->tile_masks, io->tile_masks + (io->tile_masks ? io->n_tiles : 0));
+  if (fio.src || fio.dst)
+    for (uint64_t& m : masks) m &= (1ull << kPairFieldShift) - 1;
+  return masks;
+}
+
 static int apply_ops_io_deferred(qsim_chunk* c, int n_ops, const int32_t* nq, const int32_t* qubits, const double* mats,
                                  const qsim_ops_io* io, const FusedIo& fio_in, const std::vector<FusedOp>& ops, bool tiles, int* n_passes) {
   DeferredIo* d = c->deferred ? c->deferred : (c->deferred = new DeferredIo());
@@ -208,7 +215,8 @@
   if (io->src && !d->fio.src) ++passes;
   if (tiles) {
     int p = 0;
-    const TileHint hint = {io->tile_masks, io->n_tiles};
+    const std::vector<uint64_t> masks = io_tile_masks(io, d->fio);
+    const TileHint hint = {masks.data(), io->n_tiles};
     if ((rc = run_fused(c, ops, &p, &d->fio, n_ops, nq, qubits, mats, &d->passes, io->n_tiles ? &hint : nullptr))) return rc;
     d->io.tile_masks = nullptr;
     d->io.n_tiles = 0;
@@ -293,7 +301,8 @@
   }
   if (tiles) {
     int p = 0;
-    const TileHint hint = {io->tile_masks, io->n_tiles};
+    const std::vector<uint64_t> masks = io_tile_masks(io, fio);
+    const TileHint hint = {masks.data(), io->n_tiles};
     if ((rc = run_fused(c, ops, &p, &fio, n_ops, nq, qubits, mats, nullptr, io->n_tiles ? &hint : nullptr))) return rc;
     passes += p;
     c->own_in_chunk = fio.own_in_chunk;
diff --git a/quantum_simulations_amd/csrc/tile_groups.h b/quantum_simulations_amd/csrc/tile_groups.h
--- a/quantum_simulations_amd/csrc/tile_groups.h
+++ b/quantum_simulations_amd/csrc/tile_groups.h
@@ -81,6 +81,7 @@
   const std::vector<size_t>& members;
   const std::vector<int>& high;
   const int T, low = kTileLow;
+  const int budget;
   std::vector<TileGroup>* out;
   std::vector<char>* emitted;
   const unsigned line_bits = (1u << kTileLow) - 1;
@@ -100,14 +101,15 @@
   struct Half { FusedOp op; size_t stands_for; };
 
   GroupEmitter(const std::vector<FusedOp>& ops_, const std::vector<size_t>& members_, const std::vector<int>& high_, int T_,
-               std::vector<TileGroup>* out_, std::vector<char>* emitted_)
-      : ops(ops_), members(members_), high(high_), T(T_), out(out_), emitted(emitted_),
+               std::vector<TileGroup>* out_, std::vector<char>* emitted_, int budget_)
+      : ops(ops_), members(members_), high(high_), T(T_), budget(budget_), out(out_), emitted(emitted_),
         direct_ends(tuning().tile_direct && T_ == kTileBitsMax), done(members_.size(), 0), left(members_.size()),
         reserved(members_.size(), 0) {}
 
   static void emit(const std::vector<FusedOp>& ops, const std::vector<size_t>& members, const std::vector<int>& high, int T,
-                   std::vector<TileGroup>* out, std::vector<char>* emitted, bool last_search = false) {
-    GroupEmitter e(ops, members, high, T, out, emitted);
+                   std::vector<TileGroup>* out, std::vector<char>* emitted, bool last_search = false,
+                   int budget = kTileRecordBudget) {
+    GroupEmitter e(ops, members, high, T, out, emitted, budget);
     out->clear();
     if (e.direct_ends && last_search && members.size() > 1) e.reserve_last();
     while (e.left > e.n_reserved) {
@@ -145,7 +147,7 @@
     int count = 0, bytes = kGroupRecordBytes;
     for (size_t mi = members.size(); mi-- > 0;) {
       const Pending& t = tail[mi];
-      if ((blocked & t.qm) || (t.need & ~own) || bytes + t.bytes > kTileRecordBudget / 2) { blocked |= t.qm; continue; }
+      if ((blocked & t.qm) || (t.need & ~own) || bytes + t.bytes > budget / 2) { blocked |= t.qm; continue; }
       bytes += t.bytes;
       ++count;
       if (mark) (*mark)[mi] = 1;
@@ -196,7 +198,7 @@
       bool ok = !(blocked & pd.qm);
       if (ok && first_come && __builtin_popcount(claimed | pd.need) > kGroupBits) ok = false;
       if (ok && !first_come && (pd.need & ~own)) ok = false;
-      if (ok && est + pd.bytes > kTileRecordBudget) ok = false;
+      if (ok && est + pd.bytes > budget) ok = false;
       if (!ok) { blocked |= pd.qm; continue; }
       claimed |= pd.need;
       est += pd.bytes;
@@ -352,7 +354,7 @@
       const OpShape shape = op_shape(o);
       {
         const bool mergeable = merge_on && o.kind == TG_PHASE;
-        if (used + runs.reserve() + (mergeable ? desc_bytes(14) : desc_bytes(shape.nd)) + item.with_next > kTileRecordBudget) { cut = true; break; }
+        if (used + runs.reserve() + (mergeable ? desc_bytes(14) : desc_bytes(shape.nd)) + item.with_next > budget) { cut = true; break; }
       }
       done[item.mi] = 1;
       (*emitted)[item.mi] = 1;
diff --git a/quantum_simulations_amd/csrc/tile_kernel.h b/quantum_simulations_amd/csrc/tile_kernel.h
--- a/quantum_simulations_amd/csrc/tile_kernel.h
+++ b/quantum_simulations_amd/csrc/tile_kernel.h
@@ -80,6 +80,13 @@
 };
 constexpr uint8_t kTilePermIn = 1, kTilePermOut = 2, kTileOwnOut = 4;
 constexpr uint8_t kTileDirectIn = 0x10, kTileDirectOut = 0x20, kTileOrderMask = 0x03;
+struct TilePairOp { u64 mask; double u[8]; };
+struct TilePairBlock { uint8_t p, flags, pad[6]; TilePairOp op[2]; };
+constexpr uint8_t kTilePairPass = 0x40;
+constexpr uint8_t kTilePairOpening = 1, kTilePairClosing = 2;
+constexpr int kTilePairOff = kTileArgBytes - 8 - (int)sizeof(TilePairBlock);
+constexpr int kTilePairReserve = (int)sizeof(TilePairBlock) + 8;
+static_assert(sizeof(TilePairBlock) == 152 && kTilePairOff == 3936 && kTilePairOff % 8 == 0, "pair block: 8-byte words the kernel reads with scalar loads");
 static_assert(sizeof(TileArgs) == kTileArgBytes, "kernel arguments are one 4 KiB block");
 static_assert(offsetof(TileArgs, nbits) % 8 == 0 && offsetof(TileArgs, nfix) == offsetof(TileArgs, nbits) + 2 &&
               offsetof(TileArgs, fix_pos) == offsetof(TileArgs, nbits) + 3 && offsetof(TileArgs, fix_or) == offsetof(TileArgs, nbits) + 8,
@@ -272,6 +279,163 @@
 #endif
 }
 
+template <int T, bool NT, bool WIDE>
+__global__ __launch_bounds__(kTileThreads, tile_waves(T, 2)) void k_tile_pair(const TileArgs a) {
+  constexpr int N = 1 << T;
+  constexpr int LOW = kTileLow;
+  constexpr int NH = T - LOW;
+  constexpr int BLOCK = kTileThreads;
+  constexpr int TB = kTileThreadBits;
+  constexpr int PER = N / BLOCK;
+  static_assert(PER == 8 && (N >> kGroupBits) == BLOCK, "pair passes run on full tiles: the thread's elements are the engine's x0..x7");
+  __shared__ double2 lds[N];
+  const int tid = threadIdx.x;
+  int hs[NH];
+#pragma unroll
+  for (int j = 0; j < NH; ++j) hs[j] = __builtin_amdgcn_readfirstlane((int)a.h[j]);
+  using off_t = typename std::conditional<WIDE, u64, unsigned>::type;
+  constexpr int NTB = TB - LOW;
+  const bool din = (a.order & kTileDirectIn) != 0, dout = (a.order & kTileDirectOut) != 0;
+  auto thread_off = [&](const uint8_t* lay) -> off_t {
+    off_t o = tid & ((1 << LOW) - 1);
+#pragma unroll
+    for (int i = 0; i < NTB; ++i) o |= (off_t)((tid >> (LOW + i)) & 1) << __builtin_amdgcn_readfirstlane((int)lay[i]);
+    return o;
+  };
+  const off_t tin = thread_off(a.lay_in), tout = thread_off(a.lay_out);
+  int rin[NH - NTB], rout[NH - NTB];
+#pragma unroll
+  for (int i = NTB; i < NH; ++i) {
+    rin[i - NTB] = __builtin_amdgcn_readfirstlane((int)a.lay_in[i]);
+    rout[i - NTB] = __builtin_amdgcn_readfirstlane((int)a.lay_out[i]);
+  }
+  typedef __attribute__((address_space(4))) const u64 cu64_t;
+  auto block_words = [&](int byte_off) -> cu64_t* {
+    cu64_t* w = (cu64_t*)((__attribute__((address_space(4))) const char*)__builtin_amdgcn_kernarg_segment_ptr() + kTilePairOff + byte_off);
+    asm volatile("" : "+s"(w));
+    return w;
+  };
+  const unsigned head = __builtin_amdgcn_readfirstlane((unsigned)block_words(0)[0]);
+  const int p = (int)(head & 0xffu);
+  const bool opening = (head >> 8) & kTilePairOpening, closing = (head >> 8) & kTilePairClosing;
+  u64 base_a = (u64)blockIdx.x << LOW;
+  {
+    int pos = p;
+#pragma unroll
+    for (int j = 0; j < NH; ++j) pos -= hs[j] < p ? 1 : 0;
+    base_a = ((base_a >> pos) << (pos + 1)) | (base_a & ((1ull << pos) - 1));
+#pragma unroll
+    for (int j = 0; j < NH; ++j) {
+      const int h = hs[j];
+      base_a = ((base_a >> h) << (h + 1)) | (base_a & ((1ull << h) - 1));
+    }
+  }
+  typedef double amp_t __attribute__((ext_vector_type(2)));
+  typedef __attribute__((address_space(1))) amp_t gamp_t;
+  auto row_off = [&](int j, const int* rbits) -> u64 {
+    u64 oj = 0;
+#pragma unroll
+    for (int i = 0; i < NH - NTB; ++i) oj |= (u64)((j >> i) & 1) << rbits[i];
+    return oj;
+  };
+  auto element = [&](u64 base, int j, off_t toff, const int* rbits, double2* amp) -> gamp_t* {
+    const u64 oj = row_off(j, rbits);
+    if constexpr (WIDE) {
+      u64 t = toff;
+      asm volatile("" : "+v"(t));
+      return (gamp_t*)(u64)(amp + base + oj + t);
+    } else {
+      const u64 r = reinterpret_cast<u64>(amp + base + oj);
+      const u64 row = ((u64)__builtin_amdgcn_readfirstlane((unsigned)(r >> 32)) << 32) |
+                      (unsigned)__builtin_amdgcn_readfirstlane((unsigned)r);
+      unsigned tb = toff << 4;
+      asm volatile("" : "+v"(tb));
+      return (gamp_t*)((__attribute__((address_space(1))) char*)row + tb);
+    }
+  };
+  auto load = [&](gamp_t* q) -> amp_t { return (NT && QSIM_TILE_LOAD_NT) ? __builtin_nontemporal_load(q) : *q; };
+  auto store = [&](gamp_t* q, amp_t v) { if (NT && QSIM_TILE_STORE_NT) __builtin_nontemporal_store(v, q); else *q = v; };
+  auto pair_op = [&](int which, amp_t* lo, amp_t* hi, off_t toff, const int* rbits) {
+    cu64_t* w = block_words(8 + 72 * which);
+    const u64 mask = w[0];
+    double u[8];
+#pragma unroll
+    for (int e = 0; e < 8; ++e) u[e] = __builtin_bit_cast(double, w[1 + e]);
+    const u64 need = mask & ~base_a;
+    off_t t = toff;
+    asm volatile("" : "+v"(t));
+#pragma unroll
+    for (int j = 0; j < PER; ++j) {
+      const u64 need_j = need & ~row_off(j, rbits);
+      if constexpr (WIDE) {
+        if (need_j & ~t) continue;
+      } else {
+        if ((need_j >> 32) || ((unsigned)need_j & ~t)) continue;
+      }
+      const amp_t l = lo[j], h = hi[j];
+      lo[j] = amp_t{u[0] * l.x - u[1] * l.y + u[2] * h.x - u[3] * h.y, u[0] * l.y + u[1] * l.x + u[2] * h.y + u[3] * h.x};
+      hi[j] = amp_t{u[4] * l.x - u[5] * l.y + u[6] * h.x - u[7] * h.y, u[4] * l.y + u[5] * l.x + u[6] * h.y + u[7] * h.x};
+    }
+  };
+  const unsigned slot0 = lds_slot(tid);
+  amp_t* const tile = reinterpret_cast<amp_t*>(lds);
+  const u64 base_b = base_a | (1ull << p);
+  amp_t x[PER], oth[PER];
+#pragma unroll
+  for (int j = 0; j < PER; ++j) x[j] = load(element(base_a, j, tin, rin, a.amp));
+  if (opening) {
+#pragma unroll
+    for (int j = 0; j < PER; ++j) oth[j] = load(element(base_b, j, tin, rin, a.amp));
+    pair_op(0, x, oth, tin, rin);
+  }
+#pragma unroll 1
+  for (int it = 0; it < 2; ++it) {
+    if (!din) {
+#pragma unroll
+      for (int j = 0; j < PER; ++j) tile[slot0 + BLOCK * j] = x[j];
+      __syncthreads();
+    }
+    if (it == 0 && !opening) {
+#pragma unroll
+      for (int j = 0; j < PER; ++j) oth[j] = load(element(base_b, j, tin, rin, a.amp));
+    }
+    const u64 here = it == 0 ? base_a : base_b;
+    {
+      const auto karg = __builtin_amdgcn_kernarg_segment_ptr();
+      const unsigned baseh = __builtin_amdgcn_readfirstlane((unsigned)(here >> LOW));
+      asm volatile(QS_ENGINE_ASM_FULL
+                   : "+{v[4:7]}"(x[0]), "+{v[8:11]}"(x[1]), "+{v[12:15]}"(x[2]), "+{v[16:19]}"(x[3]),
+                     "+{v[20:23]}"(x[4]), "+{v[24:27]}"(x[5]), "+{v[28:31]}"(x[6]), "+{v[32:35]}"(x[7])
+                   : [tid] "v"(tid), [karg] "s"(karg), [baseh] "s"(baseh), [first] "i"(kTileStreamOff)
+                   : QS_ENGINE_CLOBBERS);
+    }
+    if (!dout) {
+#pragma unroll
+      for (int j = 0; j < PER; ++j) x[j] = tile[slot0 + BLOCK * j];
+    }
+    if (it == 0) {
+      if (closing) {
+#pragma unroll
+        for (int j = 0; j < PER; ++j) { const amp_t r = x[j]; x[j] = oth[j]; oth[j] = r; }
+      } else {
+#pragma unroll
+        for (int j = 0; j < PER; ++j) store(element(base_a, j, tout, rout, a.amp_out), x[j]);
+#pragma unroll
+        for (int j = 0; j < PER; ++j) x[j] = oth[j];
+      }
+      __syncthreads();
+    } else {
+      if (closing) {
+        pair_op(1, oth, x, tout, rout);
+#pragma unroll
+        for (int j = 0; j < PER; ++j) store(element(base_a, j, tout, rout, a.amp_out), oth[j]);
+      }
+#pragma unroll
+      for (int j = 0; j < PER; ++j) store(element(base_b, j, tout, rout, a.amp_out), x[j]);
+    }
+  }
+}
+
 struct TileDesc {
   uint8_t opcode;
   uint16_t blk_mask;
@@ -292,6 +456,7 @@
 constexpr int kEndRecordBytes = 16;
 constexpr int kScaleRecordBytes = 32;
 constexpr int kTileRecordBudget = kTileStreamBytes - kEndRecordBytes - kTileStreamSlack - kScaleRecordBytes;
+static_assert(kTileStreamOff + kTileRecordBudget - kTilePairReserve + kScaleRecordBytes + 64 <= kTilePairOff, "a pair pass's stream ends below its pair block");
 
 static int serialize_pass(const std::vector<TileGroup>& groups, TileArgs* a) {
   unsigned char* const base = reinterpret_cast<unsigned char*>(a);
diff --git a/quantum_simulations_amd/csrc/tile_launch.h b/quantum_simulations_amd/csrc/tile_launch.h
--- a/quantum_simulations_amd/csrc/tile_launch.h
+++ b/quantum_simulations_amd/csrc/tile_launch.h
@@ -59,6 +59,23 @@
   else if (nt) hipLaunchKernelGGL((k_tile<T, true, false, TPW, PART>), dim3(grid), dim3(kTileThreads), 0, stream, args);
   else if (wide) hipLaunchKernelGGL((k_tile<T, false, true, TPW, PART>), dim3(grid), dim3(kTileThreads), 0, stream, args);
   else hipLaunchKernelGGL((k_tile<T, false, false, TPW, PART>), dim3(grid), dim3(kTileThreads), 0, stream, args);
+}
+
+template <int T>
+static void launch_k_tile_pair(bool nt, bool wide, unsigned grid, hipStream_t stream, const TileArgs& args) {
+  if (nt && wide) hipLaunchKernelGGL((k_tile_pair<T, true, true>), dim3(grid), dim3(kTileThreads), 0, stream, args);
+  else if (nt) hipLaunchKernelGGL((k_tile_pair<T, true, false>), dim3(grid), dim3(kTileThreads), 0, stream, args);
+  else if (wide) hipLaunchKernelGGL((k_tile_pair<T, false, true>), dim3(grid), dim3(kTileThreads), 0, stream, args);
+  else hipLaunchKernelGGL((k_tile_pair<T, false, false>), dim3(grid), dim3(kTileThreads), 0, stream, args);
+}
+static int check_pair_pass(const TileArgs& a, int T, int k) {
+  TilePairBlock blk;
+  std::memcpy(&blk, reinterpret_cast<const unsigned char*>(&a) + kTilePairOff, sizeof blk);
+  bool ok = T == kTileBitsMax && kTileBitsMax - kTileLow == kTileThreadBits && k > T && !a.nfix && !a.perm && a.amp_out_own == nullptr &&
+            blk.p >= kTileLow && blk.p < k && blk.flags && !(blk.flags & ~(kTilePairOpening | kTilePairClosing));
+  for (int j = 0; ok && j < T - kTileLow; ++j) ok = a.h[j] != blk.p && a.h[j] < k;
+  for (int i = 0; ok && i < 2; ++i) ok = !(blk.op[i].mask >> k) && !((blk.op[i].mask >> blk.p) & 1);
+  return ok ? (int)QSIM_OK : fail(QSIM_ERR_INVALID, "internal: a pair pass that cannot be launched");
 }
 
 static int tiles_per_workgroup(int k, int T, int nfix) {
@@ -99,6 +116,18 @@
   constexpr int TPW = QSIM_TILES_PER_WG;
   const bool two = per_wg > 1;
   const unsigned grid = (unsigned)(two ? ntiles / TPW : ntiles);
+  if constexpr (T == kTileBitsMax && kTileBitsMax - kTileLow == kTileThreadBits) {
+    if (a.order & kTilePairPass) {
+      const int rc = check_pair_pass(args, T, c->k);
+      if (rc) return rc;
+      launch_k_tile_pair<T>(nt, wide, (unsigned)(ntiles / 2), stream, args);
+      prof.done(stream);
+      HIP_TRY(hipGetLastError());
+      return QSIM_OK;
+    }
+  } else if (a.order & kTilePairPass) {
+    return fail(QSIM_ERR_INVALID, "internal: a pair pass that cannot be launched");
+  }
   bool part = false;
   if constexpr (T == kTileBitsMax) {
     part = args.nfix != 0;
diff --git a/quantum_simulations_amd/csrc/tile_planner.h b/quantum_simulations_amd/csrc/tile_planner.h
--- a/quantum_simulations_amd/csrc/tile_planner.h
+++ b/quantum_simulations_amd/csrc/tile_planner.h
@@ -1,6 +1,7 @@
 constexpr int kTileMinChunk = kTileThreadBits > 8 ? kTileThreadBits : 8;
 
 struct TileHint { const uint64_t* masks; int n; };
+constexpr int kPairFieldShift = 56;
 struct PeekPlan {
   int n_total;
   const uint8_t* done;
@@ -88,6 +89,76 @@
     }
     return count;
   }
+  struct PairSel {
+    int p = -1;
+    long open = -1, close = -1;
+    bool any() const { return open >= 0 || close >= 0; }
+  };
+  bool pair_shape(size_t i, int p) const {
+    const FusedOp& o = ops[i];
+    return o.ntargets == 1 && o.target[0] == p && !o.control_zero && (o.kind == TG_DENSE1 || o.kind == TG_ANTI1 || o.kind == TG_SWAP1);
+  }
+  int holds_pair_form(u64 tile_mask, int p, bool allow_open, std::vector<size_t>* out, PairSel* sel) const {
+    Blocked blocked{*this};
+    int count = 0, seen = 0;
+    u64 member_q = 0;
+    *sel = PairSel();
+    sel->p = p;
+    for (size_t i = first; i < n_ops && count < tune.max_gates_per_pass; ++i) {
+      if (done[i]) continue;
+      if (++seen > scan_window) break;
+      bool ok = blocked.admits(i), as_open = false, as_close = false;
+      if (ok && (need[i] & ~tile_mask)) {
+        ok = false;
+        if (pair_shape(i, p)) {
+          if (allow_open && sel->open < 0 && sel->close < 0 && !(member_q & qm[i])) ok = as_open = true;
+          else if (sel->close < 0) ok = as_close = true;
+        }
+      }
+      if (!ok) {
+        if (blocked.add(i)) break;
+        continue;
+      }
+      ++count;
+      member_q |= qm[i];
+      if (out) out->push_back(i);
+      if (as_open) sel->open = (long)i;
+      if (as_close) {
+        sel->close = (long)i;
+        blocked.bt |= qm[i];
+        if (blocked.bt == all_qubits) break;
+      }
+    }
+    return count;
+  }
+  int holds_pair(u64 tile_mask, int p, std::vector<size_t>* out, PairSel* sel) const {
+    PairSel a, b;
+    const int closing = holds_pair_form(tile_mask, p, false, nullptr, &a), both = holds_pair_form(tile_mask, p, true, nullptr, &b);
+    const bool allow_open = both > closing;
+    if (!out) { *sel = allow_open ? b : a; return allow_open ? both : closing; }
+    return holds_pair_form(tile_mask, p, allow_open, out, sel);
+  }
+  u64 grow_pair(u64 mask, int p) {
+    PairSel sel;
+    mask &= ~(1ull << p);
+    while (__builtin_popcountll(mask) < cap) {
+      int pick = -1, pick_count = -(1 << 20);
+      for (int b = low; b < k; ++b) {
+        if (((mask >> b) & 1) || b == p) continue;
+        const u64 m = mask | (1ull << b);
+        const int c = keyed(holds_pair_form(m, p, true, nullptr, &sel) - penalty(m), m);
+        if (c > pick_count) { pick_count = c; pick = b; }
+      }
+      if (pick < 0) break;
+      mask |= 1ull << pick;
+    }
+    return mask;
+  }
+  bool pair_allowed(u64 tile_mask, int p) const {
+    return T == kTileBitsMax && kTileBitsMax - kTileLow == kTileThreadBits && k > T && p >= low && p < k && !((tile_mask >> p) & 1) &&
+           __builtin_popcountll(tile_mask) == cap;
+  }
+
   static int conflicts(u64 mask) {
     int c = 0;
     for (int b = 13; b <= 16; ++b) c += 2 * (int)(((mask >> b) & (mask >> (b + 7)) & 1));
@@ -171,9 +242,37 @@
     return high;
   }
 
-  void emit(const std::vector<size_t>& members, const std::vector<int>& high, std::vector<TileGroup>* groups, std::vector<char>* emitted) const {
+  void emit(const std::vector<size_t>& members, const std::vector<int>& high, std::vector<TileGroup>* groups, std::vector<char>* emitted,
+            const PairSel* sel = nullptr) const {
+    if (sel && sel->any()) {
+      std::vector<size_t> rest, at;
+      for (size_t mi = 0; mi < members.size(); ++mi)
+        if ((long)members[mi] != sel->open && (long)members[mi] != sel->close) { rest.push_back(members[mi]); at.push_back(mi); }
+      std::vector<char> got;
+      if (!rest.empty()) emit_records(rest, high, groups, &got, kTileRecordBudget - kTilePairReserve);
+      else groups->clear();
+      if (groups->empty()) {
+        TileGroup g;
+        for (int j = 0; j < 3; ++j) g.s[j] = T - 3 + j;
+        groups->push_back(g);
+        got.assign(rest.size(), 0);
+      }
+      emitted->assign(members.size(), 0);
+      for (size_t r = 0; r < rest.size(); ++r) (*emitted)[at[r]] = got[r];
+      bool all_before = true;
+      for (size_t mi = 0; mi < members.size(); ++mi) {
+        if ((long)members[mi] == sel->open) (*emitted)[mi] = 1;
+        else if ((long)members[mi] == sel->close) (*emitted)[mi] = all_before;
+        all_before = all_before && (*emitted)[mi];
+      }
+      return;
+    }
+    emit_records(members, high, groups, emitted, kTileRecordBudget);
+  }
+  void emit_records(const std::vector<size_t>& members, const std::vector<int>& high, std::vector<TileGroup>* groups, std::vector<char>* emitted,
+                    int budget) const {
     emitted->assign(members.size(), 0);
-    GroupEmitter::emit(ops, members, high, T, groups, emitted);
+    GroupEmitter::emit(ops, members, high, T, groups, emitted, false, budget);
     if (lookahead && tune.tile_direct && tune.tile_last_search && T == kTileBitsMax) {
       auto trips = [&](const std::vector<TileGroup>& g) {
         return g.empty() ? 1 << 20 : (int)g.size() + (g.front().s[0] < kTileLow) + (g.back().s[0] < kTileLow);
@@ -181,7 +280,7 @@
       auto count = [](const std::vector<char>& e) { size_t c = 0; for (char x : e) c += x != 0; return c; };
       std::vector<char> emitted2(members.size(), 0);
       std::vector<TileGroup> groups2;
-      GroupEmitter::emit(ops, members, high, T, &groups2, &emitted2, true);
+      GroupEmitter::emit(ops, members, high, T, &groups2, &emitted2, true, budget);
       if (count(emitted2) > count(*emitted) || (count(emitted2) == count(*emitted) && trips(groups2) < trips(*groups))) {
         groups->swap(groups2);
         emitted->swap(emitted2);
@@ -189,9 +288,15 @@
     }
   }
 
-  u64 choose_tile(const TileHint* hint, int pass, u64 prev_mask, bool depth2) {
+  u64 choose_tile(const TileHint* hint, int pass, u64 prev_mask, bool depth2, int* pair = nullptr) {
+    if (pair) *pair = -1;
     if (hint && pass < hint->n) {
       const u64 m = hint->masks[pass] & all_qubits & ~((1ull << low) - 1);
+      const int p = (int)((hint->masks[pass] >> kPairFieldShift) & 0x7f) - 1;
+      if (pair && m && pair_allowed(m, p)) {
+        PairSel sel;
+        if (holds_pair(m, p, nullptr, &sel) > 0 && sel.any()) { *pair = p; return m; }
+      }
       if (m && __builtin_popcountll(m) <= cap && holds(m, nullptr) > 0) return m;
     }
     candidates(&cands, 6, 2, prev_mask);
@@ -285,6 +390,35 @@
 #endif
 }
 
+static int write_pair_block(const std::vector<FusedOp>& ops, const std::vector<size_t>& members, const std::vector<char>& emitted,
+                            const PassBuilder::PairSel& sel, TileArgs* a) {
+  const unsigned char* const base = reinterpret_cast<const unsigned char*>(a);
+  uint32_t end_off = 0;
+  for (uint32_t off = kTileStreamOff;;) {
+    uint32_t d[2];
+    std::memcpy(d, base + off, 8);
+    if (d[1] == off) { end_off = off; break; }
+    off = d[1];
+  }
+  if ((int)end_off + 64 > kTilePairOff) return fail(QSIM_ERR_INVALID, "internal: the records of a pair pass reach its pair block");
+  TilePairBlock blk;
+  std::memset(&blk, 0, sizeof blk);
+  blk.p = (uint8_t)sel.p;
+  for (size_t mi = 0; mi < members.size(); ++mi) {
+    const bool opening = (long)members[mi] == sel.open;
+    if (!emitted[mi] || !(opening || (long)members[mi] == sel.close)) continue;
+    const FusedOp& o = ops[members[mi]];
+    TilePairOp& t = blk.op[opening ? 0 : 1];
+    t.mask = o.control >= 0 ? 1ull << o.control : 0;
+    for (int e = 0; e < 4; ++e) { t.u[2 * e] = o.m[e].x; t.u[2 * e + 1] = o.m[e].y; }
+    blk.flags |= opening ? kTilePairOpening : kTilePairClosing;
+  }
+  if (!blk.flags) return QSIM_OK;
+  std::memcpy(reinterpret_cast<unsigned char*>(a) + kTilePairOff, &blk, sizeof blk);
+  a->order |= kTilePairPass;
+  return QSIM_OK;
+}
+
 template <class Sink>
 static int plan_fused(int k, const std::vector<FusedOp>& ops_in, int* n_passes, Sink&& sink, const TileHint* hint = nullptr,
                       PeekPlan* peek = nullptr) {
@@ -303,10 +437,13 @@
   u64 prev_mask = 0;
   while (pb.remaining) {
     pb.begin_pass();
-    const u64 best_mask = pb.choose_tile(hint, *n_passes, prev_mask, depth2);
+    int pair = -1;
+    const u64 best_mask = pb.choose_tile(hint, *n_passes, prev_mask, depth2, peek ? nullptr : &pair);
     std::vector<int> high = pb.bits_of(best_mask);
     std::vector<size_t> members;
-    pb.holds(best_mask, &members);
+    PassBuilder::PairSel sel;
+    if (pair >= 0) pb.holds_pair(best_mask, pair, &members, &sel);
+    else pb.holds(best_mask, &members);
     if (peek) {
       if (members.empty()) { *n_passes = 0; return QSIM_OK; }
       peek->need_mask = pb.keep_needed(members, peek->avoid, &high);
@@ -321,7 +458,7 @@
     for (size_t j = 0; j < high.size(); ++j) a.h[j] = (uint8_t)high[j];
     std::vector<char> emitted;
     std::vector<TileGroup> groups;
-    pb.emit(members, high, &groups, &emitted);
+    pb.emit(members, high, &groups, &emitted, &sel);
     size_t n_emitted = 0;
     const double alg_bytes = pb.account(members, emitted, &n_emitted);
     if (!n_emitted) return fail(QSIM_ERR_INVALID, "internal: fused planner emitted nothing");
@@ -334,6 +471,7 @@
     probe_strip_gates(&groups);
     int rc = serialize_pass(groups, &a);
     if (rc) return rc;
+    if (sel.any() && (rc = write_pair_block(ops, members, emitted, sel, &a))) return rc;
     probe_remap_tile(T, pb.cap, &a);
     if (tune.debug_stats) {
       size_t descs = 0;
diff --git a/quantum_simulations_amd/csrc/tile_search.h b/quantum_simulations_amd/csrc/tile_search.h
--- a/quantum_simulations_amd/csrc/tile_search.h
+++ b/quantum_simulations_amd/csrc/tile_search.h
@@ -6,26 +6,39 @@
   u64 mask;
   long rank;
   int conflicts;
+  int pairs;
   u64 hash;
 };
 
 constexpr int kSearchBeamDefault = 8;
 constexpr size_t kSearchPairSeeds = 10;
 constexpr int kSearchBeamMax = 4096;
+constexpr int kSearchPairRank = 2;
+constexpr size_t kSearchPairBits = 6, kSearchPairGrowSeeds = 4;
 
 static int planned_tiles(int k, const std::vector<FusedOp>& ops, const TileHint* hint, std::vector<u64>* masks, int* n_passes) {
   masks->clear();
   return plan_fused(k, ops, n_passes, [&](TileArgs& a, int T, double, bool, bool) {
     u64 m = 0;
     for (int j = 0; j < T - kTileLow; ++j) m |= 1ull << a.h[j];
+    if (a.order & kTilePairPass) m |= (u64)(reinterpret_cast<const unsigned char*>(&a)[kTilePairOff] + 1) << kPairFieldShift;
     masks->push_back(m);
     return (int)QSIM_OK;
   }, hint);
 }
 
-static int plan_search(int k, const std::vector<FusedOp>& ops_in, int beam, std::vector<u64>* masks, int* n_passes) {
+static int plan_search(int k, const std::vector<FusedOp>& ops_in, int beam, std::vector<u64>* masks, int* n_passes, bool pair = false,
+                       int pair_rank = -1) {
   beam = std::max(1, std::min(beam > 0 ? beam : kSearchBeamDefault, kSearchBeamMax));
-  int rc = planned_tiles(k, ops_in, nullptr, masks, n_passes);
+  if (pair && pair_rank < 0) {
+    std::vector<u64> other;
+    int other_passes = 0, rc = plan_search(k, ops_in, beam, masks, n_passes, true, 0);
+    if (rc || (rc = plan_search(k, ops_in, beam, &other, &other_passes, true, kSearchPairRank))) return rc;
+    auto pairs = [](const std::vector<u64>& ms) { int c = 0; for (u64 m : ms) c += (m >> kPairFieldShift) != 0; return c; };
+    if (other_passes < *n_passes || (other_passes == *n_passes && pairs(other) < pairs(*masks))) { *masks = other; *n_passes = other_passes; }
+    return QSIM_OK;
+  }
+  int rc = pair ? plan_search(k, ops_in, beam, masks, n_passes, false) : planned_tiles(k, ops_in, nullptr, masks, n_passes);
   if (rc) return rc;
   const int greedy_passes = *n_passes;
   const std::vector<FusedOp> ops = planned_ops(ops_in);
@@ -40,9 +53,10 @@
   states[0].parent = -1;
   states[0].mask = 0;
   states[0].conflicts = 0;
+  states[0].pairs = 0;
   std::vector<u64> cands, tried, seeds;
   std::vector<size_t> members, order;
-  std::vector<int> claimed;
+  std::vector<int> claimed, pair_front;
   std::vector<char> emitted;
   std::vector<TileGroup> groups;
   int finished = -1;
@@ -72,6 +86,38 @@
           for (size_t b = a + 1; b < seeds.size() && b < kSearchPairSeeds; ++b)
             if (__builtin_popcountll(seeds[a] | seeds[b]) <= pb.cap) cands.push_back(pb.grow(seeds[a] | seeds[b]));
       }
+      u64 pair_bits = 0;
+      pair_front.clear();
+      if (pair) {
+        int seen = 0;
+        for (size_t i = pb.first; i < n_ops; ++i) {
+          if (pb.done[i]) continue;
+          if (++seen > pb.scan_window) break;
+          const int t = pb.ops[i].ntargets == 1 ? pb.ops[i].target[0] : -1;
+          if (t < pb.low || !pb.pair_shape(i, t) || ((pair_bits >> t) & 1)) continue;
+          pair_bits |= 1ull << t;
+          pair_front.push_back(t);
+        }
+      }
+      auto add_child = [&](u64 mask, const std::vector<int>& high, const PassBuilder::PairSel* sel) {
+        pb.emit(members, high, &groups, &emitted, sel);
+        SearchState c;
+        c.done = s.done;
+        c.remaining = s.remaining;
+        bool pair_ran = false;
+        for (size_t mi = 0; mi < members.size(); ++mi)
+          if (emitted[mi]) {
+            c.done[members[mi]] = 1; --c.remaining;
+            pair_ran = pair_ran || (sel && ((long)members[mi] == sel->open || (long)members[mi] == sel->close));
+          }
+        if (c.remaining == s.remaining || (sel && !pair_ran)) return;
+        c.parent = depth == 0 ? -1 : (int)si;
+        c.mask = sel ? mask | (u64)(sel->p + 1) << kPairFieldShift : mask;
+        c.conflicts = s.conflicts + PassBuilder::conflicts(mask);
+        c.pairs = s.pairs + (sel ? 1 : 0);
+        c.hash = fnv1a(reinterpret_cast<const unsigned char*>(c.done.data()), n_ops);
+        children.push_back(std::move(c));
+      };
       tried.clear();
       for (u64 cand : cands) {
         const std::vector<int> high = pb.filled(pb.bits_of(cand));
@@ -80,19 +126,41 @@
         if (std::find(tried.begin(), tried.end(), mask) != tried.end()) continue;
         tried.push_back(mask);
         members.clear();
-        if (pb.holds(mask, &members) == 0) continue;
-        pb.emit(members, high, &groups, &emitted);
-        SearchState c;
-        c.done = s.done;
-        c.remaining = s.remaining;
-        for (size_t mi = 0; mi < members.size(); ++mi)
-          if (emitted[mi]) { c.done[members[mi]] = 1; --c.remaining; }
-        if (c.remaining == s.remaining) continue;
-        c.parent = depth == 0 ? -1 : (int)si;
-        c.mask = mask;
-        c.conflicts = s.conflicts + PassBuilder::conflicts(mask);
-        c.hash = fnv1a(reinterpret_cast<const unsigned char*>(c.done.data()), n_ops);
-        children.push_back(std::move(c));
+        const int plain = pb.holds(mask, &members);
+        if (plain > 0) add_child(mask, high, nullptr);
+        int best_p = -1, best_count = plain;
+        PassBuilder::PairSel sel;
+        for (u64 pbits = pair_bits & ~mask; pbits; pbits &= pbits - 1) {
+          const int p = __builtin_ctzll(pbits);
+          if (!pb.pair_allowed(mask, p)) continue;
+          const int count = pb.holds_pair(mask, p, nullptr, &sel);
+          if (sel.any() && count > best_count) { best_count = count; best_p = p; }
+        }
+        if (best_p < 0) continue;
+        members.clear();
+        pb.holds_pair(mask, best_p, &members, &sel);
+        add_child(mask, high, &sel);
+      }
+      for (size_t pi = 0; pi < pair_front.size() && pi < kSearchPairBits; ++pi) {
+        const int p = pair_front[pi];
+        cands.clear();
+        cands.push_back(pb.grow_pair(pb.forced_static, p));
+        size_t grown = 0;
+        for (size_t a = 0; a < seeds.size() && grown < kSearchPairGrowSeeds; ++a)
+          if (!((seeds[a] >> p) & 1)) { cands.push_back(pb.grow_pair(seeds[a], p)); ++grown; }
+        for (u64 cand : cands) {
+          const std::vector<int> high = pb.filled(pb.bits_of(cand));
+          u64 mask = 0;
+          for (int b : high) mask |= 1ull << b;
+          const u64 key = mask | (u64)(p + 1) << kPairFieldShift;
+          if (!pb.pair_allowed(mask, p) || std::find(tried.begin(), tried.end(), key) != tried.end()) continue;
+          tried.push_back(key);
+          PassBuilder::PairSel sel;
+          if (pb.holds_pair(mask, p, nullptr, &sel) <= pb.holds(mask, nullptr) || !sel.any()) continue;
+          members.clear();
+          pb.holds_pair(mask, p, &members, &sel);
+          add_child(mask, high, &sel);
+        }
       }
     }
     for (SearchState& c : children) {
@@ -102,12 +170,13 @@
       pb.begin_pass();
       claimed.clear();
       const u64 next = pb.first_come(pb.forced_static, &claimed);
-      c.rank = 2 * (long)c.remaining - std::min(pb.holds(next, nullptr), PassBuilder::kSaturated);
+      c.rank = 2 * (long)c.remaining - std::min(pb.holds(next, nullptr), PassBuilder::kSaturated) + (long)(pair ? pair_rank : 0) * c.pairs;
     }
     order.resize(children.size());
     for (size_t i = 0; i < order.size(); ++i) order[i] = i;
     std::stable_sort(order.begin(), order.end(), [&](size_t a, size_t b) {
       if (children[a].rank != children[b].rank) return children[a].rank < children[b].rank;
+      if (children[a].pairs != children[b].pairs) return children[a].pairs < children[b].pairs;
       return children[a].conflicts < children[b].conflicts;
     });
     std::vector<SearchState> kept;
@@ -135,6 +204,16 @@
   const TileHint hint = {named.data(), (int)named.size()};
   rc = planned_tiles(k, ops_in, &hint, &replay, &replay_passes);
   if (rc) return rc;
-  if (replay_passes == (int)found.size() && replay == found) { *masks = found; *n_passes = replay_passes; }
+  if (!(replay_passes == (int)found.size() && replay == found)) return QSIM_OK;
+  *masks = found;
+  *n_passes = replay_passes;
+  for (size_t i = 0; pair && i < masks->size(); ++i) {
+    if (!((*masks)[i] >> kPairFieldShift)) continue;
+    std::vector<uint64_t> trial(masks->begin(), masks->end());
+    trial[i] &= (1ull << kPairFieldShift) - 1;
+    const TileHint plain = {trial.data(), (int)trial.size()};
+    if ((rc = planned_tiles(k, ops_in, &plain, &replay, &replay_passes))) return rc;
+    if (replay_passes == *n_passes && std::equal(replay.begin(), replay.end(), trial.begin())) *masks = replay;
+  }
   return QSIM_OK;
 }
diff --git a/quantum_simulations_amd/kernel/planner.py b/quantum_simulations_amd/kernel/planner.py
--- a/quantum_simulations_amd/kernel/planner.py
+++ b/quantum_simulations_amd/kernel/planner.py
@@ -16,6 +16,13 @@
                        ("slab_in", "u1", (40,)), ("slab_out", "u1", (40,)), ("nbits", "u1"), ("perm", "u1"), ("reserved", "u1", (22,)),
                        ("stream", "u1", (IMAGE_BYTES - STREAM_OFF,))])
 assert PASS_IMAGE.itemsize == IMAGE_BYTES
+ORDER_PAIR = 0x40
+PAIR_OFF = IMAGE_BYTES - 8 - 152
+PAIR_OPENING, PAIR_CLOSING = 1, 2
+PAIR_OP_OFF = (PAIR_OFF + 8, PAIR_OFF + 80)
+PAIR_FIELD_SHIFT, PAIR_FIELD_MASK = 56, 0x7F
+PAIR_BLOCK = np.dtype([("p", "u1"), ("flags", "u1"), ("pad", "u1", (6,)), ("op", [("mask", "<u8"), ("u", "<c16", (2, 2))], (2,))])
+assert PAIR_BLOCK.itemsize == 152
 _FIRST_BUFFER = 64
 
 
@@ -24,7 +31,22 @@
 
 
 def tile_masks(images) -> np.ndarray:
-    return np.array([sum(1 << b for b in tile_bits(img)) for img in images], dtype=np.uint64)
+    return np.array([sum(1 << b for b in tile_bits(img)) | ((pair_bit(img) + 1) << PAIR_FIELD_SHIFT) for img in images], dtype=np.uint64)
+
+
+def pair_block(image):
+    if not int(image["order"]) & ORDER_PAIR:
+        return None
+    return np.frombuffer(bytes(image.tobytes()), dtype=PAIR_BLOCK, count=1, offset=PAIR_OFF)[0]
+
+
+def pair_bit(image) -> int:
+    block = pair_block(image)
+    return -1 if block is None else int(block["p"])
+
+
+def mask_pair_bit(mask) -> int:
+    return ((int(mask) >> PAIR_FIELD_SHIFT) & PAIR_FIELD_MASK) - 1
 
 
 def _plan(n: int, ops, tiles, images) -> tuple:
@@ -69,6 +91,14 @@
     return out[:count.value].copy()
 
 
+def search_tiles_pair(n: int, ops, beam: int = 0) -> np.ndarray:
+    nq, qubits, mats = as_packed(ops)
+    count = C.c_int32()
+    out = np.zeros(len(nq), dtype=np.uint64)
+    _lib.check(_lib.load().qsim_plan_search_pair(n, len(nq), ptr(nq), ptr(qubits), ptr(mats), beam, ptr(out), len(out), C.byref(count)))
+    return out[:count.value].copy()
+
+
 def rewrite_ops(n: int, ops, stats: dict = None) -> list:
     nq, qubits, mats = as_packed(ops)
     room = 2 * len(nq) + n
diff --git a/quantum_simulations_amd/runner/engine.py b/quantum_simulations_amd/runner/engine.py
--- a/quantum_simulations_amd/runner/engine.py
+++ b/quantum_simulations_amd/runner/engine.py
@@ -27,6 +27,7 @@
     LAYOUT_CANDIDATES = 31
     LAYOUT_BEAM = 0
     LAYOUT_FINALISTS = 8
+    LAYOUT_PAIR = True
 
     def __init__(self, n_qubits: int, device: int = 0, mode: str = "fused", layout: str = "auto", tune_on_device: bool = False):
         if layout not in ("auto", "search", "identity"):
@@ -108,7 +109,7 @@
                 rewrite[key] += stats[key]
         own_identity = int(_count_passes(self.n, own_batches, np.arange(self.n, dtype=np.int32)[None, :], 1)[0])
         finalists = choose_plan_layout(self.n, batches, self.LAYOUT_CANDIDATES, n_finalists=self.LAYOUT_FINALISTS if tune else 4,
-                                       all_finalists=True, beam=self.LAYOUT_BEAM)
+                                       all_finalists=True, beam=self.LAYOUT_BEAM, pair=self.LAYOUT_PAIR)
 
         def build(l2p, masks, info):
             plan = GpuPlan([pack_ops([([l2p[q] for q in qs], U) for qs, U in ops]) for ops in batches])
@@ -329,19 +330,24 @@
     return total
 
 
-def choose_plan_layout(n: int, batches, n_candidates: int = 31, seed: int = 20260504, n_finalists: int = 4,
-                       all_finalists: bool = False, beam: int = 0):
-    import os
-    from concurrent.futures import ThreadPoolExecutor
-
-    from quantum_simulations_amd import _lib
-    from quantum_simulations_amd.runner import tile_layout
+def line_triple_layouts(n: int, n_candidates: int = 31, seed: int = 20260504) -> np.ndarray:
     rng = np.random.default_rng(seed)
     layouts = np.tile(np.arange(n, dtype=np.int32), (n_candidates + 1, 1))
     for row in layouts[1:]:
         for bit, q in enumerate(int(x) for x in rng.choice(n, size=3, replace=False)):
             j = int(np.flatnonzero(row == bit)[0])
             row[j], row[q] = row[q], bit
+    return layouts
+
+
+def choose_plan_layout(n: int, batches, n_candidates: int = 31, seed: int = 20260504, n_finalists: int = 4,
+                       all_finalists: bool = False, beam: int = 0, pair: bool = False):
+    import os
+    from concurrent.futures import ThreadPoolExecutor
+
+    from quantum_simulations_amd import _lib
+    from quantum_simulations_amd.runner import tile_layout
+    layouts = line_triple_layouts(n, n_candidates, seed)
     try:
         threads = len(os.sched_getaffinity(0))
     except AttributeError:
@@ -354,7 +360,8 @@
 
     def search(lay):
         none = np.zeros(0, dtype=np.uint64)
-        return [planner.search_tiles(n, ops, beam) if len(ops) >= 2 else none for ops in relabelled(lay)]
+        find = planner.search_tiles_pair if pair else planner.search_tiles
+        return [find(n, ops, beam) if len(ops) >= 2 else none for ops in relabelled(lay)]
     with ThreadPoolExecutor(threads) as pool:
         found = list(pool.map(search, layouts))
     short = sum(len(ops) for ops in batches if len(ops) < 2)
@@ -369,7 +376,11 @@
         masks = found[f]
         tiles = [[b for b in range(tile_layout.LOW, n) if (int(m) >> b) & 1] for ms in masks for m in ms]
         second, cost0, cost1 = min((tile_layout.choose_layout(tiles, n, seed=s) for s in range(1, 9)), key=lambda r: r[2])
-        final_masks = [np.array([sum(1 << second[b] for b in range(n) if (int(m) >> b) & 1) for m in ms], dtype=np.uint64) for ms in masks]
+
+        def placed(m):
+            p = planner.mask_pair_bit(m)
+            return sum(1 << second[b] for b in range(n) if (int(m) >> b) & 1) | ((second[p] + 1 if p >= 0 else 0) << planner.PAIR_FIELD_SHIFT)
+        final_masks = [np.array([placed(m) for m in ms], dtype=np.uint64) for ms in masks]
         replanned = sum(planner.pass_count(n, [([second[b] for b in qs], U) for qs, U in ops], ms) if len(ops) >= 2 else len(ops)
                         for ops, ms in zip(moved, final_masks))
         if replanned != best:
@@ -378,9 +389,10 @@
         info = {"passes_identity": greedy_identity, "passes_chosen": best, "candidates": n_candidates + 1,
                 "candidates_by_passes": {int(c): int((counts == c).sum()) for c in np.unique(counts)},
                 "passes_identity_searched": int(counts[0]), "beam": int(beam) if beam > 0 else "default",
-                "model_ms": (round(cost0, 3), round(cost1, 3))}
+                "model_ms": (round(cost0, 3), round(cost1, 3)),
+                "pair_passes": sum(planner.mask_pair_bit(m) >= 0 for ms in masks for m in ms)}
         out.append((l2p, final_masks, info))
-    out.sort(key=lambda r: r[2]["model_ms"][1])
+    out.sort(key=lambda r: r[2]["model_ms"][1] * (1.0 + tile_layout.PAIR_PASS_COST * r[2]["pair_passes"] / max(1, best)))
     return out if all_finalists else out[0]
 
 
diff --git a/quantum_simulations_amd/runner/tile_layout.py b/quantum_simulations_amd/runner/tile_layout.py
--- a/quantum_simulations_amd/runner/tile_layout.py
+++ b/quantum_simulations_amd/runner/tile_layout.py
@@ -6,6 +6,7 @@
 import numpy as np
 
 LOW = 3
+PAIR_PASS_COST = 0.036
 _MODEL_PATH = Path(__file__).resolve().parent / "tile_cost_model.json"
 _models: dict | None = None
 
```

Result: no change. 39410 (median of 6 runs) (+0.8%).
